# llliuqingyu/RSPL-SLAM

Measured on AMD Instinct MI355X. Metric: stereo frames/sec SuperPoint+SuperGlue+localBA @752x480 (all-keyframe: 2xSP, 2xSG, 1 BA per frame), higher is better.
Workload: dtype fp16 MFMA with fp32 accumulation for SuperPoint/SuperGlue (the reference's TensorRT kFP16 engines), fp32 Sinkhorn/decode, fp64 BA

## Files before the change

### include/rspl.h

```cpp
#ifndef RSPL_H_
#define RSPL_H_

#include <stddef.h>
#include <stdint.h>

#ifdef __cplusplus
extern "C" {
#endif

#define RSPL_OK 0
#define RSPL_E_ARG (-1)
#define RSPL_E_WEIGHTS (-2)
#define RSPL_E_DEVICE (-3)
#define RSPL_E_CAPACITY (-4)
#define RSPL_E_SOLVER (-5)

#define RSPL_FEATURE_ROWS 259

enum { RSPL_PREC_FP32 = 0, RSPL_PREC_FP16 = 1, RSPL_PREC_FP16X3 = 2 };

const char* rspl_last_error(void);
const char* rspl_version(void);
#define RSPL_ABI_VERSION 2
int rspl_abi_version(void);
// ... 163 lines not shown
  double th_mono_point, th_stereo_point, th_mono_line, th_stereo_line;
  int iterations_first;
  int iterations_second;
} rspl_ba_problem;

typedef struct {
  double* pose_q;
  double* pose_p;
  double* points;
  double* lines;
  uint8_t* mono_inlier;
  uint8_t* stereo_inlier;
  uint8_t* mono_line_inlier;
  uint8_t* stereo_line_inlier;
  double chi2_first;
  double chi2_second;
  int iterations_done_first;
  int iterations_done_second;
} rspl_ba_result;

typedef struct {
  int max_poses;
  int max_points;
  int max_lines;
  int max_edges;
  int device;
} rspl_ba_config;

typedef struct rspl_ba rspl_ba;

int rspl_ba_create(const rspl_ba_config* cfg, rspl_ba** out);
int rspl_ba_local(rspl_ba* ba, const rspl_ba_problem* problem, rspl_ba_result* result);
void rspl_ba_destroy(rspl_ba* ba);
int rspl_ba_submit(rspl_ba* ba, const rspl_ba_problem* problem, rspl_ba_result* result);
int rspl_ba_join(rspl_ba* ba, long long* calls, long long* iterations, double* ms);
int rspl_ba_use_reserved_cus(rspl_ba* ba, int reserve_cus);
int rspl_ba_kernel_timing(rspl_ba* ba, int every);
int rspl_ba_kernel_times(rspl_ba* ba, double* ms, long long* launches);
int rspl_ba_set_line_jacobian(rspl_ba* ba, int analytic);
#define RSPL_BA_TRACE_W 12
int rspl_ba_trace(rspl_ba* ba, double* out, int cap, int* n);
int rspl_ba_debug_stage(const rspl_ba_problem* problem, int par_edges, int rank, int nranks, int* n_local,
                        int* lm_off, int8_t* etype, int* epose, int* elm, int* ecam, int* gmap, int* lpose,
                        double* eobs);
typedef struct {
  int32_t nchk, lmchunk, dsub, lmsub;
  int32_t chunks, grid, ue_bpr;
  int64_t slots;
} rspl_ba_chunk_plan;
int rspl_ba_debug_chunk_plan(int n_landmarks, int n_poses, int max_landmarks, int max_poses,
                             rspl_ba_chunk_plan* out);
int rspl_ba_debug_chunk_geometry(int n_landmarks, int n_poses, int max_landmarks, int max_poses, int32_t* chunks,
                                 int32_t* order);

typedef int (*rspl_allreduce_fn)(void* ctx, double* d_buf, size_t count, void* stream);
int rspl_ba_set_shard(rspl_ba* ba, int rank, int nranks, rspl_allreduce_fn allreduce, void* ctx);

#define RSPL_COMM_ID_BYTES 128
typedef struct rspl_comm rspl_comm;
int rspl_comm_unique_id(uint8_t* id );
int rspl_comm_create(const uint8_t* id, int rank, int nranks, int device, rspl_comm** out);
int rspl_comm_allreduce_sum(void* comm, double* d_buf, size_t count, void* stream);
void rspl_comm_destroy(rspl_comm* comm);
int rspl_ba_set_comm(rspl_ba* ba, rspl_comm* comm);

typedef struct rspl_group rspl_group;
int rspl_group_create(int nranks, rspl_group** out);
void rspl_group_destroy(rspl_group* group);
int rspl_ba_set_group(rspl_ba* ba, rspl_group* group, int rank);

typedef struct {
  int n_cameras;
  const double* cameras;
  double pose_q[4];
  double pose_p[3];
  int n_points;
  const double* points;
  int n_mono;
  const int32_t* mono_point;
  const int32_t* mono_camera;
  const double* mono_obs;
  const uint8_t* mono_inlier_in;
  int n_stereo;
  const int32_t* stereo_point;
  const int32_t* stereo_camera;
  const double* stereo_obs;
  const uint8_t* stereo_inlier_in;
  double th_mono_point, th_stereo_point;
} rspl_frame_problem;

typedef struct {
  double pose_q[4];
  double pose_p[3];
  uint8_t* mono_inlier;
  uint8_t* stereo_inlier;
  int n_inliers;
  int rounds;
  int iterations[4];
  double chi2[4];
} rspl_frame_result;

typedef struct {
  int max_batch;
  int max_edges;
  int max_points;
  int device;
// ... 480 lines not shown
```

### rspl-slam_amd/api.py

```python
from __future__ import annotations

import ctypes as C
from dataclasses import dataclass, field
from typing import List, Optional, Tuple

import numpy as np

from . import capi


@dataclass
class SuperPointConfig:
    max_keypoints: int = 400
    keypoint_threshold: float = 0.004
    remove_borders: int = 4
    weights: str = ""
    max_height: int = 480
    max_width: int = 752
    max_batch: int = 2
    precision: int = capi.RSPL_PREC_FP32
    device: int = 0


class SuperPoint:
# ... 252 lines not shown

class LocalBA:

    def __init__(self, max_poses=32, max_points=20000, max_lines=2000, max_edges=200000, device=0):
        self._lib = capi.load()
        self._h = C.c_void_p()
        cfg = capi.BaConfig(max_poses, max_points, max_lines, max_edges, device)
        capi.check(self._lib.rspl_ba_create(C.byref(cfg), C.byref(self._h)), "rspl_ba_create")

    def run(self, problem, out=None):
        from .ba_types import DenseResult
        res = out if out is not None and out.fits(problem) else DenseResult.alloc(problem)
        P, R = problem.to_ctypes(), res.to_ctypes()
        capi.check(self._lib.rspl_ba_local(self._h, C.byref(P), C.byref(R)), "rspl_ba_local")
        res.read_back(R)
        return res

    def submit(self, problem, out=None):
        from .ba_types import DenseResult
        res = out if out is not None and out.fits(problem) else DenseResult.alloc(problem)
        P, R = problem.to_ctypes(), res.to_ctypes()
        inflight = self.__dict__.setdefault("_inflight", [])
        inflight.append((problem, res, P, R))
        capi.check(self._lib.rspl_ba_submit(self._h, C.byref(P), C.byref(R)), "rspl_ba_submit")
        return res

    def join(self):
        n, it, ms = C.c_longlong(), C.c_longlong(), C.c_double()
        rc = self._lib.rspl_ba_join(self._h, C.byref(n), C.byref(it), C.byref(ms))
        inflight, self._inflight = self.__dict__.get("_inflight", []), []
        for _, res, _, R in inflight:
            res.read_back(R)
        capi.check(rc, "rspl_ba_join")
        return n.value, it.value, ms.value

    def kernel_timing(self, every: int):
        capi.check(self._lib.rspl_ba_kernel_timing(self._h, every), "rspl_ba_kernel_timing")

    def kernel_times(self):
        ms, n = (C.c_double * 2)(), (C.c_longlong * 2)()
        capi.check(self._lib.rspl_ba_kernel_times(self._h, ms, n), "rspl_ba_kernel_times")
        return {"chunks+solve": (ms[0], n[0]), "update": (ms[1], n[1])}

    def set_line_jacobian(self, analytic: bool):
        capi.check(self._lib.rspl_ba_set_line_jacobian(self._h, 1 if analytic else 0), "rspl_ba_set_line_jacobian")

    def trace(self, cap=4096):
        if not hasattr(self._lib, "rspl_ba_trace"):
            return []
        buf, n = (C.c_double * (cap * capi.BA_TRACE_W))(), C.c_int()
        capi.check(self._lib.rspl_ba_trace(self._h, buf, cap, C.byref(n)), "rspl_ba_trace")
        a = np.frombuffer(buf, np.float64, n.value * capi.BA_TRACE_W).reshape(n.value, capi.BA_TRACE_W)
        return [dict(zip(capi.BA_TRACE_FIELDS, map(float, row))) for row in a]

    def use_reserved_cus(self, reserve_cus: int):
        capi.check(self._lib.rspl_ba_use_reserved_cus(self._h, reserve_cus), "rspl_ba_use_reserved_cus")

    def set_group(self, group: "ShardGroup", rank: int):
        capi.check(self._lib.rspl_ba_set_group(self._h, group.handle, rank), "rspl_ba_set_group")
        self._shard = group

    def set_shard(self, rank: int, nranks: int, host_allreduce):
        lib = self._lib
        AR = C.CFUNCTYPE(C.c_int, C.c_void_p, C.c_void_p, C.c_size_t, C.c_void_p)

        def cb(ctx, d_buf, count, stream):
            try:
                h = np.empty(count, np.float64)
                if lib.rspl_memcpy_d2h(h.ctypes.data, d_buf, count * 8, stream):
                    return -1
                host_allreduce(h)
                return 1 if lib.rspl_memcpy_h2d(d_buf, h.ctypes.data, count * 8, stream) else 0
            except Exception:
                return -1
        self._ar_cb = AR(cb)
        capi.check(lib.rspl_ba_set_shard(self._h, rank, nranks, self._ar_cb, None), "rspl_ba_set_shard")

    def set_comm(self, comm: "Comm"):
        capi.check(self._lib.rspl_ba_set_comm(self._h, comm.handle), "rspl_ba_set_comm")
        self._shard = comm

    def __del__(self):
        if getattr(self, "_h", None) and self._h.value:
            self._lib.rspl_ba_destroy(self._h)
            self._h = C.c_void_p()


class ShardGroup:

    def __init__(self, nranks: int):
        self._lib = capi.load()
        self.handle = C.c_void_p()
        self.nranks = nranks
        capi.check(self._lib.rspl_group_create(nranks, C.byref(self.handle)), "rspl_group_create")

    def __del__(self):
        if getattr(self, "handle", None) and self.handle.value:
            self._lib.rspl_group_destroy(self.handle)
            self.handle = C.c_void_p()


COMM_ID_BYTES = 128


def comm_unique_id() -> bytes:
    buf = (C.c_uint8 * COMM_ID_BYTES)()
# ... 579 lines not shown
```

### rspl-slam_amd/capi.py

```python
from __future__ import annotations

import ctypes as C
import os
import pathlib

PKG = pathlib.Path(__file__).resolve().parent
LIB_PATH = PKG / os.environ.get("RSPL_LIB", "librspl.so")

RSPL_OK = 0
RSPL_ABI_VERSION = 2
RSPL_PREC_FP32 = 0
RSPL_PREC_FP16 = 1
RSPL_PREC_FP16X3 = 2

BA_TRACE_W = 12
BA_TRACE_FIELDS = ("submit", "stage0", "stage1", "run0", "upload", "opt1", "opt2", "end", "slot", "grew", "iters",
                   "sync")

EXPORTS = [
    "rspl_last_error", "rspl_version", "rspl_abi_version",
    "rspl_device_count", "rspl_set_device", "rspl_malloc", "rspl_free", "rspl_memcpy_h2d", "rspl_memcpy_d2h",
    "rspl_memset", "rspl_memcpy_d2d", "rspl_stream_create", "rspl_stream_create_priority", "rspl_stream_create_reserving", "rspl_stream_destroy", "rspl_stream_synchronize",
    "rspl_device_synchronize", "rspl_event_create", "rspl_event_record", "rspl_stream_wait_event",
    "rspl_event_destroy", "rspl_timer_create", "rspl_timer_record", "rspl_timer_elapsed_ms",
    "rspl_timer_destroy",
    "rspl_sp_create", "rspl_sp_infer", "rspl_sp_infer_device", "rspl_sp_debug_maps", "rspl_sp_debug_nms", "rspl_sp_debug_layer",
    "rspl_sp_profile",
    "rspl_sp_stage_times", "rspl_sp_destroy",
    "rspl_sg_create", "rspl_sg_infer", "rspl_sg_infer_device", "rspl_sg_infer_device2", "rspl_sg_debug_scores", "rspl_sg_profile",
    "rspl_sg_status", "rspl_sg_debug_inject", "rspl_sg_debug_sinkhorn", "rspl_sg_debug_decode", "rspl_sg_debug_layers",
    "rspl_sg_debug_sinkhorn_plan",
    "rspl_sg_stage_times", "rspl_sg_destroy",
    "rspl_pm_match",
    "rspl_ba_create", "rspl_ba_local", "rspl_ba_submit", "rspl_ba_join", "rspl_ba_destroy", "rspl_ba_use_reserved_cus", "rspl_ba_kernel_timing",
    "rspl_ba_kernel_times", "rspl_ba_trace", "rspl_ba_set_line_jacobian", "rspl_ba_debug_stage",
    "rspl_ba_debug_chunk_plan", "rspl_ba_debug_chunk_geometry",
    "rspl_frame_create", "rspl_frame_optimize", "rspl_frame_destroy",
    "rspl_ba_set_shard", "rspl_comm_unique_id", "rspl_comm_create", "rspl_comm_allreduce_sum", "rspl_comm_destroy",
    "rspl_ba_set_comm", "rspl_group_create", "rspl_group_destroy", "rspl_ba_set_group",
    "rspl_pnp_create", "rspl_pnp_solve", "rspl_pnp_destroy", "rspl_pnp_debug_hypotheses",
    "rspl_line_extract", "rspl_lines_create", "rspl_lines_destroy", "rspl_lines_assign", "rspl_lines_match",
    "rspl_lines_stereo", "rspl_lines_stereo_device", "rspl_lines_status", "rspl_lines_detect",
    "rspl_lines_debug_canny",
    "rspl_lines_detect_device", "rspl_lines_detect_status", "rspl_lines_extract_async_device",
    "rspl_lines_debug_hysteresis", "rspl_lines_debug_chains", "rspl_lines_debug_fld_host",
    "rspl_lines_debug_fld_stats", "rspl_lines_debug_fld_profile", "rspl_lines_debug_fld_stage_ms",
    "rspl_track_create", "rspl_track_destroy", "rspl_track_set_keyframe", "rspl_track_enqueue", "rspl_track_fetch",
    "rspl_track_debug_stage", "rspl_track_keyframe_table",
    "rspl_track_enable_lines", "rspl_track_set_keyframe_lines", "rspl_track_enqueue_ext", "rspl_track_fetch_ext",
    "rspl_track_debug_lines", "rspl_track_frame_lines",
    "rspl_kf_create", "rspl_kf_destroy", "rspl_kf_enqueue", "rspl_kf_fetch", "rspl_kf_triangulate",
    "rspl_map_insert_keyframe", "rspl_map_get_mapline_observers",
    "rspl_rect_build_maps", "rspl_rect_debug_fixed", "rspl_rect_debug_sizeof", "rspl_rect_debug_copy", "rspl_rect_create", "rspl_rect_destroy",
    "rspl_rect_get_maps", "rspl_rect_set_maps", "rspl_rect_enqueue_device", "rspl_rect_pair",
    "rspl_rcf_debug_sizeof", "rspl_rcf_create", "rspl_rcf_destroy", "rspl_rcf_infer", "rspl_rcf_infer_device",
    "rspl_rcf_debug_logits", "rspl_rcf_debug_tile_rows", "rspl_rcf_profile", "rspl_rcf_stage_times",
    "rspl_fm_create", "rspl_fm_destroy", "rspl_fm_solve", "rspl_fm_enqueue", "rspl_fm_fetch",
    "rspl_fm_debug_subsets", "rspl_fm_debug_seven_point", "rspl_fm_debug_hypotheses",
]


class SpConfig(C.Structure):
    _fields_ = [("max_keypoints", C.c_int), ("keypoint_threshold", C.c_double), ("remove_borders", C.c_int),
                ("max_height", C.c_int), ("max_width", C.c_int), ("max_batch", C.c_int),
                ("precision", C.c_int), ("device", C.c_int)]


class SgConfig(C.Structure):
    _fields_ = [("image_width", C.c_int), ("image_height", C.c_int), ("max_keypoints", C.c_int),
                ("max_batch", C.c_int), ("sinkhorn_iterations", C.c_int), ("precision", C.c_int),
                ("device", C.c_int)]


class SgSinkhornPlan(C.Structure):
    _fields_ = [("kind", C.c_int32), ("groups", C.c_int32), ("rows_per_wave", C.c_int32), ("reserved", C.c_int32),
                ("ug_granules", C.c_uint64), ("vg_granules", C.c_uint64)]


class BaChunkPlan(C.Structure):
    _fields_ = [("nchk", C.c_int32), ("lmchunk", C.c_int32), ("dsub", C.c_int32), ("lmsub", C.c_int32),
                ("chunks", C.c_int32), ("grid", C.c_int32), ("ue_bpr", C.c_int32), ("slots", C.c_int64)]


class DMatch(C.Structure):
    _fields_ = [("query_idx", C.c_int32), ("train_idx", C.c_int32), ("distance", C.c_float)]


class BaConfig(C.Structure):
    _fields_ = [("max_poses", C.c_int), ("max_points", C.c_int), ("max_lines", C.c_int),
# ... 161 lines not shown
    lib.rspl_malloc.argtypes = [C.POINTER(vp), C.c_size_t]
    lib.rspl_free.argtypes = [vp]
    lib.rspl_memcpy_h2d.argtypes = [vp, vp, C.c_size_t, vp]
    lib.rspl_memcpy_d2h.argtypes = [vp, vp, C.c_size_t, vp]
    lib.rspl_memset.argtypes = [vp, ip, C.c_size_t, vp]
    lib.rspl_memcpy_d2d.argtypes = [vp, vp, C.c_size_t, vp]
    lib.rspl_sp_profile.argtypes = [vp, ip]
    lib.rspl_sp_stage_times.argtypes = [vp, C.POINTER(C.c_float), C.POINTER(ip)]
    lib.rspl_stream_create.argtypes = [C.POINTER(vp)]
    lib.rspl_stream_create_priority.argtypes = [C.POINTER(vp), ip]
    lib.rspl_stream_create_reserving.argtypes = [C.POINTER(vp), ip]
    lib.rspl_stream_destroy.argtypes = [vp]
    lib.rspl_stream_synchronize.argtypes = [vp]
    lib.rspl_event_create.argtypes = [C.POINTER(vp)]
    lib.rspl_event_record.argtypes = [vp, vp]
    lib.rspl_stream_wait_event.argtypes = [vp, vp]
    lib.rspl_event_destroy.argtypes = [vp]
    lib.rspl_timer_create.argtypes = [C.POINTER(vp)]
    lib.rspl_timer_record.argtypes = [vp, ip, vp]
    lib.rspl_timer_elapsed_ms.argtypes = [vp, C.POINTER(C.c_float)]
    lib.rspl_timer_destroy.argtypes = [vp]
    lib.rspl_timer_destroy.restype = None
    if hasattr(lib, "rspl_sg_create"):
        lib.rspl_sg_create.argtypes = [C.POINTER(SgConfig), C.c_char_p, C.POINTER(vp)]
        lib.rspl_sg_infer.argtypes = [vp, vp, ip, vp, ip, vp, vp, vp, vp]
        lib.rspl_sg_infer_device.argtypes = [vp, ip, vp, vp, vp, vp, ip, ip, vp, vp, vp, vp, vp]
        lib.rspl_sg_infer_device2.argtypes = [vp, ip, vp, vp, vp, vp, ip, ip, vp, vp, vp, vp, vp, vp]
        lib.rspl_sg_debug_scores.argtypes = [vp, ip, vp]
        lib.rspl_sg_status.argtypes = [vp, C.POINTER(C.c_uint32)]
        lib.rspl_sg_debug_inject.argtypes = [vp, ip, C.c_uint]
        lib.rspl_sg_debug_sinkhorn.argtypes = [vp, vp, ip, ip, C.c_float, ip, vp]
        lib.rspl_sg_debug_decode.argtypes = [vp, vp, ip, ip, vp, vp, vp, vp]
        lib.rspl_sg_debug_layers.argtypes = [vp, ip, vp, vp, vp, ip, ip, vp]
        lib.rspl_sg_debug_sinkhorn_plan.argtypes = [ip, ip, ip, C.POINTER(SgSinkhornPlan)]
        lib.rspl_sg_profile.argtypes = [vp, ip]
        lib.rspl_sg_stage_times.argtypes = [vp, C.POINTER(C.c_float), C.POINTER(ip)]
        lib.rspl_sg_destroy.argtypes = [vp]
        lib.rspl_sg_destroy.restype = None
        lib.rspl_pm_match.argtypes = [vp, vp, ip, vp, ip, C.POINTER(DMatch), ip, C.POINTER(ip), ip]
    if hasattr(lib, "rspl_ba_create"):
        lib.rspl_ba_create.argtypes = [C.POINTER(BaConfig), C.POINTER(vp)]
        lib.rspl_ba_local.argtypes = [vp, vp, vp]
        lib.rspl_ba_submit.argtypes = [vp, vp, vp]
        lib.rspl_ba_join.argtypes = [vp, vp, vp, vp]
        lib.rspl_ba_use_reserved_cus.argtypes = [vp, ip]
        lib.rspl_ba_kernel_timing.argtypes = [vp, ip]
        lib.rspl_ba_kernel_times.argtypes = [vp, C.POINTER(C.c_double), C.POINTER(C.c_longlong)]
        lib.rspl_ba_destroy.argtypes = [vp]
        lib.rspl_ba_destroy.restype = None
        lib.rspl_ba_debug_stage.argtypes = [vp, ip, ip, ip] + [vp] * 9
    if hasattr(lib, "rspl_ba_debug_chunk_plan"):
        lib.rspl_ba_debug_chunk_plan.argtypes = [ip, ip, ip, ip, C.POINTER(BaChunkPlan)]
        lib.rspl_ba_debug_chunk_geometry.argtypes = [ip, ip, ip, ip, vp, vp]
    if hasattr(lib, "rspl_ba_trace"):
        lib.rspl_ba_trace.argtypes = [vp, C.POINTER(C.c_double), ip, C.POINTER(ip)]
        lib.rspl_ba_set_line_jacobian.argtypes = [vp, ip]
    if hasattr(lib, "rspl_ba_set_shard"):
        lib.rspl_ba_set_shard.argtypes = [vp, ip, ip, vp, vp]
        lib.rspl_comm_unique_id.argtypes = [vp]
        lib.rspl_comm_create.argtypes = [vp, ip, ip, ip, C.POINTER(vp)]
        lib.rspl_comm_allreduce_sum.argtypes = [vp, vp, C.c_size_t, vp]
        lib.rspl_comm_destroy.argtypes = [vp]
        lib.rspl_comm_destroy.restype = None
        lib.rspl_ba_set_comm.argtypes = [vp, vp]
        lib.rspl_group_create.argtypes = [ip, C.POINTER(vp)]
        lib.rspl_group_destroy.argtypes = [vp]
        lib.rspl_group_destroy.restype = None
        lib.rspl_ba_set_group.argtypes = [vp, vp, ip]
    if hasattr(lib, "rspl_pnp_create"):
        lib.rspl_pnp_create.argtypes = [C.POINTER(PnpConfig), C.POINTER(vp)]
        lib.rspl_pnp_solve.argtypes = [vp, vp, ip, vp]
        lib.rspl_pnp_destroy.argtypes = [vp]
        lib.rspl_pnp_destroy.restype = None
        lib.rspl_pnp_debug_hypotheses.argtypes = [vp, C.c_int, C.c_int, vp, vp]
    if hasattr(lib, "rspl_fm_create"):
        lib.rspl_fm_create.argtypes = [C.POINTER(FmConfig), C.POINTER(vp)]
        lib.rspl_fm_destroy.argtypes = [vp]
        lib.rspl_fm_destroy.restype = None
        lib.rspl_fm_solve.argtypes = [vp, vp, ip, vp]
        lib.rspl_fm_enqueue.argtypes = [vp, ip, vp, vp]
        lib.rspl_fm_fetch.argtypes = [vp, vp]
        lib.rspl_fm_debug_subsets.argtypes = [ip, ip, vp, vp, vp, C.POINTER(C.c_int)]
        lib.rspl_fm_debug_seven_point.argtypes = [vp, vp, vp, C.POINTER(C.c_int)]
        lib.rspl_fm_debug_hypotheses.argtypes = [vp, ip, ip, vp, vp, vp]
    if hasattr(lib, "rspl_frame_create"):
        lib.rspl_frame_create.argtypes = [C.POINTER(FrameConfig), C.POINTER(vp)]
        lib.rspl_frame_optimize.argtypes = [vp, vp, ip, vp]
        lib.rspl_frame_destroy.argtypes = [vp]
        lib.rspl_frame_destroy.restype = None
    if hasattr(lib, "rspl_track_create"):
        lib.rspl_track_create.argtypes = [C.POINTER(TrackConfig), C.POINTER(vp)]
        lib.rspl_track_destroy.argtypes = [vp]
        lib.rspl_track_destroy.restype = None
        lib.rspl_track_set_keyframe.argtypes = [vp, ip, ip, vp, vp, vp, vp]
        lib.rspl_track_enqueue.argtypes = [vp, ip, vp, vp]
        lib.rspl_track_fetch.argtypes = [vp, vp]
        lib.rspl_track_debug_stage.argtypes = [vp, ip, C.POINTER(TrackDebug)]
    if hasattr(lib, "rspl_track_enable_lines"):
        lib.rspl_track_enable_lines.argtypes = [vp, C.POINTER(TrackLinesConfig)]
        lib.rspl_track_set_keyframe_lines.argtypes = [vp, ip, ip, vp, vp, vp, vp, vp, vp]
        lib.rspl_track_enqueue_ext.argtypes = [vp, ip, vp, vp, vp]
        lib.rspl_track_fetch_ext.argtypes = [vp, vp, vp]
        lib.rspl_track_debug_lines.argtypes = [vp, ip, C.POINTER(TrackDebugLines)]
        lib.rspl_track_frame_lines.argtypes = [vp, ip, C.POINTER(vp), C.POINTER(vp)]
    if hasattr(lib, "rspl_kf_create"):
        lib.rspl_track_keyframe_table.argtypes = [vp, ip, ip, C.POINTER(vp), C.POINTER(vp), C.POINTER(vp)]
# ... 165 lines not shown
```

### rspl-slam_amd/csrc/ba.cpp

```cpp
#include <immintrin.h>

#include <algorithm>
#include <chrono>
#include <cmath>
#include <cstdlib>
#include <cstring>
#include <limits>
#include <numeric>
#include <string>
#include <type_traits>
#include <memory>
#include <vector>
#include <condition_variable>
#include <deque>
#include <mutex>
#include <thread>

#include "ba_kernels.hpp"
#include "common.hpp"
#include "ba_stage.hpp"
#include "se3_host.hpp"

using namespace rspl;

// ... 27 lines not shown
  int *pp_cnt, *pp_off;
  size_t chunk_slots = 0;
  int4* pp_buf = nullptr;
  size_t pp_cap = 0;
  char* cbuf[2] = {nullptr, nullptr};
  char* stage[2] = {nullptr, nullptr};
  char* stage_dev[2] = {nullptr, nullptr};
  size_t stage_cap[2] = {0, 0};
  ba::Mail* mail = nullptr;
  ba::Mail* mail_dev = nullptr;
  unsigned long long seq = 0;
  ba::Stager stg;
  int rank = 0, nranks = 1;
  rspl_allreduce_fn allreduce = nullptr;
  void* ar_ctx = nullptr;
  double* red = nullptr;
  ba::LmCtrl* lmctl = nullptr;
  double* lm_trace = nullptr;
  double* gbuf = nullptr;
  size_t gcap = 0;
  double* pdg = nullptr;
  size_t pdg_cap = 0;
  int ktime_every = 0;
  unsigned long long ncalls = 0;
  bool ktime_on = false;
  std::vector<hipEvent_t> kev;
  std::vector<int> kev_eval;
  int kev_used = 0;
  double kt_ms[2] = {0, 0};
  long long kt_n[2] = {0, 0};
  struct Job {
    const rspl_ba_problem* pr;
    rspl_ba_result* res;
    std::shared_ptr<ba::StagedCall> sc;
    int state;
  };
  std::thread worker;
  std::thread stager;
  bool slot_busy[2] = {false, false};
  std::mutex qmu;
  std::condition_variable qcv;
  std::deque<Job> jobs;
  bool busy = false, quit = false;
  bool tracking_call = false;
  int q_err = 0;
  std::string q_msg;
  long long q_done = 0, q_iters = 0;
  double q_ms = 0.0;
  static constexpr int kTraceCap = 4096;
  std::vector<double> trace;
  long long trace_n = 0;
  unsigned grew = 0;
  int line_jac = 0;
};

namespace {

constexpr int kMaxCams = 16;
constexpr int kMaxRanks = 64;
constexpr int kParEdges = 8192;
constexpr int kChunkWaves = 1024;
constexpr int kEventTrials = 64;
int allreduce(rspl_ba* b, double* d, size_t n) {
  const int rc = b->allreduce(b->ar_ctx, d, n, b->stream);
  if (rc) {
    set_error("BA shard all-reduce failed (rank %d of %d, %zu doubles, rc %d)", b->rank, b->nranks, n, rc);
    return RSPL_E_DEVICE;
  }
  return RSPL_OK;
}


struct CallLayout {
  size_t cams, T, X, L, obs, type, pose, lm, cam, gmap, lm_pose, pidx, lm_off, lm_act, pairs, ltab, level, flags, out,
      bytes;
  CallLayout() = default;
  CallLayout(int ncam, int np, int nq, int nl, int E, size_t nobs) {
    const size_t nL = (size_t)nq + nl;
    size_t so = 0;
    auto place = [&](size_t n) {
      const size_t o = so;
      so = al256(so + n);
      return o;
    };
    cams = place(sizeof(double) * 5 * ncam); T = place(sizeof(double) * 8 * np); X = place(sizeof(double) * 3 * nq);
    L = place(sizeof(double) * 6 * nl); obs = place(sizeof(double) * nobs); type = place(E);
    pose = place(4 * (size_t)E); lm = place(4 * (size_t)E); cam = place(4 * (size_t)E); gmap = place(4 * (size_t)E);
    lm_pose = place(4 * (size_t)E);
    pidx = place(4 * (size_t)np); lm_off = place(4 * (nL + 1)); lm_act = place(nL);
    pairs = place(8 * (size_t)np * (np + 1) / 2);
    const size_t line_edges = nobs >= 4 * (size_t)E ? (nobs - 4 * (size_t)E) / 4 : 0;
    ltab = place(16 * ((size_t)nl + line_edges / ba::kLineBlk + 2));
    level = place(E); flags = place(4 * sizeof(int)); out = place(8 * sizeof(double));
    bytes = so;
  }
};

struct DownLayout {
  size_t inl, T, X, L, bytes;
  DownLayout() = default;
  DownLayout(int np, int nq, int nl, int E) {
    inl = 0; T = al256(E); X = T + al256(sizeof(double) * 8 * np); L = X + al256(sizeof(double) * 3 * nq);
    bytes = L + al256(sizeof(double) * 6 * nl);
  }
};

struct HostMarks {
  static bool on() {
    static const bool t = getenv("RSPL_BA_TIMING") != nullptr;
    return t;
  }
  std::chrono::steady_clock::time_point t[16];
  const char* name[16];
  int n = 0;
  void mark(const char* s) {
    if (on() && n < 16) {
      name[n] = s;
      t[n++] = std::chrono::steady_clock::now();
    }
  }
  void print(const char* label) const {
    if (!on()) return;
    fprintf(stderr, "%s", label);
    for (int i = 1; i < n; i++)
      fprintf(stderr, " %s %.1f", name[i], std::chrono::duration<double, std::micro>(t[i] - t[i - 1]).count());
    fprintf(stderr, "\n");
  }
};

double mono_s() {
  timespec ts;
  clock_gettime(CLOCK_MONOTONIC, &ts);
  return (double)ts.tv_sec + 1e-9 * (double)ts.tv_nsec;
}

}

struct rspl::ba::StagedCall {
  int slot = 0;
  int rc = RSPL_OK;
  std::string msg;
  int E = 0, Ep = 0, K = 0, n_lblk = 0;
  size_t pair_bound = 0;
  CallLayout cl;
  DownLayout dl;
  HostMarks tm;
  double tr[RSPL_BA_TRACE_W] = {};
  bool uploaded = false;
};

namespace {

template <typename F>
void carve(F& ar, rspl_ba* b) {
  const size_t E = b->maxE, NL = b->maxL, K = b->maxK, nq = b->cfg.max_points, nl = b->cfg.max_lines;
  auto take = [&](auto*& p, size_t n) {
    using Tp = std::remove_pointer_t<std::remove_reference_t<decltype(p)>>;
    if constexpr (std::is_same_v<F, Arena>) p = ar.template take<Tp>(n ? n : 1);
    else ar.template take<Tp>(n ? n : 1);
  };
  take(b->Tb, K * 8); take(b->Xb, nq * 3); take(b->Lb, nl * 6);
  take(b->err, E * 4);
  for (LinBank& k : b->bank) {
    take(k.Hpp, E * 21); take(k.bp, E * 6); take(k.Hll, E * 16); take(k.bl, E * 4); take(k.Hpl, E * 24);
  }
  take(b->bank[1].lm_Hll, NL * 16); take(b->bank[1].lm_bl, NL * 4);
  take(b->lm_act2, NL);
  take(b->bank[0].lm_Hll, NL * 16); take(b->bank[0].lm_bl, NL * 4); take(b->bp, K * 6);
  const size_t nblk = std::max(E / 256, NL * 8 / 256) + 2;
  take(b->S, 36 * K * K); take(b->x, 6 * K); take(b->partial, nblk + NL + E / ba::kLineBlk + 1032);
  take(b->partial2, std::max(std::max((size_t)b->maxV / 256, nblk) + 1026, K * (E / 256 + 1) * 6));
  take(b->lm_ctr, nl);
  const size_t npairs = K * (K + 1) / 2, slots = ba::chunk_slots_for((int)NL, (int)K);
  take(b->chunk, slots * 48); take(b->pairfin, npairs * 48 + 8); take(b->pair_ctr, npairs + 1);
  take(b->red, 6 * K + kMaxRanks + 8);
  take(b->lmctl, 2);
  take(b->pp_cnt, slots); take(b->pp_off, slots + 1);
  b->chunk_slots = slots;
}

int ensure_stage(rspl_ba* b, int slot, size_t bytes, bool* grew = nullptr) {
  if (bytes <= b->stage_cap[slot]) return RSPL_OK;
  const size_t cap = std::max(bytes, b->stage_cap[slot] * 2);
  char *nh = nullptr, *nd = nullptr;
  RSPL_HIP(hipHostMalloc((void**)&nh, cap, hipHostMallocMapped | hipHostMallocCoherent));
  if (hipHostGetDevicePointer((void**)&nd, nh, 0) != hipSuccess) {
    (void)hipHostFree(nh);
    set_error("BA staging slot: no device mapping");
    return RSPL_E_DEVICE;
  }
  if (b->stage[slot]) (void)hipHostFree(b->stage[slot]);
  b->stage[slot] = nh;
  b->stage_dev[slot] = nd;
  b->stage_cap[slot] = cap;
  if (grew) *grew = true;
  return RSPL_OK;
// ... 34 lines not shown
    volatile const double* mv = b->mail->v;
    for (int k = 0; k < 4; k++) v[k] = mv[k];
  }
  return RSPL_OK;
}

template <typename T>
int grow_device(rspl_ba* b, T*& buf, size_t& cap, size_t need, size_t min_cap, unsigned grew_bit) {
  if (need <= cap) return RSPL_OK;
  RSPL_HIP(hipStreamSynchronize(b->stream));
  if (buf) (void)hipFree(buf);
  buf = nullptr;
  cap = 0;
  const size_t n = std::max(need, min_cap);
  RSPL_HIP(hipMalloc((void**)&buf, sizeof(T) * n));
  cap = n;
  b->grew |= grew_bit;
  return RSPL_OK;
}

using se3h::Se3h;

void report_prof(rspl_ba* b) {
  std::vector<unsigned long long> h(ba::kProfLen);
  if (hipStreamSynchronize(b->stream) != hipSuccess ||
      hipMemcpy(h.data(), b->prof, sizeof(unsigned long long) * h.size(), hipMemcpyDeviceToHost) != hipSuccess)
    return;
  auto us = [](unsigned long long a, unsigned long long c) { return c && a ? ((double)c - (double)a) / 100.0 : -1.0; };
  auto first = [&](int off, int b0, int b1) {
    unsigned long long t = ~0ull;
    for (int i = b0; i < std::min(b1, 4096); i++)
      if (h[off + 4 * i]) t = std::min(t, h[off + 4 * i]);
    return t;
  };
  auto last = [&](int off, int b0, int b1, int slot) {
    unsigned long long t = 0;
    for (int i = b0; i < std::min(b1, 4096); i++) t = std::max(t, h[off + 4 * i + slot]);
    return t;
  };
  const int npc = b->prof_nb[0], nue = b->prof_nb[1], nbu = b->prof_nb[2];
  const unsigned long long p0 = first(ba::kProfPc, 0, npc), u0 = first(ba::kProfUe, 0, nue);
  fprintf(stderr,
          "ba_prof us: pcstarts %.1f pcloop %.1f pcticket %.1f pcend %.1f gap %.1f asm %.1f factor %.1f back %.1f"
          " poses %.1f gap %.1f uestarts %.1f loaded %.1f grpdone %.1f groupsend %.1f lineswait %.1f linescomp %.1f"
          " linesend %.1f sApanel %.1f sAtrail %.1f sBpanel %.1f sBtrail %.1f\n",
          us(p0, last(ba::kProfPc, 0, npc, 0)), us(p0, last(ba::kProfPc, 0, npc, 1)),
          us(p0, last(ba::kProfPc, 0, npc, 2)), us(p0, last(ba::kProfPc, 0, npc, 3)),
          us(last(ba::kProfPc, 0, npc, 3), h[0]), us(h[0], h[1]), us(h[1], h[2]), us(h[2], h[3]), us(h[3], h[4]),
          us(h[4], u0), us(u0, last(ba::kProfUe, 0, nue, 0)), us(u0, last(ba::kProfUe, 0, nbu, 1)),
          us(u0, last(ba::kProfUe, 0, nbu, 2)), us(u0, last(ba::kProfUe, 0, nbu, 3)),
          us(u0, last(ba::kProfUe, nbu, nue, 1)), us(u0, last(ba::kProfUe, nbu, nue, 2)),
          us(u0, last(ba::kProfUe, nbu, nue, 3)), us(h[1], h[5]), us(h[5], h[6]), us(h[6], h[7]), us(h[7], h[8]));
  fprintf(stderr,
          "ba_prof setup us: landmarks %.1f +pdiag %.1f lines %.1f +pdiag %.1f pairs %.1f | blocks done %.1f scan %.1f "
          "pose diagonals + control %.1f\n",
          us(h[9], h[ba::kProfX]), us(h[9], h[ba::kProfX + 1]), us(h[9], h[ba::kProfX + 2]),
          us(h[9], h[ba::kProfX + 3]), us(h[9], h[ba::kProfX + 4]), us(h[9], h[10]),
          us(h[10], h[11]), us(h[11], h[12]));
  {
    const int nchk = b->prof_nb[3], K = b->prof_nb[4];
    std::vector<double> dg, od;
    for (int c = 0; c < std::min(npc, 4096) && nchk > 0; c++) {
      const unsigned long long t0 = h[ba::kProfPc + 4 * c], t1 = h[ba::kProfPc + 4 * c + 1];
      if (!t0 || !t1) continue;
      int pr = ba::chunk_geo(b->prof_A, c).pr, a = 0, base = 0;
      while (pr >= base + (K - a)) base += K - a++;
      ((pr - base == 0) ? dg : od).push_back(((double)t1 - (double)t0) / 100.0);
    }
    auto q = [](std::vector<double>& v, double f) {
      if (v.empty()) return -1.0;
      std::sort(v.begin(), v.end());
      return v[std::min(v.size() - 1, (size_t)(f * v.size()))];
    };
    fprintf(stderr, "ba_chunks us: diag50 %.1f diag90 %.1f diagmax %.1f off50 %.1f off90 %.1f offmax %.1f "
            "ndiag %zu noff %zu\n", q(dg, 0.5), q(dg, 0.9), q(dg, 1.0), q(od, 0.5), q(od, 0.9), q(od, 1.0),
            dg.size(), od.size());
  }
  {
    std::vector<double> w, c, e, tot;
    for (int i = nbu; i < std::min(nue, 4096); i++) {
      const unsigned long long* r = &h[ba::kProfUe + 4 * i];
      if (!r[0] || !r[1] || !r[2] || !r[3]) continue;
      w.push_back((r[1] - (double)r[0]) / 100.0);
      c.push_back((r[2] - (double)r[1]) / 100.0);
      e.push_back((r[3] - (double)r[2]) / 100.0);
      tot.push_back((r[3] - (double)u0) / 100.0);
    }
    auto q = [](std::vector<double> v, double f) {
      if (v.empty()) return -1.0;
      std::sort(v.begin(), v.end());
      return v[std::min(v.size() - 1, (size_t)(f * v.size()))];
    };
    fprintf(stderr, "ba_lines us (p50/p90/max): operands %.1f/%.1f/%.1f evals %.1f/%.1f/%.1f tail %.1f/%.1f/%.1f "
            "end %.1f/%.1f/%.1f n %zu\n", q(w, .5), q(w, .9), q(w, 1), q(c, .5), q(c, .9), q(c, 1), q(e, .5), q(e, .9),
            q(e, 1), q(tot, .5), q(tot, .9), q(tot, 1), w.size());
  }
  b->prof_nb[0] = 0;
  (void)hipMemset(b->prof, 0, sizeof(unsigned long long) * ba::kProfLen);
}

void view_bank(const LinBank& k, ba::Lin& L, ba::Sys& S) {
  L.Hpp = k.Hpp; L.bp = k.bp; L.Hll = k.Hll; L.bl = k.bl; L.Hpl = k.Hpl;
  S.Hll = k.lm_Hll; S.bl = k.lm_bl;
}
void bank_views(const rspl_ba* b, ba::Lin& Lr, ba::Sys& S, ba::Lin& Ls, ba::Sys& Ss) {
  view_bank(b->bank[0], Lr, S);
  Ls = Lr;
  Ss = S;
  view_bank(b->bank[1], Ls, Ss);
}

void accept_swap(rspl_ba* b, ba::Problem& P, ba::Lin& Lr, ba::Sys& S, bool lin) {
  std::swap(P.T, P.Tn);
  std::swap(P.X, P.Xn);
  std::swap(P.L, P.Ln);
  if (!lin) return;
  std::swap(b->bank[0], b->bank[1]);
  view_bank(b->bank[0], Lr, S);
}

void arm_prof(rspl_ba* b, const ba::Active& A, ba::Sys& S) {
  if (!b->prof || b->prof_nb[0]) return;
  S.prof = b->prof;
  b->prof_A = A;
  b->prof_nb[0] = ba::chunk_count(A);
  b->prof_nb[1] = ba::update_errors_blocks(A) + A.n_lblk;
  b->prof_nb[2] = ba::update_errors_blocks(A);
  b->prof_nb[3] = A.nchk;
  b->prof_nb[4] = A.K;
}

struct SpecSetup {
  ba::Active A2{};
  uint8_t* level = nullptr;
  int iters2 = 0;
  bool queued = false;
  bool extra = false;
  bool topped_up = false;
};

struct SpecFinish {
  bool on = false;
  ba::Lin L{};
  int E = 0;
  const int* gmap = nullptr;
  uint8_t* inl = nullptr;
  double *Th = nullptr, *Xh = nullptr, *Lh = nullptr;
  unsigned long long q = 0;
};

void preupload_next(rspl_ba* b);

struct DevLmArgs {
  uint8_t* cls_level = nullptr;
  bool build_pp = false;
  SpecFinish* fin = nullptr;
  SpecSetup* nxt = nullptr;
  bool setup_done = false;
};

int optimize_dev(rspl_ba* b, ba::Problem& P, ba::Lin& Lr, ba::Sys& S, const ba::Active& A, int iters,
                 double* chi2_out, int* done_out, const DevLmArgs& d) {
  hipStream_t st = b->stream;
  uint8_t* const cls_level = d.cls_level;
  SpecFinish* const fin = d.fin;
  SpecSetup* const nxt = d.nxt;
  S.lm = b->lmctl;
  S.lm_slot = 0;
  static const bool trace = getenv("RSPL_BA_LMTRACE") != nullptr;
  if (trace && !b->lm_trace) {
    RSPL_HIP(hipMalloc((void**)&b->lm_trace, sizeof(double) * 8 * 64));
    RSPL_HIP(hipMemset(b->lm_trace, 0, sizeof(double) * 8 * 64));
  }
  S.lm_trace = trace ? b->lm_trace + (iters == 10 ? 0 : 8 * 32) : nullptr;
  if (d.setup_done) {
  } else {
    int rg;
    if ((rg = grow_device(b, b->pdg, b->pdg_cap, (size_t)ba::setup_pdg_len(A), (size_t)1 << 14, 4u))) return rg;
    ba::Sys Su = S;
    Su.prof = b->prof && !b->prof_nb[0] && !cls_level ? b->prof : nullptr;
    RSPL_HIP(ba::setup_dev(P, Lr, A, Su, cls_level, cls_level ? const_cast<uint8_t*>(A.lm_act) : nullptr, iters,
                           d.build_pp ? b->pp_cnt : nullptr, b->pp_off, b->pp_buf, b->pdg, st));
  }
  unsigned long long q = b->seq;
  const unsigned long long q_first = b->seq + 1;
  ba::Lin Ls;
  ba::Sys Ss;
  bank_views(b, Lr, S, Ls, Ss);
  int queued = 0;
  const int kev0 = b->kev_used;
  auto enqueue = [&](int n) -> int {
    for (int k = 0; k < n; k++, queued++) {
      q = ++b->seq;
      ba::Spec sp{Ls, Ss};
      if (queued == 3) arm_prof(b, A, S);
      S.lm_slot = queued & 1;
      S.lm_post = k == n - 1;
      hipEvent_t* ev = nullptr;
      if (b->ktime_on) {
        if ((size_t)3 * (b->kev_used + 1) > b->kev.size()) {
          for (int i = 0; i < 3; i++) {
            hipEvent_t e;
            RSPL_HIP(hipEventCreate(&e));
            b->kev.push_back(e);
          }
          b->grew |= 8;
        }
        ev = &b->kev[3 * (size_t)b->kev_used++];
      }
      const hipError_t e = ba::trial_dev(P, Lr, A, S, q, st, sp, ev);
      S.prof = nullptr;
      if (e != hipSuccess) {
        set_error("BA trial launch failed: %s", hipGetErrorString(e));
        return RSPL_E_DEVICE;
      }
    }
    return RSPL_OK;
  };
  int rc;
  unsigned long long q_last = 0;
  auto enqueue_batch = [&](int n) -> int {
    int r;
    if ((r = enqueue(n))) return r;
    q_last = b->seq;
    if (fin) {
      ba::Sys Sf = S;
      Sf.lm = b->lmctl;
      Sf.lm_slot = queued & 1;
      Sf.prof = nullptr;
      fin->q = ++b->seq;
      fin->on = true;
      RSPL_HIP(ba::finish(P, fin->L, fin->E, fin->gmap, fin->inl, fin->Th, fin->Xh, fin->Lh, Sf, fin->q, st));
    }
    return RSPL_OK;
  };
  if ((rc = enqueue_batch(iters))) return rc;
  if (fin) preupload_next(b);
  auto queue_spec_setup = [&]() -> int {
    if (!nxt || (size_t)ba::setup_pdg_len(nxt->A2) > b->pdg_cap) return RSPL_OK;
    ba::Sys S2 = S;
    S2.lm = b->lmctl;
    S2.lm_slot = 0;
    S2.prof = nullptr;
    S2.lm_trace = nullptr;
    RSPL_HIP(ba::setup_dev(P, Lr, nxt->A2, S2, nxt->level, const_cast<uint8_t*>(nxt->A2.lm_act), nxt->iters2,
                           nullptr, b->pp_off, b->pp_buf, b->pdg, st, queued & 1, &Ls, &Ss));
    nxt->queued = true;
    nxt->extra = false;
    return RSPL_OK;
  };
  if ((rc = queue_spec_setup())) return rc;
  double v[4];
  for (;;) {
    if ((rc = spin_mail(b, "the LM trials", [&] {
          const unsigned long long s1 = __atomic_load_n(&b->mail->seq, __ATOMIC_ACQUIRE);
          if (s1 >= q_first && s1 <= q_last) {
            volatile const double* mv = b->mail->v;
            for (int k = 0; k < 4; k++) v[k] = mv[k];
            __atomic_thread_fence(__ATOMIC_ACQUIRE);
            return __atomic_load_n(&b->mail->vseq, __ATOMIC_ACQUIRE) == s1 && (s1 == q_last || v[3] != 0.0);
          }
          if (fin && s1 == fin->q) {
            volatile const double* mv = b->mail->v;
            for (int k = 0; k < 4; k++) v[k] = mv[k];
            __atomic_thread_fence(__ATOMIC_ACQUIRE);
            const unsigned long long vs = __atomic_load_n(&b->mail->vseq, __ATOMIC_ACQUIRE);
            return vs >= q_first && vs <= q_last && v[3] != 0.0;
          }
          return false;
        })))
      return rc;
    if (v[3] != 0.0) {
      if (b->ktime_on) {
        unsigned long long s1 = __atomic_load_n(&b->mail->seq, __ATOMIC_ACQUIRE);
        for (unsigned long long t = q_first; t <= s1 && t <= q_last; t++) b->kev_eval.push_back(kev0 + (int)(t - q_first));
      }
      break;
    }
    if (nxt) nxt->extra = nxt->topped_up = true;
    if ((rc = enqueue_batch(std::max(1, iters - (int)v[1])))) return rc;
    if ((rc = queue_spec_setup())) return rc;
  }
  S.lm = nullptr;
  if (v[2] != 0.0) accept_swap(b, P, Lr, S, true);
  *chi2_out = v[0];
  *done_out = (int)v[1];
  return RSPL_OK;
}

bool dev_lm(const rspl_ba* b, const ba::Active& A, int iters) {
  return b->allreduce == nullptr && iters > 0 && ba::fast_path(A.K);
}

int optimize_host(rspl_ba* b, ba::Problem& P, ba::Lin& Lr, ba::Sys& S, const ba::Active& A, int iters,
                  double* chi2_out, int* done_out) {
  hipStream_t st = b->stream;
  double v[4];
  int rc;
  const bool sh = b->allreduce != nullptr;
// ... 54 lines not shown
      const double scale = ok ? v[1] + 1e-3 : 1.0;
      rho /= scale;
      if (rho > 0 && std::isfinite(tempChi) && ok) {
        double alpha = 1. - std::pow(2 * rho - 1, 3);
        alpha = std::min(alpha, 2. / 3.);
        lambda *= std::max(1. / 3., alpha);
        ni = 2;
        currentChi = tempChi;
        accept_swap(b, P, Lr, S, it + 1 < iters);
      } else {
        lambda *= ni;
        ni *= 2;
        if (!std::isfinite(lambda)) break;
      }
      qmax++;
    } while (rho < 0 && qmax < 10);
    done++;
    if (qmax == 10 || rho == 0 || !std::isfinite(lambda)) break;
  }
  *chi2_out = currentChi;
  *done_out = done;
  return RSPL_OK;
}

int optimize(rspl_ba* b, ba::Problem& P, ba::Lin& Lr, ba::Sys& S, const ba::Active& A, int iters,
             double* chi2_out, int* done_out, const DevLmArgs& d = {}) {
  return dev_lm(b, A, iters) ? optimize_dev(b, P, Lr, S, A, iters, chi2_out, done_out, d)
                             : optimize_host(b, P, Lr, S, A, iters, chi2_out, done_out);
}

}

extern "C" int rspl_ba_create(const rspl_ba_config* cfg, rspl_ba** out) {
  RSPL_CHECK_ARG(cfg && out, "rspl_ba_create: NULL argument");
  RSPL_CHECK_ARG(cfg->max_poses > 0 && cfg->max_poses <= 64 && cfg->max_points >= 0 && cfg->max_lines >= 0 &&
                     cfg->max_edges >= 0,
                 "capacities: 1 <= max_poses <= 64, others >= 0");
  *out = nullptr;
  RSPL_HIP(hipSetDevice(cfg->device));
  auto* b = new rspl_ba();
  b->cfg = *cfg;
  b->maxE = 4 * cfg->max_edges;
  b->maxL = cfg->max_points + cfg->max_lines;
  b->maxK = cfg->max_poses;
  b->maxV = cfg->max_poses + cfg->max_points + cfg->max_lines;
  Sizer sz;
  carve(sz, b);
  int rc = b->arena.reserve(sz.used);
  if (rc) { delete b; return rc; }
  carve(b->arena, b);
  int prio_lo = 0, prio_hi = 0;
  (void)hipDeviceGetStreamPriorityRange(&prio_lo, &prio_hi);
  {
    const size_t cbytes = CallLayout(kMaxCams, b->maxK, cfg->max_points, cfg->max_lines, b->maxE, 8 * (size_t)b->maxE).bytes;
    const char* what = nullptr;
    hipError_t e = hipSuccess;
    auto step = [&](hipError_t r, const char* w) {
      if (e == hipSuccess && r != hipSuccess) {
        e = r;
        what = w;
      }
    };
    step(hipStreamCreateWithPriority(&b->stream, hipStreamNonBlocking, prio_hi), "hipStreamCreateWithPriority");
    if (e == hipSuccess)
      step(hipHostMalloc((void**)&b->mail, sizeof(ba::Mail), hipHostMallocMapped | hipHostMallocCoherent), "hipHostMalloc(mailbox)");
    if (e == hipSuccess) step(hipHostGetDevicePointer((void**)&b->mail_dev, b->mail, 0), "hipHostGetDevicePointer(mailbox)");
    for (int i = 0; i < 2 && e == hipSuccess; i++) step(hipMalloc((void**)&b->cbuf[i], cbytes), "hipMalloc(call buffer)");
    if (e == hipSuccess) step(hipMemset(b->lm_ctr, 0, sizeof(unsigned) * std::max(b->cfg.max_lines, 1)), "hipMemset(lm_ctr)");
    if (e == hipSuccess)
      step(hipMemset(b->pair_ctr, 0, sizeof(unsigned) * (b->maxK * (b->maxK + 1) / 2 + 1)), "hipMemset(pair_ctr)");
    if (e != hipSuccess) {
      set_error("BA stream / mailbox allocation failed: %s: %s (call buffer %zu bytes, arena %zu bytes)", what,
                hipGetErrorString(e), cbytes, b->arena.size);
      rspl_ba_destroy(b);
      return RSPL_E_DEVICE;
    }
  }
  memset(b->mail, 0, sizeof(ba::Mail));
  {
    const size_t sb = std::max(CallLayout(kMaxCams, b->maxK, cfg->max_points, cfg->max_lines, b->maxE,
                                          8 * (size_t)b->maxE).bytes,
                               DownLayout(b->maxK, cfg->max_points, cfg->max_lines, b->maxE).bytes);
    ba::Active Amax{};
    Amax.nL = b->maxL;
    Amax.K = b->maxK;
    Amax.n_lblk = cfg->max_lines + b->maxE / ba::kLineBlk + 2;
    const size_t pdg = (size_t)ba::setup_pdg_len(Amax);
    const size_t pp = std::max<size_t>((size_t)1 << 16, 8 * (size_t)b->maxE);
    if (ensure_stage(b, 0, sb) || ensure_stage(b, 1, sb) ||
        hipMalloc((void**)&b->pdg, sizeof(double) * pdg) != hipSuccess ||
        hipMalloc((void**)&b->pp_buf, sizeof(int4) * pp) != hipSuccess) {
      set_error("BA staging / scratch allocation failed");
      rspl_ba_destroy(b);
      return RSPL_E_DEVICE;
    }
    b->pdg_cap = pdg;
    b->pp_cap = pp;
  }
  b->trace.assign((size_t)rspl_ba::kTraceCap * RSPL_BA_TRACE_W, 0.0);
  if (getenv("RSPL_BA_PROF") &&
      (hipMalloc((void**)&b->prof, sizeof(unsigned long long) * ba::kProfLen) != hipSuccess ||
       hipMemset(b->prof, 0, sizeof(unsigned long long) * ba::kProfLen) != hipSuccess)) {
    set_error("BA trace allocation failed");
    rspl_ba_destroy(b);
    return RSPL_E_DEVICE;
  }
  *out = b;
  return RSPL_OK;
}

extern "C" int rspl_ba_use_reserved_cus(rspl_ba* b, int reserve_cus) {
  RSPL_CHECK_ARG(b, "rspl_ba_use_reserved_cus: NULL handle");
  hipStream_t ns = nullptr;
  if (reserve_cus > 0) {
    std::vector<uint32_t> mask;
    int rc = cu_mask(reserve_cus, true, mask);
    if (rc) return rc;
    RSPL_HIP(hipExtStreamCreateWithCUMask(&ns, (uint32_t)mask.size(), mask.data()));
  } else {
    int lo = 0, hi = 0;
    RSPL_HIP(hipDeviceGetStreamPriorityRange(&lo, &hi));
    RSPL_HIP(hipStreamCreateWithPriority(&ns, hipStreamNonBlocking, hi));
  }
  RSPL_HIP(hipStreamSynchronize(b->stream));
  RSPL_HIP(hipStreamDestroy(b->stream));
  b->stream = ns;
  return RSPL_OK;
}

namespace {
bool queue_active(rspl_ba* b);
}

extern "C" int rspl_ba_set_shard(rspl_ba* b, int rank, int nranks, rspl_allreduce_fn fn, void* ctx) {
  RSPL_CHECK_ARG(b, "rspl_ba_set_shard: NULL handle");
  RSPL_CHECK_ARG(!queue_active(b), "rspl_ba_set_shard: calls are queued on the tracking thread (rspl_ba_join first)");
  RSPL_CHECK_ARG(nranks >= 1 && nranks <= kMaxRanks && rank >= 0 && rank < nranks, "rank %d of %d (1..%d ranks)", rank,
                 nranks, kMaxRanks);
  RSPL_CHECK_ARG(nranks == 1 || fn, "an all-reduce function is required for nranks > 1");
  b->rank = rank;
  b->nranks = nranks;
  b->allreduce = fn;
  b->ar_ctx = ctx;
  return RSPL_OK;
}

extern "C" void rspl_ba_destroy(rspl_ba* b) {
  if (!b) return;
  if (b->worker.joinable()) {
    {
      std::lock_guard<std::mutex> lk(b->qmu);
      b->quit = true;
    }
    b->qcv.notify_all();
    b->worker.join();
    b->stager.join();
  }
  for (hipEvent_t e : b->kev) (void)hipEventDestroy(e);
  if (b->stream) (void)hipStreamSynchronize(b->stream);
  if (b->gbuf) (void)hipFree(b->gbuf);
  if (b->pdg) (void)hipFree(b->pdg);
  b->arena.release();
  for (char* cb : b->cbuf)
    if (cb) (void)hipFree(cb);
  if (b->pp_buf) (void)hipFree(b->pp_buf);
  if (b->prof) (void)hipFree(b->prof);
  for (char* sg : b->stage)
    if (sg) (void)hipHostFree(sg);
  if (b->mail) (void)hipHostFree(b->mail);
  if (b->stream) (void)hipStreamDestroy(b->stream);
  delete b;
}

namespace {
int ba_local_impl(rspl_ba* b, const rspl_ba_problem* pr, rspl_ba_result* res);
int stage_call(rspl_ba* b, int slot, const rspl_ba_problem* pr, rspl_ba_result* res, ba::StagedCall& c);
int run_call(rspl_ba* b, const ba::StagedCall& c, const rspl_ba_problem* pr, rspl_ba_result* res, double* tr);
void push_trace(rspl_ba* b, const double* tr);

bool queue_active(rspl_ba* b) {
  std::lock_guard<std::mutex> lk(b->qmu);
  return !b->jobs.empty() || b->busy;
}

void begin_call(rspl_ba* b) {
  b->ktime_on = b->ktime_every > 0 && b->ncalls++ % (unsigned long long)b->ktime_every == 0;
  b->kev_used = 0;
  b->kev_eval.clear();
}

int end_call(rspl_ba* b, int rc) {
  if (rc != RSPL_E_DEVICE) return rc;
  const std::string msg = rspl_last_error();
  if (hipStreamSynchronize(b->stream) != hipSuccess ||
      hipMemset(b->lm_ctr, 0, sizeof(unsigned) * std::max(b->cfg.max_lines, 1)) != hipSuccess ||
      hipMemset(b->pair_ctr, 0, sizeof(unsigned) * (b->maxK * (b->maxK + 1) / 2 + 1)) != hipSuccess) {
    set_error("%s; the BA stream could not be drained: recreate the handle", msg.c_str());
    return rc;
  }
  set_error("%s", msg.c_str());
  return rc;
}
}

extern "C" int rspl_ba_kernel_timing(rspl_ba* b, int every) {
  RSPL_CHECK_ARG(b && every >= 0, "rspl_ba_kernel_timing: NULL handle or every < 0");
  RSPL_CHECK_ARG(!queue_active(b), "rspl_ba_kernel_timing: calls are queued on the tracking thread (rspl_ba_join first)");
  for (size_t n = b->kev.size(); every > 0 && n < 3 * (size_t)kEventTrials; n++) {
    hipEvent_t e;
    RSPL_HIP(hipEventCreate(&e));
    b->kev.push_back(e);
  }
  b->ktime_every = every;
  b->ncalls = 0;
  return RSPL_OK;
}

extern "C" int rspl_ba_set_line_jacobian(rspl_ba* b, int analytic) {
  RSPL_CHECK_ARG(b && (analytic == 0 || analytic == 1), "rspl_ba_set_line_jacobian: NULL handle or mode not 0 / 1");
  RSPL_CHECK_ARG(!queue_active(b), "rspl_ba_set_line_jacobian: calls are queued on the tracking thread (rspl_ba_join first)");
  b->line_jac = analytic;
  return RSPL_OK;
}

extern "C" int rspl_ba_trace(rspl_ba* b, double* out, int cap, int* n) {
  RSPL_CHECK_ARG(b && n && cap >= 0 && (out || cap == 0), "rspl_ba_trace: NULL argument or cap < 0");
  std::lock_guard<std::mutex> lk(b->qmu);
  const long long have = std::min<long long>(b->trace_n, rspl_ba::kTraceCap);
  const long long first = b->trace_n - have;
  const int m = (int)std::min<long long>(have, cap);
  for (int i = 0; i < m; i++) {
    const size_t r = (size_t)((first + i) % rspl_ba::kTraceCap);
    std::copy(b->trace.begin() + r * RSPL_BA_TRACE_W, b->trace.begin() + (r + 1) * RSPL_BA_TRACE_W,
              out + (size_t)i * RSPL_BA_TRACE_W);
  }
  *n = m;
  b->trace_n = 0;
  return RSPL_OK;
}

extern "C" int rspl_ba_kernel_times(rspl_ba* b, double* ms, long long* launches) {
  RSPL_CHECK_ARG(b && ms && launches, "rspl_ba_kernel_times: NULL argument");
  for (int i = 0; i < 2; i++) {
    ms[i] = b->kt_ms[i];
    launches[i] = b->kt_n[i];
    b->kt_ms[i] = 0;
    b->kt_n[i] = 0;
  }
  return RSPL_OK;
}

extern "C" int rspl_ba_local(rspl_ba* b, const rspl_ba_problem* pr, rspl_ba_result* res) {
  if (!b) return ba_local_impl(b, pr, res);
  RSPL_CHECK_ARG(!queue_active(b), "rspl_ba_local: calls are queued on the tracking thread (rspl_ba_join first)");
  begin_call(b);
  return end_call(b, ba_local_impl(b, pr, res));
}

namespace {
constexpr size_t kTrackingBuffer = 2;

void staging_loop(rspl_ba* b) {
  (void)hipSetDevice(b->cfg.device);
  std::unique_lock<std::mutex> lk(b->qmu);
  for (;;) {
    rspl_ba::Job* j = nullptr;
    int slot = -1;
    b->qcv.wait(lk, [&] {
      j = nullptr;
      for (rspl_ba::Job& q : b->jobs)
        if (q.state == 0) {
          j = &q;
          break;
        }
      slot = !b->slot_busy[0] ? 0 : !b->slot_busy[1] ? 1 : -1;
      return (j && slot >= 0) || (b->quit && !j);
    });
    if (!j) return;
    j->state = 1;
    b->slot_busy[slot] = true;
    const std::shared_ptr<ba::StagedCall> sc = j->sc;
    const rspl_ba_problem* pr = j->pr;
    rspl_ba_result* res = j->res;
    lk.unlock();
    sc->slot = slot;
    sc->tr[1] = mono_s();
    sc->rc = stage_call(b, slot, pr, res, *sc);
    sc->tr[2] = mono_s();
    sc->tr[8] = slot;
    if (sc->rc) sc->msg = rspl_last_error();
    lk.lock();
    j->state = 2;
    b->qcv.notify_all();
  }
}

void tracking_loop(rspl_ba* b) {
  (void)hipSetDevice(b->cfg.device);
  std::unique_lock<std::mutex> lk(b->qmu);
  for (;;) {
    b->qcv.wait(lk, [&] { return (!b->jobs.empty() && b->jobs.front().state == 2) || (b->quit && b->jobs.empty()); });
    if (b->jobs.empty()) return;
    const rspl_ba::Job j = b->jobs.front();
    b->jobs.pop_front();
    b->busy = true;
    lk.unlock();
    b->qcv.notify_all();
    const auto t0 = std::chrono::steady_clock::now();
    j.sc->tr[3] = mono_s();
    int rc;
    if (j.sc->rc) {
      set_error("%s", j.sc->msg.c_str());
      rc = j.sc->rc;
    } else {
      begin_call(b);
      b->tracking_call = true;
      rc = end_call(b, run_call(b, *j.sc, j.pr, j.res, j.sc->tr));
      b->tracking_call = false;
    }
    const double ms = std::chrono::duration<double, std::milli>(std::chrono::steady_clock::now() - t0).count();
    const std::string msg = rc ? std::string(rspl_last_error()) : std::string();
    lk.lock();
    b->slot_busy[j.sc->slot] = false;
    b->busy = false;
    b->q_done++;
    b->q_ms += ms;
    if (!rc) push_trace(b, j.sc->tr);
    if (!rc) b->q_iters += j.res->iterations_done_first + j.res->iterations_done_second;
    if (rc && !b->q_err) {
      b->q_err = rc;
      b->q_msg = msg;
    }
    b->qcv.notify_all();
  }
}
}

extern "C" int rspl_ba_submit(rspl_ba* b, const rspl_ba_problem* pr, rspl_ba_result* res) {
  RSPL_CHECK_ARG(b && pr && res, "rspl_ba_submit: NULL argument");
  std::unique_lock<std::mutex> lk(b->qmu);
// ... 70 lines not shown
}

extern "C" int rspl_ba_debug_chunk_geometry(int n_landmarks, int n_poses, int max_landmarks, int max_poses,
                                            int32_t* chunks, int32_t* order) {
  RSPL_CHECK_ARG(chunks && order, "rspl_ba_debug_chunk_geometry: NULL argument");
  rspl_ba_chunk_plan pl;
  if (const int rc = rspl_ba_debug_chunk_plan(n_landmarks, n_poses, max_landmarks, max_poses, &pl)) return rc;
  ba::Active A{};
  A.nchk = pl.nchk; A.lmchunk = pl.lmchunk; A.dsub = pl.dsub; A.lmsub = pl.lmsub;
  A.K = n_poses;
  A.npairs = n_poses * (n_poses + 1) / 2;
  A.nL = n_landmarks;
  for (int c = 0; c < pl.chunks; c++) {
    const ba::ChunkGeo q = ba::chunk_geo(A, c);
    const int32_t row[6] = {q.pr, q.g0, q.g1, q.c0, q.c1, q.gend};
    std::copy(row, row + 6, chunks + 6 * c);
  }
  for (int vb = 0; vb < pl.grid; vb++) {
    int c = -1;
    ba::ChunkGeo q;
    order[vb] = -1;
    if (!ba::chunk_at(A, vb, c, q)) continue;
    const ba::ChunkGeo r = ba::chunk_geo(A, c);
    const bool same = q.pr == r.pr && q.lb == r.lb && q.g0 == r.g0 && q.g1 == r.g1 && q.gend == r.gend &&
                      q.c0 == r.c0 && q.c1 == r.c1;
    order[vb] = same ? c : -2;
  }
  return RSPL_OK;
}

extern "C" int rspl_ba_debug_stage(const rspl_ba_problem* pr, int par_edges, int rank, int nranks, int* n_local,
                                   int* lm_off, int8_t* etype, int* epose, int* elm, int* ecam, int* gmap,
                                   int* lpose, double* eobs) {
  RSPL_CHECK_ARG(pr && n_local && lm_off && etype && epose && elm && ecam && gmap && lpose && eobs,
                 "rspl_ba_debug_stage: NULL argument");
  RSPL_CHECK_ARG(pr->n_poses >= 0 && pr->n_points >= 0 && pr->n_lines >= 0 && pr->n_mono >= 0 &&
                     pr->n_stereo >= 0 && pr->n_mono_line >= 0 && pr->n_stereo_line >= 0 &&
                     (pr->n_poses == 0 || pr->pose_fixed) && pr->n_cameras >= 1,
                 "rspl_ba_debug_stage: bad problem sizes");
  RSPL_CHECK_ARG(nranks >= 1 && rank >= 0 && rank < nranks, "rspl_ba_debug_stage: bad rank");
  ba::Stager stg;
  int rc;
  if ((rc = stg.count(pr, nranks > 1, rank, nranks, par_edges))) return rc;
  std::vector<int> pidx(pr->n_poses);
  int K = 0;
  for (int p = 0; p < pr->n_poses; p++) pidx[p] = (stg.pose_has_edge[p] && !pr->pose_fixed[p]) ? K++ : -1;
  ba::Stager::Out so{lm_off, etype, epose, elm, ecam, gmap, lpose, eobs, pidx.data()};
  stg.place(pr, so);
  n_local[0] = stg.E;
  n_local[1] = stg.Ep;
  return RSPL_OK;
}

namespace {
int stage_call(rspl_ba* b, int slot, const rspl_ba_problem* pr, rspl_ba_result* res, ba::StagedCall& c) {
  RSPL_CHECK_ARG(b && pr && res, "rspl_ba_local: NULL argument");
  const int np = pr->n_poses, nq = pr->n_points, nl = pr->n_lines;
  const int ne[4] = {pr->n_mono, pr->n_stereo, pr->n_mono_line, pr->n_stereo_line};
  RSPL_CHECK_ARG(np >= 0 && np <= b->cfg.max_poses && nq >= 0 && nq <= b->cfg.max_points && nl >= 0 &&
                     nl <= b->cfg.max_lines,
                 "problem exceeds the handle's vertex capacity");
  for (int t = 0; t < 4; t++) RSPL_CHECK_ARG(ne[t] >= 0 && ne[t] <= b->cfg.max_edges, "edge capacity exceeded");
  RSPL_CHECK_ARG(pr->n_cameras >= 1 && pr->n_cameras <= kMaxCams && pr->cameras, "1..16 cameras required");
  RSPL_CHECK_ARG(res->pose_q && res->pose_p && (res->points || !nq) && (res->lines || !nl), "NULL result arrays");
  RSPL_CHECK_ARG(np == 0 || pr->pose_fixed, "NULL pose_fixed");
  const int Eg = ne[0] + ne[1] + ne[2] + ne[3], nL = nq + nl;
  const bool sh = b->allreduce != nullptr;
  HostMarks tm;
  tm.mark("start");
  int rc;
  if ((rc = b->stg.count(pr, sh, b->rank, b->nranks, kParEdges))) return rc;
  const int E = b->stg.E, Ep = b->stg.Ep, n_line_local = E - Ep;
  tm.mark("count");
  const CallLayout cl(pr->n_cameras, np, nq, nl, E, 4 * (size_t)Ep + 8 * (size_t)(E - Ep));
  const DownLayout dl(np, nq, nl, Eg);
  bool grew = false;
  if ((rc = ensure_stage(b, slot, std::max(cl.bytes, dl.bytes), &grew))) return rc;
  if (grew) c.tr[9] = (double)((unsigned)c.tr[9] | 1u);
  char* sg = b->stage[slot];
  double* T = reinterpret_cast<double*>(sg + cl.T);
  for (int p = 0; p < np; p++) {
    Se3h Twc;
    Twc.q[0] = pr->pose_q[4 * p + 3];
    Twc.q[1] = pr->pose_q[4 * p + 0];
    Twc.q[2] = pr->pose_q[4 * p + 1];
    Twc.q[3] = pr->pose_q[4 * p + 2];
    for (int k = 0; k < 3; k++) Twc.t[k] = pr->pose_p[3 * p + k];
    normalize(Twc);
    const Se3h Tcw = inverse(Twc);
    for (int k = 0; k < 4; k++) T[8 * p + k] = Tcw.q[k];
    for (int k = 0; k < 3; k++) T[8 * p + 4 + k] = Tcw.t[k];
    T[8 * p + 7] = 0;
  }
  int* pidx = reinterpret_cast<int*>(sg + cl.pidx);
  int K = 0;
  for (int p = 0; p < np; p++) pidx[p] = (b->stg.pose_has_edge[p] && !pr->pose_fixed[p]) ? K++ : -1;
  int* lm_off = reinterpret_cast<int*>(sg + cl.lm_off);
  tm.mark("vertices");
  {
    ba::Stager::Out so;
    so.lm_off = lm_off;
    so.etype = reinterpret_cast<int8_t*>(sg + cl.type);
    so.epose = reinterpret_cast<int*>(sg + cl.pose);
    so.elm = reinterpret_cast<int*>(sg + cl.lm);
    so.ecam = reinterpret_cast<int*>(sg + cl.cam);
    so.gmap = reinterpret_cast<int*>(sg + cl.gmap);
    so.lpose = reinterpret_cast<int*>(sg + cl.lm_pose);
    so.eobs = reinterpret_cast<double*>(sg + cl.obs);
    so.pidx = pidx;
    b->stg.place(pr, so);
  }
  tm.mark("scatter");
  uint8_t* lm_act = reinterpret_cast<uint8_t*>(sg + cl.lm_act);
  size_t pair_bound = 0;
  for (int g = 0; g < nL; g++) {
    const size_t k = lm_off[g + 1] - lm_off[g];
    pair_bound += k * k;
    lm_act[g] = k > 0;
  }
  int4* ltab = reinterpret_cast<int4*>(sg + cl.ltab);
  int n_lblk = 0;
  {
    constexpr int kB = ba::kLineBlk;
    int p0 = 0, cnt = 0, gb = -1, ge = 0;
    auto flush = [&]() {
      if (gb >= 0 && cnt > 0) ltab[n_lblk++] = make_int4(p0, cnt, gb, ge);
      gb = -1;
      cnt = 0;
    };
    for (int g = nq; g < nL; g++) {
      const int k = lm_off[g + 1] - lm_off[g];
      if (k > kB) {
        flush();
        for (int o = 0; o < k; o += kB) ltab[n_lblk++] = make_int4(lm_off[g] + o, std::min(kB, k - o) | (1 << 8), g, g + 1);
        continue;
      }
      if (gb >= 0 && (cnt + k > kB || g - gb >= kB)) flush();
      if (gb < 0) {
        p0 = lm_off[g];
        gb = g;
      }
      cnt += k;
      ge = g + 1;
    }
    flush();
  }
  int* pairs = reinterpret_cast<int*>(sg + cl.pairs);
  for (int a = 0, q = 0; a < K; a++)
    for (int c = a; c < K; c++, q++) {
      pairs[2 * q] = a;
      pairs[2 * q + 1] = c;
    }
  tm.mark("tables");
  memcpy(sg + cl.cams, pr->cameras, sizeof(double) * 5 * pr->n_cameras);
  if (nq) memcpy(sg + cl.X, pr->points, sizeof(double) * 3 * nq);
  if (nl) memcpy(sg + cl.L, pr->lines, sizeof(double) * 6 * nl);
  memset(sg + cl.level, 0, cl.bytes - cl.level);
  c.slot = slot;
  c.E = E;
  c.Ep = Ep;
  c.K = K;
  c.n_lblk = n_lblk;
  c.pair_bound = pair_bound;
  c.cl = cl;
  c.dl = dl;
  c.tm = tm;
  return RSPL_OK;
}

void preupload_next(rspl_ba* b) {
  if (!b->tracking_call) return;
  std::shared_ptr<ba::StagedCall> nx;
  {
    std::lock_guard<std::mutex> lk(b->qmu);
    if (!b->jobs.empty() && b->jobs.front().state == 2 && b->jobs.front().sc->rc == RSPL_OK) nx = b->jobs.front().sc;
  }
  if (!nx || nx->uploaded) return;
  if (upload_mapped(b->cbuf[nx->slot], b->stage_dev[nx->slot], nx->cl.bytes, b->stream) == hipSuccess)
    nx->uploaded = true;
}

int run_call(rspl_ba* b, const ba::StagedCall& c, const rspl_ba_problem* pr, rspl_ba_result* res, double* tr) {
  const int np = pr->n_poses, nq = pr->n_points, nl = pr->n_lines;
  const int ne[4] = {pr->n_mono, pr->n_stereo, pr->n_mono_line, pr->n_stereo_line};
  hipStream_t st = b->stream;
  const int Eg = ne[0] + ne[1] + ne[2] + ne[3], nL = nq + nl;
  const bool sh = b->allreduce != nullptr;
  const int E = c.E, Ep = c.Ep, n_line_local = E - Ep, K = c.K, n_lblk = c.n_lblk;
  const size_t pair_bound = c.pair_bound;
  const CallLayout& cl = c.cl;
  const DownLayout& dl = c.dl;
  char* sg = b->stage[c.slot];
  HostMarks tm = c.tm;
  int rc;
  tm.mark("run");
  b->grew = 0;
  if ((rc = grow_device(b, b->pp_buf, b->pp_cap, pair_bound, (size_t)1 << 16, 2u))) return rc;
  char* cb = b->cbuf[c.slot];
  if (!c.uploaded)
    RSPL_HIP(upload_mapped(cb, b->stage_dev[c.slot], cl.bytes, st));
  tm.mark("upload");
  tr[4] = mono_s();
  uint8_t* level = reinterpret_cast<uint8_t*>(cb + cl.level);
  ba::Problem P{};
  P.cams = reinterpret_cast<double*>(cb + cl.cams);
  P.T = reinterpret_cast<double*>(cb + cl.T);
// ... 2 lines not shown
  P.np = np; P.nq = nq; P.nl = nl; P.ncam = pr->n_cameras;
  P.Tn = b->Tb; P.Xn = b->Xb; P.Ln = b->Lb;
  P.etype = reinterpret_cast<const int8_t*>(cb + cl.type);
  P.epose = reinterpret_cast<const int*>(cb + cl.pose);
  P.elm = reinterpret_cast<const int*>(cb + cl.lm);
  P.ecam = reinterpret_cast<const int*>(cb + cl.cam);
  P.eobs = reinterpret_cast<const double*>(cb + cl.obs);
  P.Ep = Ep;
  const double th[4] = {pr->th_mono_point, pr->th_stereo_point, pr->th_mono_line, pr->th_stereo_line};
  for (int t = 0; t < 4; t++) {
    P.th[t] = th[t];
    P.delta[t] = (double)(float)std::sqrt(th[t]);
  }
  P.line_jac = b->line_jac;
  ba::Lin Lr{};
  Lr.err = b->err;
  ba::Sys S{};
  view_bank(b->bank[0], Lr, S);
  S.bp = b->bp; S.S = b->S; S.x = b->x; S.partial = b->partial;
  S.partial2 = b->partial2;
  S.out = reinterpret_cast<double*>(cb + cl.out);
  S.fail = reinterpret_cast<int*>(cb + cl.flags);
  S.counter = reinterpret_cast<unsigned*>(cb + cl.flags + sizeof(int));
  S.lm_ctr = b->lm_ctr;
  S.mail = b->mail_dev;
  S.chunk = b->chunk;
  S.pairfin = b->pairfin;
  S.pair_ctr = b->pair_ctr;
  S.solve_ctr = b->pair_ctr + b->maxK * (b->maxK + 1) / 2;
  S.shard_out = sh ? b->red + 6 * K + b->nranks : nullptr;
  S.pose_scale = !sh || b->rank == 0;
  ba::Active A{};
  A.Ea = E;
  A.pidx = reinterpret_cast<const int*>(cb + cl.pidx);
  A.lm_off = reinterpret_cast<const int*>(cb + cl.lm_off);
  A.lm_pose = reinterpret_cast<const int*>(cb + cl.lm_pose);
  A.lm_act = reinterpret_cast<const uint8_t*>(cb + cl.lm_act);
  A.pairs = reinterpret_cast<const int*>(cb + cl.pairs);
  A.npairs = K * (K + 1) / 2;
  {
    const ba::ChunkPlan cp = ba::chunk_plan(nL, K, b->chunk_slots);
    A.nchk = cp.nchk;
    A.lmchunk = cp.lmchunk;
    A.dsub = cp.dsub;
    A.lmsub = cp.lmsub;
    ba::set_update_geometry(A);
  }
  A.n_line_edges = n_line_local;
  A.ltab = reinterpret_cast<const int4*>(cb + cl.ltab);
  A.n_lblk = n_lblk;
  A.K = K;
  A.nL = nL;
  A.robust = 1;
  A.pp_off = b->pp_off;
  A.pp = b->pp_buf;
  const bool pp_fused = dev_lm(b, A, pr->iterations_first);
  if (!pp_fused) RSPL_HIP(ba::build_pairs(A, b->pp_cnt, b->pp_off, b->pp_buf, st));
  tm.mark("pairs");
  SpecSetup nxt;
  nxt.A2 = A;
  nxt.A2.robust = 0;
  nxt.A2.elevel = level;
  nxt.A2.lm_act = b->lm_act2;
  nxt.level = level;
  nxt.iters2 = pr->iterations_second;
  const bool spec_setup = pp_fused && !sh && !b->ktime_on && dev_lm(b, nxt.A2, pr->iterations_second);
  DevLmArgs d1;
  d1.build_pp = pp_fused;
  d1.nxt = spec_setup ? &nxt : nullptr;
  if ((rc = optimize(b, P, Lr, S, A, pr->iterations_first, &res->chi2_first, &res->iterations_done_first, d1)))
    return rc;
  tm.mark("opt1");
  tr[5] = mono_s();
  uint8_t* inl_h = reinterpret_cast<uint8_t*>(b->stage_dev[c.slot] + dl.inl);
  double* T_h = reinterpret_cast<double*>(b->stage_dev[c.slot] + dl.T);
  double* X_h = reinterpret_cast<double*>(b->stage_dev[c.slot] + dl.X);
  double* L_h = reinterpret_cast<double*>(b->stage_dev[c.slot] + dl.L);
  SpecFinish fin;
  {
    A.robust = 0;
    A.elevel = level;
    A.lm_act = b->lm_act2;
    const bool fused = dev_lm(b, A, pr->iterations_second);
    if (!fused) {
      RSPL_HIP(ba::classify(P, Lr, E, level, nullptr, 0, st));
      RSPL_HIP(ba::landmark_active(A, level, b->lm_act2, st));
    }
    const bool spec_fin = fused && !sh && !b->ktime_on;
    if (spec_fin) {
      fin.L = Lr;
      fin.E = E;
      fin.gmap = reinterpret_cast<const int*>(cb + cl.gmap);
      fin.inl = inl_h;
      fin.Th = T_h;
      fin.Xh = X_h;
      fin.Lh = L_h;
    }
    DevLmArgs d2;
    d2.cls_level = fused ? level : nullptr;
    d2.fin = spec_fin ? &fin : nullptr;
    d2.setup_done = nxt.queued && !nxt.extra;
    if ((rc = optimize(b, P, Lr, S, A, pr->iterations_second, &res->chi2_second, &res->iterations_done_second, d2)))
      return rc;
    tm.mark("opt2");
    tr[6] = mono_s();
    tr[9] = (double)((unsigned)tr[9] | (nxt.queued && !nxt.extra ? 16u : 0u) | (nxt.topped_up ? 32u : 0u));
  }
  const unsigned long long q = fin.on ? fin.q : ++b->seq;
  if (fin.on) {
  } else if (sh) {
    const size_t glen = 3 * (size_t)nq + 6 * (size_t)nl + Eg;
    if ((rc = grow_device(b, b->gbuf, b->gcap, glen, (size_t)1024, 0u))) return rc;
    RSPL_HIP(hipMemsetAsync(b->gbuf, 0, sizeof(double) * glen, st));
    RSPL_HIP(ba::shard_gather(P, Lr, E, reinterpret_cast<const int*>(cb + cl.gmap), b->rank, b->nranks, b->gbuf, st));
    if (glen && (rc = allreduce(b, b->gbuf, glen))) return rc;
    RSPL_HIP(ba::shard_finish(P, Eg, b->gbuf, inl_h, T_h, X_h, L_h, S, q, st));
  } else {
    RSPL_HIP(ba::finish(P, Lr, E, reinterpret_cast<const int*>(cb + cl.gmap), inl_h, T_h, X_h, L_h, S, q, st));
  }
  if ((rc = wait_mail(b, q, nullptr))) return rc;
  if (b->ktime_on) {
    for (int i : b->kev_eval) {
      float a = 0.f, c = 0.f;
      if (hipEventElapsedTime(&a, b->kev[3 * (size_t)i], b->kev[3 * (size_t)i + 1]) == hipSuccess &&
          hipEventElapsedTime(&c, b->kev[3 * (size_t)i + 1], b->kev[3 * (size_t)i + 2]) == hipSuccess) {
        b->kt_ms[0] += a;
        b->kt_ms[1] += c;
        b->kt_n[0]++;
        b->kt_n[1]++;
      }
    }
  }
  if (b->prof && b->prof_nb[0]) report_prof(b);
  tr[9] = (double)((unsigned)tr[9] | b->grew);
  if (b->lm_trace) {
    std::vector<double> h(8 * 64);
    if (hipMemcpy(h.data(), b->lm_trace, sizeof(double) * h.size(), hipMemcpyDeviceToHost) == hipSuccess)
      for (int k = 0; k < 64; k++)
        if (h[8 * k] != 0.0)
          fprintf(stderr, "lmtrace phase %d trial %d chi2 %.17g scale %.6g fail %g lambda %.6g chi0 %.17g cur %g it %g q %g\n",
                  k / 32, k % 32, h[8 * k], h[8 * k + 1], h[8 * k + 2], h[8 * k + 3], h[8 * k + 4], h[8 * k + 5],
                  h[8 * k + 6], h[8 * k + 7]);
    (void)hipMemset(b->lm_trace, 0, sizeof(double) * h.size());
  }
  if (nq) memcpy(res->points, b->stage[c.slot] + dl.X, sizeof(double) * 3 * nq);
  if (nl) memcpy(res->lines, b->stage[c.slot] + dl.L, sizeof(double) * 6 * nl);
  const double* Tout = reinterpret_cast<const double*>(b->stage[c.slot] + dl.T);
  uint8_t* outs[4] = {res->mono_inlier, res->stereo_inlier, res->mono_line_inlier, res->stereo_line_inlier};
  int e = 0;
  for (int t = 0; t < 4; t++) {
    if (outs[t]) memcpy(outs[t], b->stage[c.slot] + dl.inl + e, ne[t]);
    e += ne[t];
  }
  for (int p = 0; p < np; p++) {
    Se3h Tcw;
    for (int k = 0; k < 4; k++) Tcw.q[k] = Tout[8 * p + k];
    for (int k = 0; k < 3; k++) Tcw.t[k] = Tout[8 * p + 4 + k];
    const Se3h Twc = inverse(Tcw);
    res->pose_q[4 * p + 0] = Twc.q[1];
    res->pose_q[4 * p + 1] = Twc.q[2];
    res->pose_q[4 * p + 2] = Twc.q[3];
    res->pose_q[4 * p + 3] = Twc.q[0];
    for (int k = 0; k < 3; k++) res->pose_p[3 * p + k] = Twc.t[k];
  }
  tm.mark("final");
  tm.print("rspl_ba_local us:");
  tr[7] = mono_s();
  tr[10] = res->iterations_done_first + res->iterations_done_second;
  return RSPL_OK;
}

int ba_local_impl(rspl_ba* b, const rspl_ba_problem* pr, rspl_ba_result* res) {
  RSPL_CHECK_ARG(b && pr && res, "rspl_ba_local: NULL argument");
  ba::StagedCall c;
  c.tr[0] = c.tr[1] = mono_s();
  c.tr[11] = 1;
  int rc = stage_call(b, 0, pr, res, c);
  c.tr[2] = c.tr[3] = mono_s();
  if (!rc) rc = run_call(b, c, pr, res, c.tr);
  if (!rc) {
    std::lock_guard<std::mutex> lk(b->qmu);
    push_trace(b, c.tr);
  }
  return rc;
}

void push_trace(rspl_ba* b, const double* tr) {
  if (b->trace.empty()) return;
  const size_t i = (size_t)(b->trace_n++ % rspl_ba::kTraceCap);
  std::copy(tr, tr + RSPL_BA_TRACE_W, b->trace.begin() + i * RSPL_BA_TRACE_W);
}
}
```

### rspl-slam_amd/csrc/ba_first.hip

```cpp
#include <hip/hip_runtime.h>

#include <algorithm>
#include <cstdint>

#include "ba_kernels.hpp"
#include "ba_linearize.hpp"

namespace rspl {
namespace ba {

__global__ __launch_bounds__(256) void post_kernel(Sys S, int K, int npd, unsigned long long seq) {
  __shared__ double part[4][64];
  if (npd > 0) {
    const int lane = threadIdx.x & 63, pt = threadIdx.x >> 6, nq6 = 6 * K;
    double mx = 0;
    for (int q0 = 0; q0 < nq6; q0 += 64) {
      const int q = q0 + lane;
      double sacc = 0;
      if (q < nq6) {
        const int pa = q / 6, i = q - 6 * pa;
        const double* src = S.partial2 + (size_t)pa * npd * 6 + i;
        for (int b = pt; b < npd; b += 4) sacc += src[(size_t)b * 6];
      }
      part[pt][lane] = sacc;
// ... 105 lines not shown
    __syncthreads();
  }
}

constexpr int kPdCap = 512;
__device__ __forceinline__ void pose_diag_lds(const Active& A, const double (*pd)[6], const int* pa, int n, double* dst,
                                              int nb, int b) {
  __shared__ double ws[4][64];
  const int lane = threadIdx.x & 63, wv = threadIdx.x >> 6;
  const int l0 = (n * wv) / 4, l1 = (n * (wv + 1)) / 4, nq = 6 * A.K;
  for (int q0 = 0; q0 < nq; q0 += 64) {
    const int q = q0 + lane, j = q / 6, i = q - 6 * j;
    double sm = 0;
    if (q < nq)
      for (int l = l0; l < l1; l += 8) {
        int pv[8];
        double dv[8];
#pragma unroll
        for (int u = 0; u < 8; u++) {
          const bool ok = l + u < l1;
          pv[u] = ok ? pa[l + u] : -1;
          dv[u] = ok ? pd[l + u][i] : 0.0;
        }
#pragma unroll
        for (int u = 0; u < 8; u++) sm += pv[u] == j ? dv[u] : 0.0;
      }
    ws[wv][lane] = sm;
    __syncthreads();
    if (wv == 0 && q < nq)
      __hip_atomic_store(dst + ((size_t)j * nb + b) * 6 + i, ((ws[0][lane] + ws[1][lane]) + ws[2][lane]) + ws[3][lane],
                         __ATOMIC_RELAXED, __HIP_MEMORY_SCOPE_AGENT);
    __syncthreads();
  }
}

template <bool FILL>
__device__ __forceinline__ void pair_scan(const Active& A, int c, int* pp_cnt, const int* pp_off, int4* pp) {
  const int lane = threadIdx.x & 63;
  int pr, g0, g1, nr;
  if (A.dsub <= 1) {
    pr = c / A.nchk;
    g0 = (c - pr * A.nchk) * A.lmchunk;
    g1 = A.nL;
    nr = A.lmchunk / 64;
  } else {
    const ChunkGeo cg = chunk_geo(A, c);
    pr = cg.pr;
    g0 = cg.g0;
    g1 = cg.g1;
    nr = (cg.g1 - cg.g0 + 63) / 64;
  }
  const int pa = A.pairs[2 * pr], pb = A.pairs[2 * pr + 1];
  int base = FILL ? pp_off[c] : 0;
  for (int r0 = 0; r0 < nr; r0 += 4) {
    int k0[4], k1[4], pz[4][8];
#pragma unroll
    for (int u = 0; u < 4; u++) {
      const int g = g0 + 64 * (r0 + u) + lane;
      const bool in = r0 + u < nr && g < g1;
      const int o0 = in ? A.lm_off[g] : 0, o1 = in ? A.lm_off[g + 1] : 0;
      const bool act = in && A.lm_act[g];
      k0[u] = act ? o0 : 0;
      k1[u] = act ? o1 : 0;
    }
#pragma unroll
    for (int u = 0; u < 4; u++)
#pragma unroll
      for (int v = 0; v < 8; v++) pz[u][v] = k1[u] > k0[u] ? A.lm_pose[min(k0[u] + v, k1[u] - 1)] : -1;
#pragma unroll
    for (int u = 0; u < 4; u++) {
      if (r0 + u >= nr) break;
      const int g = g0 + 64 * (r0 + u) + lane;
      const int e0 = k0[u], e1 = k1[u];
      int cnt = 0;
      unsigned ma1 = 0, mb1 = 0;
      if (e1 - e0 <= 8) {
        unsigned ma = 0, mb = 0;
#pragma unroll
        for (int v = 0; v < 8; v++) {
          ma |= (e0 + v < e1 && pz[u][v] == pa) ? 1u << v : 0u;
          mb |= (e0 + v < e1 && pz[u][v] == pb) ? 1u << v : 0u;
        }
        cnt = ma ? __popc(ma) * __popc(mb) : 0;
        ma1 = ma;
        mb1 = mb;
      } else {
        for (int ib = e0; ib < e1; ib += 8) {
          unsigned ma = 0;
          for (int v = 0; v < 8 && ib + v < e1; v++) ma |= A.lm_pose[ib + v] == pa ? 1u << v : 0u;
          if (!ma) continue;
          for (int jb = e0; jb < e1; jb += 8) {
            unsigned mb = 0;
            for (int v = 0; v < 8 && jb + v < e1; v++) mb |= A.lm_pose[jb + v] == pb ? 1u << v : 0u;
            cnt += __popc(ma) * __popc(mb);
          }
        }
      }
      int pre = cnt;
#pragma unroll
      for (int o = 1; o < 64; o <<= 1) {
        const int t = __shfl_up(pre, o);
        if (lane >= o) pre += t;
      }
      const int total = __shfl(pre, 63);
      if (FILL && cnt && e1 - e0 <= 8) {
        int q = base + pre - cnt;
        for (unsigned ma = ma1; ma; ma &= ma - 1) {
          const int ea = (e0 + __ffs(ma) - 1);
          for (unsigned mb = mb1; mb; mb &= mb - 1) pp[q++] = make_int4(ea, (e0 + __ffs(mb) - 1), g, 0);
        }
      } else if (FILL && cnt) {
        int q = base + pre - cnt;
        for (int ib = e0; ib < e1; ib++) {
          if (A.lm_pose[ib] != pa) continue;
          for (int jb = e0; jb < e1; jb++) {
            if (A.lm_pose[jb] != pb) continue;
            pp[q] = make_int4(ib, jb, g, 0);
            q++;
          }
        }
      }
      base += total;
    }
  }
  if (!FILL && lane == 0) __hip_atomic_store(pp_cnt + c, base, __ATOMIC_RELAXED, __HIP_MEMORY_SCOPE_AGENT);
}

__global__ __launch_bounds__(64) void pair_count_kernel(Active A, int* pp_cnt) {
  pair_scan<false>(A, blockIdx.x, pp_cnt, nullptr, nullptr);
}
__global__ __launch_bounds__(64) void pair_fill_kernel(Active A, const int* pp_off, int4* pp) {
  pair_scan<true>(A, blockIdx.x, nullptr, pp_off, pp);
}
__global__ __launch_bounds__(1024) void pair_offsets_kernel(const int* cnt, int* off, int n) {
  __shared__ int part[1024];
  const int tid = threadIdx.x;
  const int per = (n + 1023) / 1024, b0 = min(tid * per, n), b1 = min(b0 + per, n);
  int s = 0;
  for (int i = b0; i < b1; i++) s += cnt[i];
  part[tid] = s;
  __syncthreads();
  for (int o = 1; o < 1024; o <<= 1) {
    const int t = tid >= o ? part[tid - o] : 0;
    __syncthreads();
    part[tid] += t;
    __syncthreads();
  }
  int run = part[tid] - s;
  for (int i = b0; i < b1; i++) {
    off[i] = run;
    run += cnt[i];
  }
  if (tid == 1023) off[n] = part[1023];
}

__device__ __forceinline__ double setup_landmark(const Problem& P, const Lin& L, const Active& A, const Sys& S, int t,
                                                 uint8_t* level, uint8_t* lm_act2, double (*pd)[6] = nullptr,
                                                 int* pa = nullptr, int pe0 = 0) {
  const int g = t / kGroup, j = t % kGroup;
  const bool in = g < A.nL, point = g < P.nq;
  double hl[9] = {0, 0, 0, 0, 0, 0, 0, 0, 0}, bv[3] = {0, 0, 0}, chi = 0;
  int live = 0;
  if (in) {
    const int k1 = A.lm_off[g + 1];
    const double* Xg = P.X + 3 * g;
    for (int k = A.lm_off[g] + j; k < k1; k += kGroup) {
      bool lev = false;
      if (level && edge_outlier(P, L, k)) {
        lev = true;
        level[k] = 1;
// ... 4 lines not shown
      if (pd) pa[k - pe0] = pose_opt ? A.lm_pose[k] : -1;
      if (lev) {
        if (pose_opt) zero_pose_records<true>(L, k);
        if (pd)
#pragma unroll
          for (int i = 0; i < 6; i++) pd[k - pe0][i] = 0.0;
        continue;
      }
      const int te = P.etype[k];
      const SE3 T = load_T(P.T + 8 * P.epose[k]);
      const double* cm = P.cams + 5 * P.ecam[k];
      double er[4];
      const double chi2 = point_error(te, cm, obs_of(P, k, te), T, Xg, er);
#pragma unroll
      for (int q = 0; q < 4; q++) L.err[4 * k + q] = er[q];
      double cst = chi2;
      if (A.robust) {
        double r1;
        huber(chi2, pick4(P.delta, te), cst, r1);
      }
      chi += cst;
      double dg6[6] = {0, 0, 0, 0, 0, 0};
      point_edge_core<true>(P, L, A, k, te, pose_opt, T, cm, Xg, er, hl, bv, dg6);
      if (pd)
#pragma unroll
        for (int i = 0; i < 6; i++) pd[k - pe0][i] = dg6[i];
    }
  }
#pragma unroll
  for (int o = 1; o < kGroup; o <<= 1) live |= __shfl_xor(live, o);
  const bool act = level ? live != 0 : (in && A.lm_act[g] != 0);
  if (level && in && j == 0) lm_act2[g] = act ? 1 : 0;
  group_sum(hl);
  group_sum(bv);
  if (in && point && j == 0 && act) {
    double* H = S.Hll + 16 * g;
#pragma unroll
    for (int i = 0; i < 9; i++) H[i] = hl[i];
#pragma unroll
    for (int i = 9; i < 16; i++) H[i] = 0.0;
#pragma unroll
    for (int i = 0; i < 3; i++) S.bl[4 * g + i] = bv[i];
    S.bl[4 * g + 3] = 0.0;
    atomic_max_pos(S.out + 2, fmax(fabs(hl[0]), fmax(fabs(hl[4]), fabs(hl[8]))));
  }
  return chi;
}

__device__ __forceinline__ void prof_max(const Sys& S, int slot) {
  if (S.prof) atomicMax(S.prof + slot, (unsigned long long)wall_clock64());
}

__global__ __launch_bounds__(256) void setup_kernel(Problem P, Lin L, Active A, Sys S, int nbq, int nb_lm,
                                                    uint8_t* level, uint8_t* lm_act2, int* pp_cnt, int* pp_off,
                                                    double* pdg, int lm_iters, int gate, Lin Ls, Sys Ss) {
  __shared__ double red[4];
  __shared__ double part[4][64];
  __shared__ int last;
  if (gate >= 0) {
    const LmCtrl* c = S.lm + gate;
    if (!c->stop) return;
    if (c->cur) {
      bank_state(P);
      bank_lin(L, Ls, S, Ss);
    }
  }
  const int b = blockIdx.x;
  if (b == 0 && threadIdx.x == 0) prof_stamp(S, 9);
  if (b >= nb_lm) {
    const int c = (b - nb_lm) * 4 + (threadIdx.x >> 6);
    if (c < chunk_count(A)) pair_scan<false>(A, c, pp_cnt, nullptr, nullptr);
    if (threadIdx.x == 0) prof_max(S, kProfX + 4);
  } else if (b >= nbq) {
    double c = 0.0;
    lin_lines<kLinSetup>(P, L, A, S, b - nbq, true, nullptr, nullptr, 0.0, false, nullptr, level != nullptr, &c, pdg,
                         nb_lm, b);
    if (threadIdx.x == 0) __hip_atomic_store(S.partial + b, c, __ATOMIC_RELAXED, __HIP_MEMORY_SCOPE_AGENT);
    if (threadIdx.x == 0) prof_max(S, kProfX + 2);
  } else {
    __shared__ double pd[kPdCap][6];
    __shared__ int pa[kPdCap];
    const int g0 = min(b * (256 / kGroup), P.nq), g1 = min(b * (256 / kGroup) + 256 / kGroup, P.nq);
    const int e0 = A.lm_off[g0], e1 = A.lm_off[g1];
    const bool staged = e1 - e0 <= kPdCap;
    double acc[1] = {setup_landmark(P, L, A, S, b * 256 + threadIdx.x, level, lm_act2, staged ? pd : nullptr, pa, e0)};
    block_reduce<1>(acc, red);
    if (threadIdx.x == 0) __hip_atomic_store(S.partial + b, red[0], __ATOMIC_RELAXED, __HIP_MEMORY_SCOPE_AGENT);
    if (threadIdx.x == 0) prof_max(S, kProfX + 0);
    if (staged) {
      pose_diag_lds(A, pd, pa, e1 - e0, pdg, nb_lm, b);
    } else {
      asm volatile("s_waitcnt vmcnt(0)" ::: "memory");
      __syncthreads();
      pose_diag_range(P, L, A, pdg, nb_lm, b, e0, e1);
    }
    if (threadIdx.x == 0) prof_max(S, kProfX + 1);
  }
  asm volatile("s_waitcnt vmcnt(0)" ::: "memory");
  __syncthreads();
  if (threadIdx.x == 0) last = ticket(S.counter) == gridDim.x - 1;
  __syncthreads();
  if (!last) return;
  if (threadIdx.x == 0) prof_stamp(S, 10);
  double cs[1] = {0.0};
  for (int k = threadIdx.x; k < nb_lm; k += 256) cs[0] += __hip_atomic_load(S.partial + k, __ATOMIC_RELAXED, __HIP_MEMORY_SCOPE_AGENT);
  block_reduce<1>(cs, red);
  const double chi2 = red[0];
  if (pp_cnt) {
    __shared__ int sc[256];
    const int tid = threadIdx.x, nc = chunk_count(A);
    const int per = (nc + 255) / 256, b0 = min(tid * per, nc), b1 = min(b0 + per, nc);
    int sm = 0;
    for (int i = b0; i < b1; i++) sm += __hip_atomic_load(pp_cnt + i, __ATOMIC_RELAXED, __HIP_MEMORY_SCOPE_AGENT);
    sc[tid] = sm;
    __syncthreads();
    for (int o = 1; o < 256; o <<= 1) {
      const int t = tid >= o ? sc[tid - o] : 0;
      __syncthreads();
      sc[tid] += t;
      __syncthreads();
    }
    int run = sc[tid] - sm;
    for (int i = b0; i < b1; i++) {
      pp_off[i] = run;
// ... 29 lines not shown
  if (pt != 0) return;
#pragma unroll
  for (int o = 32; o >= 1; o >>= 1) mx = fmax(mx, __shfl_xor(mx, o));
  if (lane != 0) return;
  __hip_atomic_store(S.counter, 0u, __ATOMIC_RELAXED, __HIP_MEMORY_SCOPE_AGENT);
  prof_stamp(S, 12);
  const double md = fmax(__hip_atomic_load(S.out + 2, __ATOMIC_RELAXED, __HIP_MEMORY_SCOPE_AGENT), mx);
  S.out[0] = chi2;
  S.out[2] = md;
  LmCtrl* ctl = S.lm;
  ctl->lambda = 1e-5 * md;
  ctl->ni = 2;
  ctl->chi = chi2;
  ctl->cur = 0;
  ctl->it = 0;
  ctl->qmax = 0;
  ctl->stop = 0;
  ctl->iters = lm_iters;
  ctl->trials = 0;
}

__global__ __launch_bounds__(256) void landmark_active_kernel(Active A, const uint8_t* level, uint8_t* lm_act) {
  const int g = blockIdx.x * blockDim.x + threadIdx.x;
  if (g >= A.nL) return;
  uint8_t on = 0;
  for (int k = A.lm_off[g]; k < A.lm_off[g + 1]; k++) on |= level[(k)] == 0;
  lm_act[g] = on;
}

__device__ __forceinline__ bool edge_inlier(const Problem& P, const Lin& L, int e) {
  double chi2;
  bool depth_ok;
  edge_status(P, L, e, chi2, depth_ok);
  return chi2 <= pick4(P.th, P.etype[e]) && depth_ok;
}
__device__ __forceinline__ void classify_edge(const Problem& P, const Lin& L, int e, uint8_t* level, uint8_t* inlier,
                                              int final_pass) {
  if (final_pass) {
    inlier[e] = edge_inlier(P, L, e) ? 1 : 0;
    return;
  }
  double chi2;
  bool depth_ok;
  edge_status(P, L, e, chi2, depth_ok);
  if (chi2 > pick4(P.th, P.etype[e]) || !depth_ok) level[e] = 1;
}

__global__ __launch_bounds__(256) void classify_kernel(Problem P, Lin L, int E, uint8_t* level, uint8_t* inlier,
                                                       int final_pass) {
  const int e = blockIdx.x * blockDim.x + threadIdx.x;
  if (e < E) classify_edge(P, L, e, level, inlier, final_pass);
}

__global__ __launch_bounds__(256) void finish_kernel(Problem P, Lin L, int E, const int* gmap, uint8_t* inl, double* Th,
                                                     double* Xh, double* Lh, Sys S, unsigned long long seq) {
  __shared__ int last;
  if (S.lm) {
    const LmCtrl* c = S.lm + S.lm_slot;
    if (!c->stop) return;
    if (c->cur) bank_state(P);
  }
  const int i = blockIdx.x * blockDim.x + threadIdx.x;
  if (i < E) inl[gmap[i]] = edge_inlier(P, L, i) ? 1 : 0;
  if (i < 8 * P.np) Th[i] = P.T[i];
  if (i < 3 * P.nq) Xh[i] = P.X[i];
  if (i < 6 * P.nl) Lh[i] = P.L[i];
  __threadfence_system();
  __syncthreads();
  if (threadIdx.x == 0) {
    const unsigned tk = __hip_atomic_fetch_add(S.counter, 1u, __ATOMIC_ACQ_REL, __HIP_MEMORY_SCOPE_AGENT);
    last = tk == gridDim.x - 1;
  }
  __syncthreads();
  if (!last || threadIdx.x != 0) return;
  __hip_atomic_store(S.counter, 0u, __ATOMIC_RELAXED, __HIP_MEMORY_SCOPE_AGENT);
  __hip_atomic_store(&S.mail->seq, seq, __ATOMIC_RELEASE, __HIP_MEMORY_SCOPE_SYSTEM);
}

__global__ __launch_bounds__(256) void shard_fold_kernel(Sys S, double* red, int K, int npd, int rank, int nranks) {
  const int n6 = 6 * K;
  for (int q = threadIdx.x; q < n6; q += 256) {
    double acc = 0;
    if (npd > 0) {
      const int pa = q / 6, i = q - 6 * pa;
      const double* src = S.partial2 + (size_t)pa * npd * 6 + i;
      for (int b = 0; b < npd; b++) acc += src[(size_t)b * 6];
    }
    red[q] = acc;
  }
  for (int r = threadIdx.x; r < nranks; r += 256) red[n6 + r] = r == rank ? S.out[2] : 0.0;
}

__global__ void shard_post_kernel(Sys S, const double* red, int n6, int nranks, int mode, int add_pose_scale,
                                  unsigned long long seq) {
  __shared__ double mxs[64];
  const double* so = red + n6 + nranks;
  double mx = 0;
  if (mode == 0) {
    for (int q = threadIdx.x; q < n6; q += 64) mx = fmax(mx, fabs(red[q]));
    for (int r = threadIdx.x; r < nranks; r += 64) mx = fmax(mx, red[n6 + r]);
  }
  mxs[threadIdx.x] = mx;
  __syncthreads();
  if (threadIdx.x != 0) return;
  for (int k = 1; k < 64; k++) mx = fmax(mx, mxs[k]);
  const double chi2 = so[0], scale = so[1] + (add_pose_scale ? S.out[4] : 0.0), f = so[2] != 0.0 ? 1.0 : 0.0;
  if (mode == 0) S.out[2] = mx;
  S.out[0] = chi2;
  S.out[1] = scale;
  S.out[3] = f;
  post_mail(S.mail, chi2, scale, mode == 0 ? mx : S.out[2], f, seq);
}

__global__ __launch_bounds__(256) void shard_gather_kernel(Problem P, Lin L, int E, const int* gmap, int rank,
                                                           int nranks, double* G) {
  const int i = blockIdx.x * blockDim.x + threadIdx.x;
  const int nq3 = 3 * P.nq, nl6 = 6 * P.nl;
  if (i < E) {
    G[nq3 + nl6 + gmap[i]] = edge_inlier(P, L, i) ? 1.0 : 0.0;
  }
  if (i < nq3 && (i / 3) % nranks == rank) G[i] = P.X[i];
  if (i < nl6 && (P.nq + i / 6) % nranks == rank) G[nq3 + i] = P.L[i];
}

__global__ __launch_bounds__(256) void shard_finish_kernel(Problem P, int E, const double* G, uint8_t* inl,
                                                           double* Th, double* Xh, double* Lh, Sys S,
                                                           unsigned long long seq) {
  __shared__ int last;
  const int i = blockIdx.x * blockDim.x + threadIdx.x;
  const int nq3 = 3 * P.nq, nl6 = 6 * P.nl;
  if (i < E) inl[i] = G[nq3 + nl6 + i] != 0.0;
  if (i < 8 * P.np) Th[i] = P.T[i];
  if (i < nq3) Xh[i] = G[i];
  if (i < nl6) Lh[i] = G[nq3 + i];
  __threadfence_system();
  __syncthreads();
  if (threadIdx.x == 0) {
    const unsigned tk = __hip_atomic_fetch_add(S.counter, 1u, __ATOMIC_ACQ_REL, __HIP_MEMORY_SCOPE_AGENT);
    last = tk == gridDim.x - 1;
  }
  __syncthreads();
  if (!last || threadIdx.x != 0) return;
  __hip_atomic_store(S.counter, 0u, __ATOMIC_RELAXED, __HIP_MEMORY_SCOPE_AGENT);
  __hip_atomic_store(&S.mail->seq, seq, __ATOMIC_RELEASE, __HIP_MEMORY_SCOPE_SYSTEM);
}

int shard_red_len(int K, int nranks) { return 6 * K + nranks + 3; }

hipError_t linearize(const Problem& P, const Lin& L, const Active& A, const Sys& S, bool with_maxdiag,
                     hipStream_t s) {
  const int nbq = (P.nq * kGroup + 255) / 256, nbl = A.n_lblk;
  if (nbq + nbl > 0)
    hipLaunchKernelGGL(linearize_kernel, dim3(nbq + nbl), dim3(256), 0, s, P, L, A, S, nbq, with_maxdiag ? 1 : 0);
  if (with_maxdiag && A.K > 0 && A.Ea > 0)
    hipLaunchKernelGGL(pose_diag_kernel, dim3((A.Ea + 255) / 256), dim3(256), 0, s, P, L, A, S);
  return hipGetLastError();
}

int setup_pdg_len(const Active& A) {
  const int nbq = A.nL > 0 ? (A.nL * kGroup + 255) / 256 : 0;
  return 6 * A.K * (nbq + A.n_lblk) + 6;
}

hipError_t setup_dev(const Problem& P, const Lin& L, const Active& A, Sys& S, uint8_t* level, uint8_t* lm_act2,
                     int lm_iters, int* pp_cnt, int* pp_off, int4* pp, double* pdg, hipStream_t s, int gate,
                     const Lin* Ls, const Sys* Ss) {
  if (gate >= 0 && (!Ls || !Ss || pp_cnt)) return hipErrorInvalidValue;
  if (!S.lm || lm_iters <= 0) return hipErrorInvalidValue;
  Active A0 = A;
  A0.elevel = nullptr;
  const int nc = chunk_count(A);
  if (nc == 0) pp_cnt = nullptr;
  const int nbq = A.nL > 0 ? (A.nL * kGroup + 255) / 256 : 0, nb = nbq + A.n_lblk;
  const int nbp = pp_cnt ? (nc + 3) / 4 : 0;
  hipLaunchKernelGGL(setup_kernel, dim3(std::max(nb + nbp, 1)), dim3(256), 0, s, P, L, A0, S, nbq, nb, level, lm_act2,
                     pp_cnt, pp_off, pdg, lm_iters, gate, Ls ? *Ls : L, Ss ? *Ss : S);
  if (pp_cnt) hipLaunchKernelGGL(pair_fill_kernel, dim3(nc), dim3(64), 0, s, A, pp_off, pp);
  return hipGetLastError();
}

hipError_t post(Sys& S, unsigned long long seq, hipStream_t s, const Active* A) {
  const int npd = (A && A->K > 0 && A->Ea > 0) ? (A->Ea + 255) / 256 : 0;
  hipLaunchKernelGGL(post_kernel, dim3(1), dim3(256), 0, s, S, A ? A->K : 0, npd, seq);
  return hipGetLastError();
}

hipError_t finish(const Problem& P, const Lin& L, int E, const int* gmap, uint8_t* inl, double* Th, double* Xh,
                  double* Lh, Sys& S, unsigned long long seq, hipStream_t s) {
  const int n = std::max(std::max(E, 8 * P.np), std::max(3 * P.nq, 6 * P.nl));
  hipLaunchKernelGGL(finish_kernel, dim3(std::max((n + 255) / 256, 1)), dim3(256), 0, s, P, L, E, gmap, inl, Th, Xh,
                     Lh, S, seq);
  return hipGetLastError();
}

hipError_t build_pairs(const Active& A, int* pp_cnt, int* pp_off, int4* pp, hipStream_t s) {
  const int nc = chunk_count(A);
  if (nc == 0) return hipSuccess;
  hipLaunchKernelGGL(pair_count_kernel, dim3(nc), dim3(64), 0, s, A, pp_cnt);
  hipLaunchKernelGGL(pair_offsets_kernel, dim3(1), dim3(1024), 0, s, pp_cnt, pp_off, nc);
  hipLaunchKernelGGL(pair_fill_kernel, dim3(nc), dim3(64), 0, s, A, pp_off, pp);
  return hipGetLastError();
}

hipError_t landmark_active(const Active& A, const uint8_t* level, uint8_t* lm_act, hipStream_t s) {
  if (A.nL > 0) hipLaunchKernelGGL(landmark_active_kernel, dim3((A.nL + 255) / 256), dim3(256), 0, s, A, level, lm_act);
  return hipGetLastError();
}

hipError_t classify(const Problem& P, const Lin& L, int E, uint8_t* level, uint8_t* inlier, int final_pass,
                    hipStream_t s) {
  if (E > 0) hipLaunchKernelGGL(classify_kernel, dim3((E + 255) / 256), dim3(256), 0, s, P, L, E, level, inlier,
                                final_pass);
  return hipGetLastError();
}

hipError_t shard_fold(const Active& A, Sys& S, double* red, int rank, int nranks, hipStream_t s) {
  const int npd = (A.K > 0 && A.Ea > 0) ? (A.Ea + 255) / 256 : 0;
  hipLaunchKernelGGL(shard_fold_kernel, dim3(1), dim3(256), 0, s, S, red, A.K, npd, rank, nranks);
  return hipGetLastError();
}

hipError_t shard_post(Sys& S, const double* red, int n6, int nranks, int mode, int add_pose_scale,
                      unsigned long long seq, hipStream_t s) {
  hipLaunchKernelGGL(shard_post_kernel, dim3(1), dim3(64), 0, s, S, red, n6, nranks, mode, add_pose_scale, seq);
  return hipGetLastError();
}

hipError_t shard_gather(const Problem& P, const Lin& L, int E, const int* gmap, int rank, int nranks, double* G,
                        hipStream_t s) {
  const int n = std::max(E, std::max(3 * P.nq, 6 * P.nl));
  if (n > 0)
    hipLaunchKernelGGL(shard_gather_kernel, dim3((n + 255) / 256), dim3(256), 0, s, P, L, E, gmap, rank, nranks, G);
  return hipGetLastError();
}

hipError_t shard_finish(const Problem& P, int E_global, const double* G, uint8_t* inl, double* Th, double* Xh,
                        double* Lh, Sys& S, unsigned long long seq, hipStream_t s) {
  const int n = std::max(std::max(E_global, 8 * P.np), std::max(3 * P.nq, 6 * P.nl));
  hipLaunchKernelGGL(shard_finish_kernel, dim3(std::max((n + 255) / 256, 1)), dim3(256), 0, s, P, E_global, G, inl,
                     Th, Xh, Lh, S, seq);
  return hipGetLastError();
}

// ... 3 lines not shown
```

### rspl-slam_amd/csrc/ba_kernels.hpp

```cpp
#pragma once
#include <hip/hip_runtime.h>

#include <cstdint>

namespace rspl {
namespace ba {

struct Problem {
  const double* cams;
  double* T;
  double* X;
  double* L;
  double* Tn;
  double* Xn;
  double* Ln;
  int np, nq, nl;
  int ncam;
  const int8_t* etype;
  const int* epose;
  const int* elm;
  const int* ecam;
  const double* eobs;
  int Ep;
  double delta[4];
// ... 108 lines not shown
struct Mail {
  double v[4];
  unsigned long long seq;
  unsigned long long vseq;
  unsigned long long pad[2];
};

struct LmCtrl {
  double lambda, ni, chi;
  int cur;
  int it;
  int qmax;
  int stop;
  int iters;
  int trials;
};

struct Sys {
  double* Hll;
  double* bl;
  double* bp;
  double* S;
  double* x;
  double* chunk;
  double* pairfin;
  unsigned* pair_ctr;
  unsigned* solve_ctr;
  double* partial;
  double* partial2;
  double* out;
  int* fail;
  unsigned* counter;
  unsigned* lm_ctr;
  Mail* mail;
  double* shard_out;
  int pose_scale;
  unsigned long long* prof;
  LmCtrl* lm;
  double* lm_trace;
  int lm_slot;
  int lm_post;
};
constexpr int kProfPc = 16, kProfUe = kProfPc + 4 * 4096, kProfX = kProfUe + 4 * 4096, kProfLen = kProfX + 8;

constexpr int kLmChunk = 256;
constexpr int kLineBlk = 8;

hipError_t compute_errors(const Problem& P, const Lin& L, const Active& A, Sys& S, unsigned long long seq,
                          hipStream_t s);
hipError_t linearize(const Problem& P, const Lin& L, const Active& A, const Sys& S, bool with_maxdiag,
                     hipStream_t s);
hipError_t post(Sys& S, unsigned long long seq, hipStream_t s, const Active* A = nullptr);
hipError_t setup_dev(const Problem& P, const Lin& L, const Active& A, Sys& S, uint8_t* level, uint8_t* lm_act2,
                     int lm_iters, int* pp_cnt, int* pp_off, int4* pp, double* pdg, hipStream_t s, int gate = -1,
                     const Lin* Ls = nullptr, const Sys* Ss = nullptr);
int setup_pdg_len(const Active& A);
struct Spec {
  Lin Ls;
  Sys Ss;
};
hipError_t trial_host_large(const Problem& P, const Lin& L, const Active& A, Sys& S, double lambda,
                            unsigned long long seq, hipStream_t s);
hipError_t trial_dev(const Problem& P, const Lin& L, const Active& A, Sys& S, unsigned long long seq, hipStream_t s,
                     const Spec& spec, hipEvent_t* ev = nullptr);
hipError_t build_pairs(const Active& A, int* pp_cnt, int* pp_off, int4* pp, hipStream_t s);
hipError_t landmark_active(const Active& A, const uint8_t* level, uint8_t* lm_act, hipStream_t s);
hipError_t classify(const Problem& P, const Lin& L, int E, uint8_t* level, uint8_t* inlier, int final_pass,
                    hipStream_t s);
hipError_t finish(const Problem& P, const Lin& L, int E, const int* gmap, uint8_t* inl, double* Th, double* Xh,
                  double* Lh, Sys& S, unsigned long long seq, hipStream_t s);
hipError_t trial_chunks(const Problem& P, const Lin& L, const Active& A, Sys& S, double lambda, hipStream_t s);
hipError_t trial_solve(const Problem& P, const Lin& L, const Active& A, Sys& S, double lambda, hipStream_t s);
hipError_t shard_fold(const Active& A, Sys& S, double* red, int rank, int nranks, hipStream_t s);
hipError_t shard_post(Sys& S, const double* red, int n6, int nranks, int mode, int add_pose_scale,
                      unsigned long long seq, hipStream_t s);
hipError_t shard_gather(const Problem& P, const Lin& L, int E, const int* gmap, int rank, int nranks, double* G,
                        hipStream_t s);
hipError_t shard_finish(const Problem& P, int E_global, const double* G, uint8_t* inl, double* Th, double* Xh,
                        double* Lh, Sys& S, unsigned long long seq, hipStream_t s);
int shard_red_len(int K, int nranks);
bool fast_path(int K);
bool wave_path(int K);
int update_blocks(const Problem& P);
int errors_blocks(int Ea);
int update_errors_blocks(const Active& A);
void set_update_geometry(Active& A);

}
}
```

### rspl-slam_amd/csrc/ba_stage.cpp

```cpp
#include "ba_stage.hpp"

#include <algorithm>

namespace rspl {
namespace ba {

namespace {

constexpr int kParWorkers = 3;

template <typename F>
void pool_run(HostPool* pool, F& f) {
  pool->run([](void* c, int q) { (*static_cast<F*>(c))(q); }, &f);
}

struct Edges {
  const int32_t* pose[4];
  const int32_t* lm[4];
  const int32_t* cam[4];
  const double* obs[4];
  int ne[4], base[5];
  explicit Edges(const rspl_ba_problem* pr) {
    const int32_t* p[4] = {pr->mono_pose, pr->stereo_pose, pr->mono_line_pose, pr->stereo_line_pose};
    const int32_t* l[4] = {pr->mono_point, pr->stereo_point, pr->mono_line_line, pr->stereo_line_line};
// ... 81 lines not shown
      rstart_[0] = 0;
      for (int q = 0; q < NP; q++) {
        int tot = 0;
        for (int c : pcnt_[q]) tot += c;
        rstart_[q + 1] = rstart_[q] + tot;
        for (int p = 0; p < np; p++) pact[p] |= ppact_[q][p];
      }
      E = Eg;
      Ep = ed.ne[0] + ed.ne[1];
      return RSPL_OK;
    }
    NP_ = 1;
  }
  lm_cnt_.assign(nL + 1, 0);
  int* cnt = lm_cnt_.data();
  for (int t = 0; t < 4; t++) {
    const int n = ed.ne[t], lmax = t < 2 ? nq : nl, loff = t < 2 ? 0 : nq;
    const int32_t *pt = ed.pose[t], *lt = ed.lm[t], *ct = ed.cam[t];
    bool bad = false;
    for (int i = 0; i < n; i++) {
      const unsigned p = (unsigned)pt[i], l = (unsigned)lt[i];
      bad |= (p >= (unsigned)np) | (l >= (unsigned)lmax);
    }
    if (ct)
      for (int i = 0; i < n; i++) bad |= (unsigned)ct[i] >= (unsigned)pr->n_cameras;
    if (bad)
      for (int i = 0; i < n; i++) {
        const int p = pt[i], l = lt[i], c = ct ? ct[i] : 0;
        RSPL_CHECK_ARG(p >= 0 && p < np && l >= 0 && l < lmax && c >= 0 && c < pr->n_cameras,
                       "edge %d of type %d references a missing vertex/camera", i, t);
      }
    for (int i = 0; i < n; i++) pact[pt[i]] = 1;
    if (!sharded) {
      for (int i = 0; i < n; i++) cnt[loff + lt[i] + 1]++;
      E += n;
      Ep += t < 2 ? n : 0;
    } else {
      for (int i = 0; i < n; i++)
        if ((loff + lt[i]) % nranks == rank) {
          cnt[loff + lt[i] + 1]++;
          E++;
          Ep += t < 2;
        }
    }
  }
  return RSPL_OK;
}

void Stager::place(const rspl_ba_problem* pr, const Out& o) {
  const Edges ed(pr);
  const int nq = pr->n_points, nL = nq + pr->n_lines;
  int* lm_off = o.lm_off;
  int* gmap = o.gmap;
  const int* pidx = o.pidx;
  const int Ep_ = Ep;
  double* lobs = o.eobs + 4 * (size_t)Ep_;
  auto gather = [&](int k0, int k1) {
    const int e1 = ed.base[1], e2 = ed.base[2], e3 = ed.base[3];
    static const double zero = 0.0;
    for (int k = k0; k < std::min(k1, Ep_); k++) {
      const int eg = gmap[k];
      const bool st = eg >= e1;
      const int i = st ? eg - e1 : eg;
      const int32_t* pt = st ? ed.pose[1] : ed.pose[0];
      const int32_t* ct = st ? ed.cam[1] : ed.cam[0];
      const int p = pt[i];
      o.etype[k] = (int8_t)st;
      o.epose[k] = p;
      o.elm[k] = (st ? ed.lm[1] : ed.lm[0])[i];
      o.ecam[k] = ct ? ct[i] : 0;
      o.lpose[k] = pidx[p];
      const double* ob = st ? ed.obs[1] + 3 * (size_t)i : ed.obs[0] + 2 * (size_t)i;
      double* ov = o.eobs + 4 * (size_t)k;
      ov[0] = ob[0];
      ov[1] = ob[1];
      ov[2] = *(st ? ob + 2 : &zero);
    }
    for (int k = std::max(k0, Ep_); k < k1; k++) {
      const int eg = gmap[k];
      const int t = eg >= e3 ? 3 : 2;
      const int i = eg - (t == 3 ? e3 : e2);
      const int p = ed.pose[t][i];
      o.etype[k] = (int8_t)t;
      o.epose[k] = p;
      o.elm[k] = nq + ed.lm[t][i];
      o.ecam[k] = ed.cam[t] ? ed.cam[t][i] : 0;
      o.lpose[k] = pidx[p];
      const int D = t == 3 ? 8 : 4;
      const double* ob = ed.obs[t] + (size_t)D * i;
      double* ov = lobs + 8 * (size_t)(k - Ep_);
      for (int q = 0; q < D; q++) ov[q] = ob[q];
    }
  };
  if (par_) {
    const int NP = NP_;
    auto place_range = [&](int q) {
      const int g0 = gcut_[q], g1 = gcut_[q + 1];
      int* c = pcnt_[q].data();
      int run = rstart_[q];
      for (int g = g0; g < g1; g++) {
        lm_off[g] = run;
        const int n = c[g - g0];
        c[g - g0] = run;
        run += n;
      }
      if (q == NP - 1) lm_off[nL] = run;
      for (int p = 0; p < NP; p++)
        for (const int2& e : bkt_[(size_t)p * NP + q]) gmap[c[e.y - g0]++] = e.x;
      gather(rstart_[q], rstart_[q + 1]);
    };
    pool_run(pool_.get(), place_range);
    return;
  }
  lm_off[0] = 0;
  for (int g = 0; g < nL; g++) lm_off[g + 1] = lm_off[g] + lm_cnt_[g + 1];
  int* fill = lm_cnt_.data();
  for (int g = 0; g < nL; g++) fill[g] = lm_off[g];
  for (int t = 0; t < 4; t++) {
    const int n = ed.ne[t], loff = t < 2 ? 0 : nq;
    const int32_t* lt = ed.lm[t];
    if (!sh_) {
      for (int i = 0; i < n; i++) gmap[fill[loff + lt[i]]++] = ed.base[t] + i;
    } else {
      for (int i = 0; i < n; i++)
        if ((loff + lt[i]) % nranks_ == rank_) gmap[fill[loff + lt[i]]++] = ed.base[t] + i;
    }
  }
  gather(0, E);
}

}
}
```

### rspl-slam_amd/csrc/ba_stage.hpp

```cpp
#pragma once

#include <memory>
#include <vector>

#include "common.hpp"
#include "host_pool.hpp"

namespace rspl {
namespace ba {

struct Stager {
  int count(const rspl_ba_problem* pr, bool sharded, int rank, int nranks, int par_edges);
  struct Out {
    int* lm_off;
    int8_t* etype;
    int* epose;
    int* elm;
    int* ecam;
    int* gmap;
    int* lpose;
    double* eobs;
    const int* pidx;
  };
  void place(const rspl_ba_problem* pr, const Out& o);

  int E = 0, Ep = 0;
  std::vector<uint8_t> pose_has_edge;

 private:
  bool sh_ = false, par_ = false;
  int rank_ = 0, nranks_ = 1, NP_ = 1;
  std::vector<int> lm_cnt_;
  std::unique_ptr<HostPool> pool_;
  std::vector<std::vector<int2>> bkt_;
  std::vector<std::vector<int>> pcnt_;
  std::vector<std::vector<uint8_t>> ppact_;
  std::vector<int> pcut_, gcut_, rstart_;
};

}
}
```

### rspl-slam_amd/csrc/common.hpp

```cpp
#pragma once

#include <hip/hip_runtime.h>

#include <cstdarg>
#include <cstdint>
#include <cstdio>
#include <string>
#include <vector>

#include "../../include/rspl.h"

namespace rspl {

void set_error(const char* fmt, ...);
int cu_mask(int reserve_cus, bool reserved_only, std::vector<uint32_t>& mask);

#define RSPL_HIP(expr)                                                                   \
  do {                                                                                   \
    hipError_t _e = (expr);                                                              \
    if (_e != hipSuccess) {                                                              \
      ::rspl::set_error("%s:%d %s: %s", __FILE__, __LINE__, #expr, hipGetErrorString(_e)); \
      return RSPL_E_DEVICE;                                                              \
    }                                                                                    \
  } while (0)
// ... 29 lines not shown
    return reinterpret_cast<T*>(base + off);
  }
  void release() {
    if (base) (void)hipFree(base);
    base = nullptr;
  }
};

struct PinnedArena {
  char *base = nullptr, *dev = nullptr;
  size_t size = 0, used = 0;
  int reserve(size_t bytes) {
    size = bytes;
    used = 0;
    if (hipHostMalloc((void**)&base, bytes, hipHostMallocMapped | hipHostMallocCoherent) != hipSuccess) {
      set_error("hipHostMalloc(%zu) failed", bytes);
      base = nullptr;
      return RSPL_E_DEVICE;
    }
    if (hipHostGetDevicePointer((void**)&dev, base, 0) != hipSuccess) {
      set_error("hipHostGetDevicePointer failed");
      release();
      return RSPL_E_DEVICE;
    }
    return RSPL_OK;
  }
  template <typename T, typename D>
  T* take(size_t count, D** dev_out) {
    size_t off = al256(used);
    used = off + count * sizeof(T);
    if (used > size) return nullptr;
    *dev_out = reinterpret_cast<T*>(dev + off);
    return reinterpret_cast<T*>(base + off);
  }
  void release() {
    if (base) (void)hipHostFree(base);
    base = dev = nullptr;
  }
};

struct Sizer {
  size_t used = 0;
  template <typename T>
  T* take(size_t count) {
    used = al256(used) + count * sizeof(T);
    return nullptr;
  }
  template <typename T, typename D>
  T* take(size_t count, D**) {
    return take<T>(count);
  }
};

struct StageTimer {
  static constexpr int kRing = 64, kMax = 8;
  int n = 0;
  bool enabled = false;
  hipEvent_t ev[kRing][kMax + 1] = {};
  bool pending[kRing] = {};
  int head = 0;
  double acc[kMax] = {};
  long calls = 0;
  int init(int nstages) {
    n = nstages;
    for (int r = 0; r < kRing; r++)
      for (int i = 0; i <= n; i++)
        if (hipEventCreate(&ev[r][i]) != hipSuccess) return RSPL_E_DEVICE;
    return RSPL_OK;
  }
  void destroy() {
    for (int r = 0; r < kRing; r++)
      for (int i = 0; i <= n; i++)
        if (ev[r][i]) (void)hipEventDestroy(ev[r][i]);
  }
  void mark(int i, hipStream_t s) {
    if (enabled) (void)hipEventRecord(ev[head][i], s);
  }
  hipEvent_t slot(int i) const { return enabled ? ev[head][i] : nullptr; }
  void harvest(int r) {
    if (!pending[r]) return;
    (void)hipEventSynchronize(ev[r][n]);
    for (int i = 0; i < n; i++) {
      float ms = 0.f;
      (void)hipEventElapsedTime(&ms, ev[r][i], ev[r][i + 1]);
      acc[i] += ms;
    }
    pending[r] = false;
    calls++;
  }
  void end_call() {
    if (!enabled) return;
    pending[head] = true;
    head = (head + 1) % kRing;
    harvest(head);
  }
  void reset(bool on) {
    for (int r = 0; r < kRing; r++) pending[r] = false;
    for (double& a : acc) a = 0;
    calls = 0;
    head = 0;
    enabled = on;
  }
  int query(float* ms, int* ncalls) {
    for (int k = 0; k < kRing; k++) harvest((head + k) % kRing);
    for (int i = 0; i < n; i++) ms[i] = (float)acc[i];
    if (ncalls) *ncalls = (int)calls;
    return RSPL_OK;
  }
};

struct Tensor {
  std::string name;
  std::vector<int64_t> dims;
  std::vector<float> data;
};
int load_blob(const char* path, std::vector<Tensor>& out);

hipError_t upload_mapped(void* dst, const void* src_mapped, size_t bytes, hipStream_t s);
const Tensor* find(const std::vector<Tensor>& ts, const std::string& name, int64_t numel);

}
```

### rspl-slam_amd/csrc/copy_kernels.hip

```cpp
#include <hip/hip_runtime.h>

#include <algorithm>
#include <cstdint>

#include "common.hpp"

namespace rspl {

__global__ __launch_bounds__(256) void upload_kernel(uint4* dst, const uint4* src, size_t n16, uint8_t* dtail,
                                                     const uint8_t* stail, int ntail) {
  const size_t t = (size_t)blockIdx.x * 256 + threadIdx.x;
  for (size_t i = t; i < n16; i += (size_t)gridDim.x * 256) dst[i] = src[i];
  if (t < (size_t)ntail) dtail[t] = stail[t];
}

hipError_t upload_mapped(void* dst, const void* src_mapped, size_t bytes, hipStream_t s) {
  const size_t n16 = bytes / 16;
  const int ntail = (int)(bytes - 16 * n16);
  if (!bytes) return hipSuccess;
  const unsigned blocks = (unsigned)std::max<size_t>(1, std::min<size_t>((n16 + 255) / 256, 1024));
  hipLaunchKernelGGL(upload_kernel, dim3(blocks), dim3(256), 0, s, static_cast<uint4*>(dst),
                     static_cast<const uint4*>(src_mapped), n16, static_cast<uint8_t*>(dst) + 16 * n16,
                     static_cast<const uint8_t*>(src_mapped) + 16 * n16, ntail);
  return hipGetLastError();
}

}
```

### rspl-slam_amd/csrc/lines.cpp

```cpp
#include <algorithm>
#include <chrono>
#include <condition_variable>
#include <mutex>
#include <string>
#include <thread>
#include <array>
#include <cmath>
#include <cstring>
#include <numeric>
#include <set>
#include <type_traits>
#include <unordered_map>
#include <vector>

#include "common.hpp"
#include "fld_kernels.hpp"
#include "line_kernels.hpp"

#pragma clang fp contract(off)

using namespace rspl;

namespace {

// ... 832 lines not shown
    h->a_img = image;
    h->a_H = H;
    h->a_W = W;
    h->a_stride = stride;
    h->a_cfg = *cfg;
    h->a_merge = do_merge;
    h->a_dev = false;
    h->job = true;
    h->done = false;
  }
  ensure_worker(h);
  h->cv.notify_all();
  return RSPL_OK;
}

extern "C" int rspl_lines_extract_wait(rspl_lines* h, double* lines, int capacity, int* n_out, double* job_us) {
  RSPL_CHECK_ARG(h && n_out && (capacity == 0 || lines) && capacity >= 0, "rspl_lines_extract_wait: bad argument");
  std::unique_lock<std::mutex> lk(h->mu);
  RSPL_CHECK_ARG(h->job, "rspl_lines_extract_wait: no job submitted");
  h->cv.wait(lk, [h] { return h->done; });
  h->job = false;
  *n_out = h->a_n;
  if (job_us) *job_us = h->a_us;
  if (h->a_rc != RSPL_OK) {
    set_error("%s", h->a_err.c_str());
    return h->a_rc;
  }
  if (h->a_n > capacity) {
    set_error("%d lines exceed capacity %d", h->a_n, capacity);
    return RSPL_E_CAPACITY;
  }
  if (h->a_n) memcpy(lines, h->a_lines.data(), sizeof(double) * 4 * h->a_n);
  return RSPL_OK;
}

extern "C" int rspl_lines_extract_wait_device(rspl_lines* h, double* d_lines, int capacity, int* n_out,
                                              double* job_us, void* stream) {
  RSPL_CHECK_ARG(h && n_out && (capacity == 0 || d_lines) && capacity >= 0,
                 "rspl_lines_extract_wait_device: bad argument");
  constexpr int S = rspl_lines::kPinSlots;
  if (h->pin_cap < capacity) {
    for (int k = 0; k < S; k++) {
      if (h->copy_pending[k]) RSPL_HIP(hipEventSynchronize(h->copy_ev[k]));
      h->copy_pending[k] = false;
      if (h->pin_lines[k]) (void)hipHostFree(h->pin_lines[k]);
      h->pin_lines[k] = nullptr;
    }
    h->pin_cap = 0;
    for (int k = 0; k < S; k++)
      RSPL_HIP(hipHostMalloc((void**)&h->pin_lines[k], sizeof(double) * 4 * capacity, hipHostMallocDefault));
    h->pin_cap = capacity;
  }
  const int k = h->pin_next;
  if (!h->copy_ev[k]) RSPL_HIP(hipEventCreateWithFlags(&h->copy_ev[k], hipEventDisableTiming));
  if (h->copy_pending[k]) {
    RSPL_HIP(hipEventSynchronize(h->copy_ev[k]));
    h->copy_pending[k] = false;
  }
  int rc = rspl_lines_extract_wait(h, h->pin_lines[k], capacity, n_out, job_us);
  if (rc != RSPL_OK) return rc;
  if (*n_out) {
    RSPL_HIP(hipMemcpyAsync(d_lines, h->pin_lines[k], sizeof(double) * 4 * *n_out, hipMemcpyHostToDevice,
                            (hipStream_t)stream));
    RSPL_HIP(hipEventRecord(h->copy_ev[k], (hipStream_t)stream));
    h->copy_pending[k] = true;
    h->pin_next = (k + 1) % S;
  }
  return RSPL_OK;
}

namespace {

int fld_check_cfg(const rspl_fld_config* cfg) {
  RSPL_CHECK_ARG(cfg, "NULL rspl_fld_config");
  RSPL_CHECK_ARG(cfg->canny_aperture_size == 3, "canny_aperture_size %d: only 3 (the configs' value)",
                 cfg->canny_aperture_size);
  RSPL_CHECK_ARG(cfg->length_threshold >= 1 && cfg->length_threshold < fld::kMaxEdge && cfg->distance_threshold >= 0,
                 "bad FLD thresholds");
  return RSPL_OK;
}

int fld_check_half(int hh, int hw) {
  RSPL_CHECK_ARG(hh >= 2 && hw >= 2 && hh < 65536 && hw < 65536, "half image %dx%d outside [2, 65535]", hw, hh);
  RSPL_CHECK_ARG(fld::mask_fits(hh, hw),
                 "half image %dx%d: its two bitmasks (rows * ceil(width / 32) * 8 = %lld bytes) exceed the %d-byte LDS "
                 "budget", hw, hh, (long long)hh * fld::words_per_row(hw) * 8, fld::kMaskLdsBytes);
  return RSPL_OK;
}

int fld_check_images(int batch, int H, int W, size_t stride, size_t pitch, const rspl_fld_config* cfg) {
  RSPL_CHECK_ARG(batch >= 1 && batch <= fld::kMaxBatch, "batch %d outside [1, %d]", batch, fld::kMaxBatch);
  RSPL_CHECK_ARG(H >= 4 && W >= 4 && H % 2 == 0 && W % 2 == 0, "image %dx%d: even sizes >= 4 required", W, H);
  RSPL_CHECK_ARG(stride >= (size_t)W && stride <= (size_t)INT32_MAX, "stride %zu below the width %d (or beyond int)",
                 stride, W);
  RSPL_CHECK_ARG(pitch >= stride * (size_t)(H - 1) + (size_t)W, "pitch %zu below one %dx%d image of stride %zu", pitch, W,
                 H, stride);
  if (int rc = fld_check_half(H / 2, W / 2)) return rc;
  return fld_check_cfg(cfg);
}

int fld_reserve(rspl_lines* h, size_t hp) {
  constexpr size_t B = fld::kMaxBatch, E = fld::kMaxEdge, S = fld::kMaxSeg;
  if (!h->fld_arena.base) {
    const size_t words = fld::kMaskLdsBytes / 8;
    const size_t bytes = B * (words * 4 + E * 4 * 5 + 4 + E * 12 + S * 8 + S * 16 + fld::kMetaInts * 4) +
                         rspl_lines::kDevSegCap * 16 + B * 4 + 16 * 256;
    if (int rc = h->fld_arena.reserve(bytes)) return rc;
    Arena& ar = h->fld_arena;
    fld::Args& a = h->fld;
    a.ebits = ar.take<uint32_t>(B * words);
    a.pix = ar.take<int>(B * E);
    a.lab = ar.take<int>(B * E);
    a.spix = ar.take<int>(B * E);
    a.cstart = ar.take<int>(B * (E + 1));
    a.pts = ar.take<uint32_t>(B * E);
    a.chains = ar.take<int>(B * E * 3);
    a.skey = ar.take<unsigned long long>(B * S);
    a.sseg = ar.take<float>(B * S * 4);
    a.meta = ar.take<int>(B * fld::kMetaInts);
    h->dev_seg = ar.take<float>((size_t)rspl_lines::kDevSegCap * 4);
    h->dev_cnt = ar.take<int32_t>(B);
    if (!h->dev_cnt) {
      h->fld_arena.release();
      set_error("detector scratch carving failed");
      return RSPL_E_DEVICE;
    }
    for (hipEvent_t& e : h->fld_ev) RSPL_HIP(hipEventCreate(&e));
  }
  if (hp > h->fld_hp) {
    if (h->fld_img) {
      RSPL_HIP(hipDeviceSynchronize());
      (void)hipFree(h->fld_img);
      h->fld_img = nullptr;
      h->fld_hp = 0;
    }
    RSPL_HIP(hipMalloc((void**)&h->fld_img, B * 2 * hp));
    h->fld_hp = hp;
  }
  return RSPL_OK;
}

void fld_shape(rspl_lines* h, int hh, int hw, const rspl_fld_config* cfg) {
  fld::Args& a = h->fld;
  a.hh = hh;
  a.hw = hw;
  a.half = h->fld_img;
  a.cls = h->fld_img + (size_t)fld::kMaxBatch * hh * hw;
  a.len_thr = cfg ? cfg->length_threshold : 1;
  a.dist_thr = cfg ? cfg->distance_threshold : 0.0;
  a.out = nullptr;
  a.capacity = 0;
  a.counts = h->dev_cnt;
}

int fld_clear_meta(rspl_lines* h, int B, hipStream_t st) {
  h->fld_batch = B;
  RSPL_HIP(hipMemsetAsync(h->fld.meta, 0, sizeof(int) * fld::kMetaInts * B, st));
  return RSPL_OK;
}

}

extern "C" int rspl_lines_detect_device(rspl_lines* h, const uint8_t* d_images, int batch, int H, int W, size_t stride,
                                        size_t pitch, const rspl_fld_config* cfg, float* d_segments, int capacity,
                                        int32_t* d_counts, void* stream) {
  if (int rc = fld_check_images(batch, H, W, stride, pitch, cfg)) return rc;
  RSPL_CHECK_ARG(capacity >= 0 && (capacity == 0 || d_segments), "capacity %d without a segment buffer", capacity);
  RSPL_CHECK_ARG(h && d_images && d_counts, "rspl_lines_detect_device: NULL argument");
  const int hh = H / 2, hw = W / 2;
  const size_t hp = (size_t)hh * hw;
  if (int rc = fld_reserve(h, hp)) return rc;
  hipStream_t st = stream ? (hipStream_t)stream : h->stream;
  fld_shape(h, hh, hw, cfg);
  fld::Args a = h->fld;
  a.out = d_segments;
  a.capacity = capacity;
  a.counts = d_counts;
  const bool prof = h->fld_profile;
  if (int rc = fld_clear_meta(h, batch, st)) return rc;
  if (prof) RSPL_HIP(hipEventRecord(h->fld_ev[0], st));
// ... 165 lines not shown
                              if (!fld::finish_segment(half, hh, hw, lt, x1, y1, x2, y2, o)) return;
                              if (n < capacity) memcpy(segments + 4 * (size_t)n, o, sizeof(o));
                              n++;
                            });
    }
  *n_out = n;
  if (n > capacity) {
    set_error("%d segments exceed capacity %d", n, capacity);
    return RSPL_E_CAPACITY;
  }
  return RSPL_OK;
}

namespace {

void extract_job_device(rspl_lines* h) {
  int rc = RSPL_OK;
  h->a_n = 0;
  if (hipEventSynchronize(h->dev_done) != hipSuccess) {
    set_error("rspl_lines_extract_async_device: the detector's stream failed");
    rc = RSPL_E_DEVICE;
  }
  const int32_t* pin = h->dev_pin;
  const int status = pin[fld::kStatus], n = pin[fld::kMetaInts];
  if (rc == RSPL_OK && (status || n > rspl_lines::kDevSegCap)) {
    set_error("device detector status %d, %d segments (1: more than %d edge pixels, 2: more than %d segments, 4: "
              "internal bound)", status, n, fld::kMaxEdge, rspl_lines::kDevSegCap);
    rc = RSPL_E_CAPACITY;
  }
  if (rc == RSPL_OK) {
    h->a_lines.resize((size_t)std::max(n, 1) * 4);
    rc = rspl_line_extract((const float*)(pin + fld::kMetaInts + 1), n, h->a_merge, h->a_lines.data(), std::max(n, 1),
                           &h->a_n);
  }
  h->a_rc = rc;
  h->a_err = rc == RSPL_OK ? std::string() : std::string(rspl_last_error());
  h->a_us = std::chrono::duration<double, std::micro>(std::chrono::steady_clock::now() - h->a_t0).count();
}

}

extern "C" int rspl_lines_extract_async_device(rspl_lines* h, const uint8_t* d_image, int H, int W, size_t stride,
                                               const rspl_fld_config* cfg, int do_merge, void* stream) {
  if (int rc = fld_check_images(1, H, W, stride, stride * (size_t)(H > 0 ? H : 0), cfg)) return rc;
  RSPL_CHECK_ARG(h && d_image, "rspl_lines_extract_async_device: NULL argument");
  {
    std::lock_guard<std::mutex> lk(h->mu);
    RSPL_CHECK_ARG(!h->job, "rspl_lines_extract_async_device: the previous job has not been waited for");
  }
  const auto t0 = std::chrono::steady_clock::now();
  constexpr size_t kPinBytes = sizeof(int32_t) * (fld::kMetaInts + 1) + sizeof(float) * 4 * rspl_lines::kDevSegCap;
  if (!h->dev_pin) {
    RSPL_HIP(hipHostMalloc((void**)&h->dev_pin, kPinBytes, hipHostMallocDefault));
    RSPL_HIP(hipEventCreateWithFlags(&h->dev_in, hipEventDisableTiming));
    RSPL_HIP(hipEventCreateWithFlags(&h->dev_done, hipEventDisableTiming));
  }
  if (int rc = fld_reserve(h, (size_t)(H / 2) * (W / 2))) return rc;
  RSPL_HIP(hipEventRecord(h->dev_in, (hipStream_t)stream));
  RSPL_HIP(hipStreamWaitEvent(h->stream, h->dev_in, 0));
  if (int rc = rspl_lines_detect_device(h, d_image, 1, H, W, stride, stride * (size_t)H, cfg, h->dev_seg,
                                        rspl_lines::kDevSegCap, h->dev_cnt, h->stream))
    return rc;
  RSPL_HIP(hipMemcpyAsync(h->dev_pin, h->fld.meta, sizeof(int32_t) * fld::kMetaInts, hipMemcpyDeviceToHost, h->stream));
  RSPL_HIP(hipMemcpyAsync(h->dev_pin + fld::kMetaInts, h->dev_cnt, sizeof(int32_t), hipMemcpyDeviceToHost, h->stream));
  RSPL_HIP(hipMemcpyAsync(h->dev_pin + fld::kMetaInts + 1, h->dev_seg, sizeof(float) * 4 * rspl_lines::kDevSegCap,
                          hipMemcpyDeviceToHost, h->stream));
  RSPL_HIP(hipEventRecord(h->dev_done, h->stream));
  {
    std::lock_guard<std::mutex> lk(h->mu);
    h->a_merge = do_merge;
    h->a_dev = true;
    h->a_t0 = t0;
    h->job = true;
    h->done = false;
  }
  ensure_worker(h);
  h->cv.notify_all();
  return RSPL_OK;
}
```

### rspl-slam_amd/csrc/runtime.cpp

```cpp
#include <vector>

#include "common.hpp"

using namespace rspl;

struct rspl_timer {
  hipEvent_t ev[2] = {nullptr, nullptr};
};

namespace rspl {
int cu_mask(int reserve_cus, bool reserved_only, std::vector<uint32_t>& mask) {
  int dev = 0, ncu = 0;
  RSPL_HIP(hipGetDevice(&dev));
  RSPL_HIP(hipDeviceGetAttribute(&ncu, hipDeviceAttributeMultiprocessorCount, dev));
  RSPL_CHECK_ARG(reserve_cus > 0 && reserve_cus < ncu, "cannot reserve %d of %d CUs", reserve_cus, ncu);
  mask.assign((ncu + 31) / 32, 0u);
  const int step = ncu / reserve_cus;
  int left = reserve_cus;
  for (int c = 0; c < ncu; c++) {
    const bool reserved = left > 0 && c % step == step - 1;
    if (reserved) left--;
    if (reserved == reserved_only) mask[c / 32] |= 1u << (c % 32);
  }
  return RSPL_OK;
}
}

extern "C" {

int rspl_device_count(int* count) {
  RSPL_CHECK_ARG(count, "NULL count");
  RSPL_HIP(hipGetDeviceCount(count));
  return RSPL_OK;
}
int rspl_set_device(int device) {
  RSPL_HIP(hipSetDevice(device));
  return RSPL_OK;
}
int rspl_malloc(void** ptr, size_t bytes) {
  RSPL_CHECK_ARG(ptr, "NULL ptr");
  RSPL_HIP(hipMalloc(ptr, bytes ? bytes : 1));
  return RSPL_OK;
}
int rspl_free(void* ptr) {
  RSPL_HIP(hipFree(ptr));
  return RSPL_OK;
}
int rspl_memcpy_h2d(void* dst, const void* src, size_t bytes, void* stream) {
  if (!bytes) return RSPL_OK;
  RSPL_HIP(hipMemcpyAsync(dst, src, bytes, hipMemcpyHostToDevice, (hipStream_t)stream));
  RSPL_HIP(hipStreamSynchronize((hipStream_t)stream));
  return RSPL_OK;
}
int rspl_memcpy_d2h(void* dst, const void* src, size_t bytes, void* stream) {
  if (!bytes) return RSPL_OK;
  RSPL_HIP(hipMemcpyAsync(dst, src, bytes, hipMemcpyDeviceToHost, (hipStream_t)stream));
  RSPL_HIP(hipStreamSynchronize((hipStream_t)stream));
  return RSPL_OK;
}
int rspl_memset(void* dst, int value, size_t bytes, void* stream) {
  RSPL_HIP(hipMemsetAsync(dst, value, bytes, (hipStream_t)stream));
  return RSPL_OK;
}
int rspl_memcpy_d2d(void* dst, const void* src, size_t bytes, void* stream) {
  if (!bytes) return RSPL_OK;
  RSPL_HIP(hipMemcpyAsync(dst, src, bytes, hipMemcpyDeviceToDevice, (hipStream_t)stream));
  return RSPL_OK;
}
int rspl_stream_create(void** stream) {
  RSPL_CHECK_ARG(stream, "NULL stream");
  RSPL_HIP(hipStreamCreateWithFlags((hipStream_t*)stream, hipStreamNonBlocking));
  return RSPL_OK;
}
int rspl_stream_create_priority(void** stream, int high) {
  RSPL_CHECK_ARG(stream, "NULL stream");
  int lo = 0, hi = 0;
  RSPL_HIP(hipDeviceGetStreamPriorityRange(&lo, &hi));
  RSPL_HIP(hipStreamCreateWithPriority((hipStream_t*)stream, hipStreamNonBlocking, high ? hi : lo));
  return RSPL_OK;
}

int rspl_stream_create_reserving(void** stream, int reserve_cus) {
  RSPL_CHECK_ARG(stream && reserve_cus >= 0, "rspl_stream_create_reserving: bad arguments");
  if (reserve_cus == 0) {
    RSPL_HIP(hipStreamCreateWithFlags((hipStream_t*)stream, hipStreamNonBlocking));
    return RSPL_OK;
  }
  std::vector<uint32_t> mask;
  int rc = rspl::cu_mask(reserve_cus, false, mask);
  if (rc) return rc;
  RSPL_HIP(hipExtStreamCreateWithCUMask((hipStream_t*)stream, (uint32_t)mask.size(), mask.data()));
  return RSPL_OK;
}
int rspl_stream_destroy(void* stream) {
  RSPL_HIP(hipStreamDestroy((hipStream_t)stream));
  return RSPL_OK;
}
int rspl_stream_synchronize(void* stream) {
  RSPL_HIP(hipStreamSynchronize((hipStream_t)stream));
  return RSPL_OK;
}
int rspl_event_create(void** event) {
  RSPL_CHECK_ARG(event, "NULL event");
  RSPL_HIP(hipEventCreateWithFlags((hipEvent_t*)event, hipEventDisableTiming));
  return RSPL_OK;
}
int rspl_event_record(void* event, void* stream) {
  RSPL_HIP(hipEventRecord((hipEvent_t)event, (hipStream_t)stream));
  return RSPL_OK;
}
int rspl_stream_wait_event(void* stream, void* event) {
  RSPL_HIP(hipStreamWaitEvent((hipStream_t)stream, (hipEvent_t)event, 0));
  return RSPL_OK;
}
int rspl_event_destroy(void* event) {
  RSPL_HIP(hipEventDestroy((hipEvent_t)event));
  return RSPL_OK;
}
int rspl_device_synchronize(void) {
  RSPL_HIP(hipDeviceSynchronize());
  return RSPL_OK;
}
int rspl_timer_create(rspl_timer** t) {
  RSPL_CHECK_ARG(t, "NULL timer");
  auto* x = new rspl_timer();
  if (hipEventCreate(&x->ev[0]) != hipSuccess || hipEventCreate(&x->ev[1]) != hipSuccess) {
    set_error("hipEventCreate failed");
    delete x;
    return RSPL_E_DEVICE;
  }
  *t = x;
  return RSPL_OK;
}
int rspl_timer_record(rspl_timer* t, int which, void* stream) {
  RSPL_CHECK_ARG(t && (which == 0 || which == 1), "bad timer / which");
  RSPL_HIP(hipEventRecord(t->ev[which], (hipStream_t)stream));
  return RSPL_OK;
}
int rspl_timer_elapsed_ms(rspl_timer* t, float* ms) {
  RSPL_CHECK_ARG(t && ms, "bad timer");
  RSPL_HIP(hipEventSynchronize(t->ev[1]));
  RSPL_HIP(hipEventElapsedTime(ms, t->ev[0], t->ev[1]));
  return RSPL_OK;
}
void rspl_timer_destroy(rspl_timer* t) {
  if (!t) return;
  for (auto& e : t->ev)
    if (e) (void)hipEventDestroy(e);
  delete t;
}

}
```

### rspl-slam_amd/csrc/sg.cpp

```cpp
#include <algorithm>
#include <cmath>
#include <cstdlib>
#include <cstring>
#include <string>
#include <vector>

#include "common.hpp"
#include "sg_kernels.hpp"

using namespace rspl;

namespace {
constexpr int kLayers = 18;
constexpr int kKencIn = 16;
const int kKencCh[6] = {3, 32, 64, 128, 256, 256};
}

struct rspl_sg {
  rspl_sg_config cfg{};
  hipStream_t stream = nullptr;
  Arena arena;
  int nmax = 0, B = 0, ld = 0;
  float* kw[5];
  float* kb[5];
// ... 258 lines not shown
  sk.nmax = s->nmax; sk.iters = iters;
  sk.sleep = 1;
  return sg::sinkhorn(sk, s->sink, B, st, t0, t1);
}

extern "C" int rspl_sg_create(const rspl_sg_config* cfg, const char* weights_path, rspl_sg** out) {
  RSPL_CHECK_ARG(cfg && out, "rspl_sg_create: NULL argument");
  RSPL_CHECK_ARG(cfg->max_keypoints > 0 && cfg->max_keypoints <= 4096, "max_keypoints must be in [1, 4096]");
  RSPL_CHECK_ARG(cfg->precision == RSPL_PREC_FP32 || cfg->precision == RSPL_PREC_FP16,
                 "precision must be RSPL_PREC_FP32 or RSPL_PREC_FP16");
  RSPL_CHECK_ARG(cfg->image_width > 0 && cfg->image_height > 0, "image size must be positive");
  RSPL_CHECK_ARG(cfg->sinkhorn_iterations < 4096, "sinkhorn_iterations must be < 4096");
  *out = nullptr;
  std::vector<Tensor> ts;
  int rc = load_blob(weights_path, ts);
  if (rc) return rc;
  RSPL_HIP(hipSetDevice(cfg->device));
  auto* s = new rspl_sg();
  s->cfg = *cfg;
  if (s->cfg.max_batch < 1) s->cfg.max_batch = 1;
  if (s->cfg.sinkhorn_iterations <= 0) s->cfg.sinkhorn_iterations = 100;
  s->B = s->cfg.max_batch;
  s->nmax = cfg->max_keypoints;
  s->ld = s->nmax + 1;
  s->ldv = (s->nmax + 31) / 32 * 32;
  {
    int ncu = 0;
    if (hipDeviceGetAttribute(&ncu, hipDeviceAttributeMultiprocessorCount, cfg->device) != hipSuccess || ncu < 1) {
      set_error("hipDeviceGetAttribute(MultiprocessorCount) failed");
      delete s;
      return RSPL_E_DEVICE;
    }
    if (int prc = plan_sinkhorn(s->nmax, s->B, ncu, &s->sink)) {
      delete s;
      return prc;
    }
  }
  Sizer sz;
  carve(sz, s);
  if ((rc = s->arena.reserve(sz.used))) { delete s; return rc; }
  carve(s->arena, s);
  if (hipMemset(s->ug, 0, sizeof(unsigned long long) * s->sink.ug_granules) != hipSuccess ||
      hipMemset(s->vg, 0, sizeof(unsigned long long) * s->sink.vg_granules) != hipSuccess ||
      hipMemset(s->Kf[0], 0, sizeof(_Float16) * s->B * 2 * 256 * s->ldv) != hipSuccess ||
      hipMemset(s->Kf[1], 0, sizeof(_Float16) * s->B * 2 * 256 * s->ldv) != hipSuccess ||
      hipMemset(s->Vf[0], 0, sizeof(_Float16) * s->B * 2 * 256 * s->ldv) != hipSuccess ||
      hipMemset(s->Vf[1], 0, sizeof(_Float16) * s->B * 2 * 256 * s->ldv) != hipSuccess) {
    set_error("sinkhorn exchange buffer init failed");
    rspl_sg_destroy(s);
    return RSPL_E_DEVICE;
  }
  const size_t nm = s->nmax;
  if (s->timer.init(RSPL_SG_STAGES) != RSPL_OK || hipStreamCreateWithFlags(&s->stream, hipStreamNonBlocking) != hipSuccess ||
      hipEventCreateWithFlags(&s->ev_ready, hipEventDisableTiming) != hipSuccess ||
      hipEventCreateWithFlags(&s->ev_sink[0], hipEventDisableTiming) != hipSuccess ||
      hipEventCreateWithFlags(&s->ev_sink[1], hipEventDisableTiming) != hipSuccess ||
      hipEventCreateWithFlags(&s->ev_done, hipEventDisableTiming) != hipSuccess ||
      hipHostMalloc(&s->h_f, sizeof(double) * nm * 259 * 2) != hipSuccess ||
      hipHostMalloc(&s->h_idx, sizeof(int32_t) * nm * 2 + 16) != hipSuccess ||
      hipHostMalloc(&s->h_ms, sizeof(double) * nm * 2) != hipSuccess ||
      hipHostMalloc(&s->err, sizeof(unsigned) * s->B, hipHostMallocMapped) != hipSuccess ||
      hipHostGetDevicePointer((void**)&s->d_err, s->err, 0) != hipSuccess) {
    set_error("stream / pinned allocation failed");
    rspl_sg_destroy(s);
    return RSPL_E_DEVICE;
  }
  memset(s->err, 0, sizeof(unsigned) * s->B);
  if ((rc = upload_weights(s, ts))) { rspl_sg_destroy(s); return rc; }
  {
    bool okh = true;
    for (int i = 0; i < 5; i++)
      okh &= sg::to_half_t(s->kw[i], i == 0 ? kKencIn : kKencCh[i], kKencCh[i + 1], s->hkw[i], s->stream) == hipSuccess;
    for (int l = 0; l < kLayers; l++) {
      okh &= sg::to_half_t(s->wqkv + (size_t)l * 256 * 768, 256, 768, s->hwqkv + (size_t)l * 256 * 768, s->stream) ==
             hipSuccess;
      okh &= sg::to_half_t(s->w1m + (size_t)l * 512 * 512, 512, 512, s->hw1 + (size_t)l * 512 * 512, s->stream) ==
             hipSuccess;
      okh &= sg::to_half_t(s->w2 + (size_t)l * 512 * 256, 512, 256, s->hw2 + (size_t)l * 512 * 256, s->stream) ==
             hipSuccess;
      okh &= sg::to_frag(s->hwqkv + (size_t)l * 256 * 768, 768, 256, s->fwqkv + (size_t)l * 256 * 768, s->stream) ==
             hipSuccess;
      okh &= sg::to_frag(s->hw1 + (size_t)l * 512 * 512, 512, 512, s->fw1 + (size_t)l * 512 * 512, s->stream) ==
             hipSuccess;
      okh &= sg::to_frag(s->hw2 + (size_t)l * 512 * 256, 256, 512, s->fw2 + (size_t)l * 512 * 256, s->stream) ==
             hipSuccess;
    }
    okh &= sg::to_half_t(s->wf, 256, 256, s->hwf, s->stream) == hipSuccess;
    okh &= hipStreamSynchronize(s->stream) == hipSuccess;
    if (!okh) {
      set_error("fp16 weight conversion failed");
      rspl_sg_destroy(s);
      return RSPL_E_DEVICE;
    }
  }
  *out = s;
  return RSPL_OK;
}

extern "C" void rspl_sg_destroy(rspl_sg* s) {
  if (!s) return;
  rspl_fm_destroy(s->fm);

  if (s->stream) (void)hipStreamSynchronize(s->stream);
  s->arena.release();
  s->timer.destroy();
  if (s->h_f) (void)hipHostFree(s->h_f);
  if (s->h_idx) (void)hipHostFree(s->h_idx);
  if (s->h_ms) (void)hipHostFree(s->h_ms);
  if (s->err) (void)hipHostFree(s->err);
  if (s->ev_ready) (void)hipEventDestroy(s->ev_ready);
// ... 361 lines not shown
```

Before: 1031.

## Precompute BA pair offsets on host, add inverse edge map, relax event fences

Several unrelated changes land together. BA pair-list offsets are now computed on the host during staging, and an inverse edge map (ginv) is uploaded so the device pair build and the finish scatter need fewer passes. Events get release-to-device or no-system-fence flags to cut synchronisation cost, and local device-to-device memcpy is routed through a custom vectorised copy kernel. Debug entry points for pairs and final state are also added. The trade-off is extra host staging work and possible ordering risk from the relaxed event fences.

```diff
diff --git a/include/rspl.h b/include/rspl.h
--- a/include/rspl.h
+++ b/include/rspl.h
@@ -239,6 +239,11 @@
                              rspl_ba_chunk_plan* out);
 int rspl_ba_debug_chunk_geometry(int n_landmarks, int n_poses, int max_landmarks, int max_poses, int32_t* chunks,
                                  int32_t* order);
+int rspl_ba_debug_pair_offsets(const rspl_ba_problem* problem, int max_landmarks, int max_poses, int32_t* pp_off,
+                               int cap, int* n_chunks);
+int rspl_ba_debug_pairs(rspl_ba* ba, int rebuild, int32_t* pp_off, int cap_off, int32_t* pp, long long cap_pairs,
+                        int* n_chunks, long long* n_pairs, int* fused);
+int rspl_ba_debug_final(rspl_ba* ba, uint8_t* inlier, double* T_dev, double* T_out, double* X, double* L);
 
 typedef int (*rspl_allreduce_fn)(void* ctx, double* d_buf, size_t count, void* stream);
 int rspl_ba_set_shard(rspl_ba* ba, int rank, int nranks, rspl_allreduce_fn allreduce, void* ctx);
diff --git a/rspl-slam_amd/api.py b/rspl-slam_amd/api.py
--- a/rspl-slam_amd/api.py
+++ b/rspl-slam_amd/api.py
@@ -328,6 +328,29 @@
         capi.check(self._lib.rspl_ba_trace(self._h, buf, cap, C.byref(n)), "rspl_ba_trace")
         a = np.frombuffer(buf, np.float64, n.value * capi.BA_TRACE_W).reshape(n.value, capi.BA_TRACE_W)
         return [dict(zip(capi.BA_TRACE_FIELDS, map(float, row))) for row in a]
+
+    def debug_pairs(self, rebuild=False):
+        cap_off, cap = 1 << 16, 1 << 20
+        while True:
+            off, pp = np.zeros(cap_off, np.int32), np.zeros((cap, 4), np.int32)
+            nc, n, fused = C.c_int(), C.c_longlong(), C.c_int()
+            rc = self._lib.rspl_ba_debug_pairs(self._h, 1 if rebuild else 0, off.ctypes.data, cap_off, pp.ctypes.data,
+                                               cap, C.byref(nc), C.byref(n), C.byref(fused))
+            if rc and (nc.value + 1 > cap_off or n.value > cap) and cap < 1 << 26:
+                cap_off, cap = max(cap_off, nc.value + 1), max(cap, int(n.value))
+                continue
+            capi.check(rc, "rspl_ba_debug_pairs")
+            return off[:nc.value + 1].copy(), pp[:n.value].copy(), bool(fused.value)
+
+    def debug_final(self, problem):
+        E = sum(problem.n_edges(k) for k in ("mono", "stereo", "mono_line", "stereo_line"))
+        npo, nq, nl = problem.pose_q.shape[0], problem.points.shape[0], problem.lines.shape[0]
+        inl = np.full(max(E, 1), 255, np.uint8)
+        Td, To = np.zeros((max(npo, 1), 8)), np.zeros((max(npo, 1), 8))
+        X, L = np.zeros((max(nq, 1), 3)), np.zeros((max(nl, 1), 6))
+        capi.check(self._lib.rspl_ba_debug_final(self._h, inl.ctypes.data, Td.ctypes.data, To.ctypes.data, X.ctypes.data,
+                                                 L.ctypes.data), "rspl_ba_debug_final")
+        return {"inlier": inl[:E], "T_dev": Td[:npo], "T_out": To[:npo], "points": X[:nq], "lines": L[:nl]}
 
     def use_reserved_cus(self, reserve_cus: int):
         capi.check(self._lib.rspl_ba_use_reserved_cus(self._h, reserve_cus), "rspl_ba_use_reserved_cus")
diff --git a/rspl-slam_amd/capi.py b/rspl-slam_amd/capi.py
--- a/rspl-slam_amd/capi.py
+++ b/rspl-slam_amd/capi.py
@@ -35,6 +35,7 @@
     "rspl_ba_create", "rspl_ba_local", "rspl_ba_submit", "rspl_ba_join", "rspl_ba_destroy", "rspl_ba_use_reserved_cus", "rspl_ba_kernel_timing",
     "rspl_ba_kernel_times", "rspl_ba_trace", "rspl_ba_set_line_jacobian", "rspl_ba_debug_stage",
     "rspl_ba_debug_chunk_plan", "rspl_ba_debug_chunk_geometry",
+    "rspl_ba_debug_pair_offsets", "rspl_ba_debug_pairs", "rspl_ba_debug_final",
     "rspl_frame_create", "rspl_frame_optimize", "rspl_frame_destroy",
     "rspl_ba_set_shard", "rspl_comm_unique_id", "rspl_comm_create", "rspl_comm_allreduce_sum", "rspl_comm_destroy",
     "rspl_ba_set_comm", "rspl_group_create", "rspl_group_destroy", "rspl_ba_set_group",
@@ -302,6 +303,11 @@
     if hasattr(lib, "rspl_ba_debug_chunk_plan"):
         lib.rspl_ba_debug_chunk_plan.argtypes = [ip, ip, ip, ip, C.POINTER(BaChunkPlan)]
         lib.rspl_ba_debug_chunk_geometry.argtypes = [ip, ip, ip, ip, vp, vp]
+    if hasattr(lib, "rspl_ba_debug_pair_offsets"):
+        lib.rspl_ba_debug_pair_offsets.argtypes = [vp, ip, ip, vp, ip, C.POINTER(ip)]
+        lib.rspl_ba_debug_pairs.argtypes = [vp, ip, vp, ip, vp, C.c_longlong, C.POINTER(ip), C.POINTER(C.c_longlong),
+                                            C.POINTER(ip)]
+        lib.rspl_ba_debug_final.argtypes = [vp, vp, vp, vp, vp, vp]
     if hasattr(lib, "rspl_ba_trace"):
         lib.rspl_ba_trace.argtypes = [vp, C.POINTER(C.c_double), ip, C.POINTER(ip)]
         lib.rspl_ba_set_line_jacobian.argtypes = [vp, ip]
diff --git a/rspl-slam_amd/csrc/ba.cpp b/rspl-slam_amd/csrc/ba.cpp
--- a/rspl-slam_amd/csrc/ba.cpp
+++ b/rspl-slam_amd/csrc/ba.cpp
@@ -103,6 +103,15 @@
   long long trace_n = 0;
   unsigned grew = 0;
   int line_jac = 0;
+  struct Last {
+    bool valid = false, fused = false;
+    rspl::ba::Problem P{};
+    rspl::ba::Lin L{};
+    rspl::ba::Active A{};
+    int E = 0;
+    const int* gmap = nullptr;
+    const double* T_out = nullptr;
+  } last;
 };
 
 namespace {
@@ -123,10 +132,10 @@
 
 
 struct CallLayout {
-  size_t cams, T, X, L, obs, type, pose, lm, cam, gmap, lm_pose, pidx, lm_off, lm_act, pairs, ltab, level, flags, out,
-      bytes;
+  size_t cams, T, X, L, obs, type, pose, lm, cam, gmap, ginv, lm_pose, pidx, lm_off, lm_act, pairs, ltab, pp_off, level,
+      flags, out, bytes;
   CallLayout() = default;
-  CallLayout(int ncam, int np, int nq, int nl, int E, size_t nobs) {
+  CallLayout(int ncam, int np, int nq, int nl, int E, size_t nobs, size_t nchunks) {
     const size_t nL = (size_t)nq + nl;
     size_t so = 0;
     auto place = [&](size_t n) {
@@ -137,11 +146,13 @@
     cams = place(sizeof(double) * 5 * ncam); T = place(sizeof(double) * 8 * np); X = place(sizeof(double) * 3 * nq);
     L = place(sizeof(double) * 6 * nl); obs = place(sizeof(double) * nobs); type = place(E);
     pose = place(4 * (size_t)E); lm = place(4 * (size_t)E); cam = place(4 * (size_t)E); gmap = place(4 * (size_t)E);
+    ginv = place(4 * (size_t)E);
     lm_pose = place(4 * (size_t)E);
     pidx = place(4 * (size_t)np); lm_off = place(4 * (nL + 1)); lm_act = place(nL);
     pairs = place(8 * (size_t)np * (np + 1) / 2);
     const size_t line_edges = nobs >= 4 * (size_t)E ? (nobs - 4 * (size_t)E) / 4 : 0;
     ltab = place(16 * ((size_t)nl + line_edges / ba::kLineBlk + 2));
+    pp_off = place(4 * (nchunks + 1));
     level = place(E); flags = place(4 * sizeof(int)); out = place(8 * sizeof(double));
     bytes = so;
   }
@@ -193,6 +204,7 @@
   std::string msg;
   int E = 0, Ep = 0, K = 0, n_lblk = 0;
   size_t pair_bound = 0;
+  bool pp_staged = false;
   CallLayout cl;
   DownLayout dl;
   HostMarks tm;
@@ -333,7 +345,7 @@
           us(u0, last(ba::kProfUe, nbu, nue, 1)), us(u0, last(ba::kProfUe, nbu, nue, 2)),
           us(u0, last(ba::kProfUe, nbu, nue, 3)), us(h[1], h[5]), us(h[5], h[6]), us(h[6], h[7]), us(h[7], h[8]));
   fprintf(stderr,
-          "ba_prof setup us: landmarks %.1f +pdiag %.1f lines %.1f +pdiag %.1f pairs %.1f | blocks done %.1f scan %.1f "
+          "ba_prof setup us: landmarks %.1f +pdiag %.1f lines %.1f +pdiag %.1f pair fill %.1f | blocks done %.1f cost %.1f "
           "pose diagonals + control %.1f\n",
           us(h[9], h[ba::kProfX]), us(h[9], h[ba::kProfX + 1]), us(h[9], h[ba::kProfX + 2]),
           us(h[9], h[ba::kProfX + 3]), us(h[9], h[ba::kProfX + 4]), us(h[9], h[10]),
@@ -424,7 +436,7 @@
   bool on = false;
   ba::Lin L{};
   int E = 0;
-  const int* gmap = nullptr;
+  const int* ginv = nullptr;
   uint8_t* inl = nullptr;
   double *Th = nullptr, *Xh = nullptr, *Lh = nullptr;
   unsigned long long q = 0;
@@ -435,6 +447,7 @@
 struct DevLmArgs {
   uint8_t* cls_level = nullptr;
   bool build_pp = false;
+  bool pp_staged = false;
   SpecFinish* fin = nullptr;
   SpecSetup* nxt = nullptr;
   bool setup_done = false;
@@ -461,7 +474,8 @@
     ba::Sys Su = S;
     Su.prof = b->prof && !b->prof_nb[0] && !cls_level ? b->prof : nullptr;
     RSPL_HIP(ba::setup_dev(P, Lr, A, Su, cls_level, cls_level ? const_cast<uint8_t*>(A.lm_act) : nullptr, iters,
-                           d.build_pp ? b->pp_cnt : nullptr, b->pp_off, b->pp_buf, b->pdg, st));
+                           d.build_pp ? b->pp_buf : nullptr, d.build_pp && !d.pp_staged ? b->pp_cnt : nullptr,
+                           b->pp_off, b->pdg, st));
   }
   unsigned long long q = b->seq;
   const unsigned long long q_first = b->seq + 1;
@@ -482,7 +496,7 @@
         if ((size_t)3 * (b->kev_used + 1) > b->kev.size()) {
           for (int i = 0; i < 3; i++) {
             hipEvent_t e;
-            RSPL_HIP(hipEventCreate(&e));
+            RSPL_HIP(hipEventCreateWithFlags(&e, kTimingEventFlags));
             b->kev.push_back(e);
           }
           b->grew |= 8;
@@ -511,7 +525,7 @@
       Sf.prof = nullptr;
       fin->q = ++b->seq;
       fin->on = true;
-      RSPL_HIP(ba::finish(P, fin->L, fin->E, fin->gmap, fin->inl, fin->Th, fin->Xh, fin->Lh, Sf, fin->q, st));
+      RSPL_HIP(ba::finish(P, fin->L, fin->E, fin->ginv, fin->inl, fin->Th, fin->Xh, fin->Lh, Sf, fin->q, st));
     }
     return RSPL_OK;
   };
@@ -525,7 +539,7 @@
     S2.prof = nullptr;
     S2.lm_trace = nullptr;
     RSPL_HIP(ba::setup_dev(P, Lr, nxt->A2, S2, nxt->level, const_cast<uint8_t*>(nxt->A2.lm_act), nxt->iters2,
-                           nullptr, b->pp_off, b->pp_buf, b->pdg, st, queued & 1, &Ls, &Ss));
+                           nullptr, nullptr, nullptr, b->pdg, st, queued & 1, &Ls, &Ss));
     nxt->queued = true;
     nxt->extra = false;
     return RSPL_OK;
@@ -686,7 +700,8 @@
   int prio_lo = 0, prio_hi = 0;
   (void)hipDeviceGetStreamPriorityRange(&prio_lo, &prio_hi);
   {
-    const size_t cbytes = CallLayout(kMaxCams, b->maxK, cfg->max_points, cfg->max_lines, b->maxE, 8 * (size_t)b->maxE).bytes;
+    const size_t cbytes = CallLayout(kMaxCams, b->maxK, cfg->max_points, cfg->max_lines, b->maxE, 8 * (size_t)b->maxE,
+                                     b->chunk_slots).bytes;
     const char* what = nullptr;
     hipError_t e = hipSuccess;
     auto step = [&](hipError_t r, const char* w) {
@@ -713,7 +728,7 @@
   memset(b->mail, 0, sizeof(ba::Mail));
   {
     const size_t sb = std::max(CallLayout(kMaxCams, b->maxK, cfg->max_points, cfg->max_lines, b->maxE,
-                                          8 * (size_t)b->maxE).bytes,
+                                          8 * (size_t)b->maxE, b->chunk_slots).bytes,
                                DownLayout(b->maxK, cfg->max_points, cfg->max_lines, b->maxE).bytes);
     ba::Active Amax{};
     Amax.nL = b->maxL;
@@ -808,7 +823,8 @@
 
 namespace {
 int ba_local_impl(rspl_ba* b, const rspl_ba_problem* pr, rspl_ba_result* res);
-int stage_call(rspl_ba* b, int slot, const rspl_ba_problem* pr, rspl_ba_result* res, ba::StagedCall& c);
+int stage_call(rspl_ba* b, int slot, const rspl_ba_problem* pr, rspl_ba_result* res, ba::StagedCall& c,
+               bool off_chain);
 int run_call(rspl_ba* b, const ba::StagedCall& c, const rspl_ba_problem* pr, rspl_ba_result* res, double* tr);
 void push_trace(rspl_ba* b, const double* tr);
 
@@ -842,7 +858,7 @@
   RSPL_CHECK_ARG(!queue_active(b), "rspl_ba_kernel_timing: calls are queued on the tracking thread (rspl_ba_join first)");
   for (size_t n = b->kev.size(); every > 0 && n < 3 * (size_t)kEventTrials; n++) {
     hipEvent_t e;
-    RSPL_HIP(hipEventCreate(&e));
+    RSPL_HIP(hipEventCreateWithFlags(&e, kTimingEventFlags));
     b->kev.push_back(e);
   }
   b->ktime_every = every;
@@ -854,6 +870,60 @@
   RSPL_CHECK_ARG(b && (analytic == 0 || analytic == 1), "rspl_ba_set_line_jacobian: NULL handle or mode not 0 / 1");
   RSPL_CHECK_ARG(!queue_active(b), "rspl_ba_set_line_jacobian: calls are queued on the tracking thread (rspl_ba_join first)");
   b->line_jac = analytic;
+  return RSPL_OK;
+}
+
+extern "C" int rspl_ba_debug_pairs(rspl_ba* b, int rebuild, int32_t* pp_off, int cap_off, int32_t* pp, long long cap_pairs,
+                                   int* n_chunks, long long* n_pairs, int* fused) {
+  RSPL_CHECK_ARG(b && pp_off && pp && n_chunks && n_pairs, "rspl_ba_debug_pairs: NULL argument");
+  RSPL_CHECK_ARG(!queue_active(b), "rspl_ba_debug_pairs: calls are queued on the tracking thread (rspl_ba_join first)");
+  RSPL_CHECK_ARG(b->last.valid, "rspl_ba_debug_pairs: no completed unsharded call");
+  ba::Active A = b->last.A;
+  const int nc = ba::chunk_count(A);
+  *n_chunks = nc;
+  *n_pairs = 0;
+  if (fused) *fused = b->last.fused;
+  RSPL_CHECK_ARG(cap_off >= nc + 1, "rspl_ba_debug_pairs: %d offsets, room for %d", nc + 1, cap_off);
+  RSPL_HIP(hipStreamSynchronize(b->stream));
+  if (rebuild) {
+    A.pp_off = b->pp_off;
+    RSPL_HIP(ba::build_pairs(A, b->pp_cnt, b->pp_off, b->pp_buf, b->stream));
+    RSPL_HIP(hipStreamSynchronize(b->stream));
+  }
+  pp_off[0] = 0;
+  if (nc == 0) return RSPL_OK;
+  RSPL_HIP(hipMemcpy(pp_off, A.pp_off, sizeof(int) * (nc + 1), hipMemcpyDeviceToHost));
+  *n_pairs = pp_off[nc];
+  RSPL_CHECK_ARG(pp_off[nc] >= 0 && (size_t)pp_off[nc] <= b->pp_cap && *n_pairs <= cap_pairs,
+                 "rspl_ba_debug_pairs: %d pairs, list capacity %zu, room for %lld", pp_off[nc], b->pp_cap, cap_pairs);
+  if (*n_pairs) RSPL_HIP(hipMemcpy(pp, b->pp_buf, sizeof(int4) * (size_t)*n_pairs, hipMemcpyDeviceToHost));
+  return RSPL_OK;
+}
+
+extern "C" int rspl_ba_debug_final(rspl_ba* b, uint8_t* inlier, double* T_dev, double* T_out, double* X, double* L) {
+  RSPL_CHECK_ARG(b && inlier && T_dev && T_out && X && L, "rspl_ba_debug_final: NULL argument");
+  RSPL_CHECK_ARG(!queue_active(b), "rspl_ba_debug_final: calls are queued on the tracking thread (rspl_ba_join first)");
+  RSPL_CHECK_ARG(b->last.valid, "rspl_ba_debug_final: no completed unsharded call");
+  const ba::Problem& P = b->last.P;
+  const int E = b->last.E;
+  RSPL_HIP(hipStreamSynchronize(b->stream));
+  if (E) {
+    uint8_t* d = nullptr;
+    RSPL_HIP(hipMalloc((void**)&d, E));
+    std::vector<uint8_t> f(E);
+    std::vector<int> gmap(E);
+    hipError_t e = ba::classify(P, b->last.L, E, nullptr, d, 1, b->stream);
+    if (e == hipSuccess) e = hipStreamSynchronize(b->stream);
+    if (e == hipSuccess) e = hipMemcpy(f.data(), d, E, hipMemcpyDeviceToHost);
+    if (e == hipSuccess) e = hipMemcpy(gmap.data(), b->last.gmap, sizeof(int) * E, hipMemcpyDeviceToHost);
+    (void)hipFree(d);
+    RSPL_HIP(e);
+    for (int k = 0; k < E; k++) inlier[gmap[k]] = f[k];
+  }
+  if (P.np) RSPL_HIP(hipMemcpy(T_dev, P.T, sizeof(double) * 8 * P.np, hipMemcpyDeviceToHost));
+  if (P.nq) RSPL_HIP(hipMemcpy(X, P.X, sizeof(double) * 3 * P.nq, hipMemcpyDeviceToHost));
+  if (P.nl) RSPL_HIP(hipMemcpy(L, P.L, sizeof(double) * 6 * P.nl, hipMemcpyDeviceToHost));
+  std::copy(b->last.T_out, b->last.T_out + 8 * (size_t)P.np, T_out);
   return RSPL_OK;
 }
 
@@ -919,7 +989,7 @@
     lk.unlock();
     sc->slot = slot;
     sc->tr[1] = mono_s();
-    sc->rc = stage_call(b, slot, pr, res, *sc);
+    sc->rc = stage_call(b, slot, pr, res, *sc, true);
     sc->tr[2] = mono_s();
     sc->tr[8] = slot;
     if (sc->rc) sc->msg = rspl_last_error();
@@ -1096,8 +1166,43 @@
   return RSPL_OK;
 }
 
+extern "C" int rspl_ba_debug_pair_offsets(const rspl_ba_problem* pr, int max_landmarks, int max_poses, int32_t* pp_off,
+                                          int cap, int* n_chunks) {
+  RSPL_CHECK_ARG(pr && pp_off && n_chunks, "rspl_ba_debug_pair_offsets: NULL argument");
+  RSPL_CHECK_ARG(pr->n_poses >= 0 && pr->n_points >= 0 && pr->n_lines >= 0 && pr->n_mono >= 0 &&
+                     pr->n_stereo >= 0 && pr->n_mono_line >= 0 && pr->n_stereo_line >= 0 &&
+                     (pr->n_poses == 0 || pr->pose_fixed) && pr->n_cameras >= 1,
+                 "rspl_ba_debug_pair_offsets: bad problem sizes");
+  const int nL = pr->n_points + pr->n_lines;
+  RSPL_CHECK_ARG(max_landmarks >= nL && max_poses >= pr->n_poses, "rspl_ba_debug_pair_offsets: window beyond the handle");
+  ba::Stager stg;
+  int rc;
+  if ((rc = stg.count(pr, false, 0, 1, 0))) return rc;
+  const int E = stg.E;
+  std::vector<int> pidx(pr->n_poses);
+  ba::Active G{};
+  for (int p = 0; p < pr->n_poses; p++) pidx[p] = (stg.pose_has_edge[p] && !pr->pose_fixed[p]) ? G.K++ : -1;
+  std::vector<int> lm_off(nL + 1), epose(E + 1), elm(E + 1), ecam(E + 1), gmap(E + 1), lpose(E + 1);
+  std::vector<int8_t> etype(E + 1);
+  std::vector<double> eobs(8 * (size_t)E + 8);
+  std::vector<uint8_t> lm_act(nL + 1);
+  ba::Stager::Out so{lm_off.data(), etype.data(), epose.data(), elm.data(), ecam.data(),
+                     gmap.data(),   lpose.data(), eobs.data(),  pidx.data()};
+  stg.place(pr, so);
+  for (int g = 0; g < nL; g++) lm_act[g] = lm_off[g + 1] > lm_off[g];
+  G.npairs = G.K * (G.K + 1) / 2;
+  G.nL = nL;
+  const ba::ChunkPlan cp = ba::chunk_plan(nL, G.K, ba::chunk_slots_for(max_landmarks, max_poses));
+  G.nchk = cp.nchk; G.lmchunk = cp.lmchunk; G.dsub = cp.dsub; G.lmsub = cp.lmsub;
+  *n_chunks = ba::chunk_count(G);
+  RSPL_CHECK_ARG(cap >= *n_chunks + 1, "rspl_ba_debug_pair_offsets: %d offsets, room for %d", *n_chunks + 1, cap);
+  ba::pair_offsets(G, lm_off.data(), lpose.data(), lm_act.data(), pp_off);
+  return RSPL_OK;
+}
+
 namespace {
-int stage_call(rspl_ba* b, int slot, const rspl_ba_problem* pr, rspl_ba_result* res, ba::StagedCall& c) {
+int stage_call(rspl_ba* b, int slot, const rspl_ba_problem* pr, rspl_ba_result* res, ba::StagedCall& c,
+               bool off_chain) {
   RSPL_CHECK_ARG(b && pr && res, "rspl_ba_local: NULL argument");
   const int np = pr->n_poses, nq = pr->n_points, nl = pr->n_lines;
   const int ne[4] = {pr->n_mono, pr->n_stereo, pr->n_mono_line, pr->n_stereo_line};
@@ -1116,7 +1221,18 @@
   if ((rc = b->stg.count(pr, sh, b->rank, b->nranks, kParEdges))) return rc;
   const int E = b->stg.E, Ep = b->stg.Ep, n_line_local = E - Ep;
   tm.mark("count");
-  const CallLayout cl(pr->n_cameras, np, nq, nl, E, 4 * (size_t)Ep + 8 * (size_t)(E - Ep));
+  ba::Active G{};
+  for (int p = 0; p < np; p++) G.K += b->stg.pose_has_edge[p] && !pr->pose_fixed[p];
+  G.npairs = G.K * (G.K + 1) / 2;
+  G.nL = nL;
+  {
+    const ba::ChunkPlan cp = ba::chunk_plan(nL, G.K, b->chunk_slots);
+    G.nchk = cp.nchk;
+    G.lmchunk = cp.lmchunk;
+    G.dsub = cp.dsub;
+    G.lmsub = cp.lmsub;
+  }
+  const CallLayout cl(pr->n_cameras, np, nq, nl, E, 4 * (size_t)Ep + 8 * (size_t)(E - Ep), (size_t)ba::chunk_count(G));
   const DownLayout dl(np, nq, nl, Eg);
   bool grew = false;
   if ((rc = ensure_stage(b, slot, std::max(cl.bytes, dl.bytes), &grew))) return rc;
@@ -1152,6 +1268,7 @@
     so.lpose = reinterpret_cast<int*>(sg + cl.lm_pose);
     so.eobs = reinterpret_cast<double*>(sg + cl.obs);
     so.pidx = pidx;
+    so.ginv = sh ? nullptr : reinterpret_cast<int*>(sg + cl.ginv);
     b->stg.place(pr, so);
   }
   tm.mark("scatter");
@@ -1196,6 +1313,11 @@
       pairs[2 * q + 1] = c;
     }
   tm.mark("tables");
+  c.pp_staged = off_chain && !sh && pr->iterations_first > 0 && ba::fast_path(G.K);
+  if (c.pp_staged)
+    pair_bound = ba::pair_offsets(G, lm_off, reinterpret_cast<const int*>(sg + cl.lm_pose), lm_act,
+                                  reinterpret_cast<int*>(sg + cl.pp_off));
+  tm.mark("ppoff");
   memcpy(sg + cl.cams, pr->cameras, sizeof(double) * 5 * pr->n_cameras);
   if (nq) memcpy(sg + cl.X, pr->points, sizeof(double) * 3 * nq);
   if (nl) memcpy(sg + cl.L, pr->lines, sizeof(double) * 6 * nl);
@@ -1304,11 +1426,14 @@
   A.K = K;
   A.nL = nL;
   A.robust = 1;
-  A.pp_off = b->pp_off;
+  A.pp_off = c.pp_staged ? reinterpret_cast<const int*>(cb + cl.pp_off) : b->pp_off;
   A.pp = b->pp_buf;
   const bool pp_fused = dev_lm(b, A, pr->iterations_first);
   if (!pp_fused) RSPL_HIP(ba::build_pairs(A, b->pp_cnt, b->pp_off, b->pp_buf, st));
   tm.mark("pairs");
+  b->last.valid = false;
+  b->last.A = A;
+  b->last.fused = pp_fused && c.pp_staged;
   SpecSetup nxt;
   nxt.A2 = A;
   nxt.A2.robust = 0;
@@ -1319,6 +1444,7 @@
   const bool spec_setup = pp_fused && !sh && !b->ktime_on && dev_lm(b, nxt.A2, pr->iterations_second);
   DevLmArgs d1;
   d1.build_pp = pp_fused;
+  d1.pp_staged = c.pp_staged;
   d1.nxt = spec_setup ? &nxt : nullptr;
   if ((rc = optimize(b, P, Lr, S, A, pr->iterations_first, &res->chi2_first, &res->iterations_done_first, d1)))
     return rc;
@@ -1342,7 +1468,7 @@
     if (spec_fin) {
       fin.L = Lr;
       fin.E = E;
-      fin.gmap = reinterpret_cast<const int*>(cb + cl.gmap);
+      fin.ginv = reinterpret_cast<const int*>(cb + cl.ginv);
       fin.inl = inl_h;
       fin.Th = T_h;
       fin.Xh = X_h;
@@ -1368,7 +1494,7 @@
     if (glen && (rc = allreduce(b, b->gbuf, glen))) return rc;
     RSPL_HIP(ba::shard_finish(P, Eg, b->gbuf, inl_h, T_h, X_h, L_h, S, q, st));
   } else {
-    RSPL_HIP(ba::finish(P, Lr, E, reinterpret_cast<const int*>(cb + cl.gmap), inl_h, T_h, X_h, L_h, S, q, st));
+    RSPL_HIP(ba::finish(P, Lr, E, reinterpret_cast<const int*>(cb + cl.ginv), inl_h, T_h, X_h, L_h, S, q, st));
   }
   if ((rc = wait_mail(b, q, nullptr))) return rc;
   if (b->ktime_on) {
@@ -1415,6 +1541,12 @@
     res->pose_q[4 * p + 3] = Twc.q[0];
     for (int k = 0; k < 3; k++) res->pose_p[3 * p + k] = Twc.t[k];
   }
+  b->last.P = P;
+  b->last.L = Lr;
+  b->last.E = E;
+  b->last.gmap = reinterpret_cast<const int*>(cb + cl.gmap);
+  b->last.T_out = Tout;
+  b->last.valid = !sh;
   tm.mark("final");
   tm.print("rspl_ba_local us:");
   tr[7] = mono_s();
@@ -1427,7 +1559,7 @@
   ba::StagedCall c;
   c.tr[0] = c.tr[1] = mono_s();
   c.tr[11] = 1;
-  int rc = stage_call(b, 0, pr, res, c);
+  int rc = stage_call(b, 0, pr, res, c, false);
   c.tr[2] = c.tr[3] = mono_s();
   if (!rc) rc = run_call(b, c, pr, res, c.tr);
   if (!rc) {
diff --git a/rspl-slam_amd/csrc/ba_first.hip b/rspl-slam_amd/csrc/ba_first.hip
--- a/rspl-slam_amd/csrc/ba_first.hip
+++ b/rspl-slam_amd/csrc/ba_first.hip
@@ -181,6 +181,7 @@
   }
   const int pa = A.pairs[2 * pr], pb = A.pairs[2 * pr + 1];
   int base = FILL ? pp_off[c] : 0;
+  const int lim = FILL ? pp_off[c + 1] : 0;
   for (int r0 = 0; r0 < nr; r0 += 4) {
     int k0[4], k1[4], pz[4][8];
 #pragma unroll
@@ -236,7 +237,8 @@
         int q = base + pre - cnt;
         for (unsigned ma = ma1; ma; ma &= ma - 1) {
           const int ea = (e0 + __ffs(ma) - 1);
-          for (unsigned mb = mb1; mb; mb &= mb - 1) pp[q++] = make_int4(ea, (e0 + __ffs(mb) - 1), g, 0);
+          for (unsigned mb = mb1; mb; mb &= mb - 1, q++)
+            if (q < lim) pp[q] = make_int4(ea, (e0 + __ffs(mb) - 1), g, 0);
         }
       } else if (FILL && cnt) {
         int q = base + pre - cnt;
@@ -244,7 +246,7 @@
           if (A.lm_pose[ib] != pa) continue;
           for (int jb = e0; jb < e1; jb++) {
             if (A.lm_pose[jb] != pb) continue;
-            pp[q] = make_int4(ib, jb, g, 0);
+            if (q < lim) pp[q] = make_int4(ib, jb, g, 0);
             q++;
           }
         }
@@ -355,8 +357,9 @@
 }
 
 __global__ __launch_bounds__(256) void setup_kernel(Problem P, Lin L, Active A, Sys S, int nbq, int nb_lm,
-                                                    uint8_t* level, uint8_t* lm_act2, int* pp_cnt, int* pp_off,
-                                                    double* pdg, int lm_iters, int gate, Lin Ls, Sys Ss) {
+                                                    uint8_t* level, uint8_t* lm_act2, int4* pp_fill, int* pp_cnt,
+                                                    int* pp_off, double* pdg, int lm_iters, int gate, Lin Ls,
+                                                    Sys Ss) {
   __shared__ double red[4];
   __shared__ double part[4][64];
   __shared__ int last;
@@ -372,7 +375,10 @@
   if (b == 0 && threadIdx.x == 0) prof_stamp(S, 9);
   if (b >= nb_lm) {
     const int c = (b - nb_lm) * 4 + (threadIdx.x >> 6);
-    if (c < chunk_count(A)) pair_scan<false>(A, c, pp_cnt, nullptr, nullptr);
+    if (c < chunk_count(A)) {
+      if (pp_fill) pair_scan<true>(A, c, nullptr, A.pp_off, pp_fill);
+      else pair_scan<false>(A, c, pp_cnt, nullptr, nullptr);
+    }
     if (threadIdx.x == 0) prof_max(S, kProfX + 4);
   } else if (b >= nbq) {
     double c = 0.0;
@@ -508,19 +514,27 @@
   if (e < E) classify_edge(P, L, e, level, inlier, final_pass);
 }
 
-__global__ __launch_bounds__(256) void finish_kernel(Problem P, Lin L, int E, const int* gmap, uint8_t* inl, double* Th,
+__global__ __launch_bounds__(256) void finish_kernel(Problem P, Lin L, int E, const int* ginv, uint8_t* inl, double* Th,
                                                      double* Xh, double* Lh, Sys S, unsigned long long seq) {
   __shared__ int last;
+  __shared__ uint4 fl4[16];
   if (S.lm) {
     const LmCtrl* c = S.lm + S.lm_slot;
     if (!c->stop) return;
     if (c->cur) bank_state(P);
   }
   const int i = blockIdx.x * blockDim.x + threadIdx.x;
-  if (i < E) inl[gmap[i]] = edge_inlier(P, L, i) ? 1 : 0;
-  if (i < 8 * P.np) Th[i] = P.T[i];
-  if (i < 3 * P.nq) Xh[i] = P.X[i];
-  if (i < 6 * P.nl) Lh[i] = P.L[i];
+  reinterpret_cast<uint8_t*>(fl4)[threadIdx.x] = i < E && edge_inlier(P, L, ginv[i]) ? 1 : 0;
+  auto put2 = [i](double* dst, const double* src, int n) {
+    if (2 * i + 1 < n) *reinterpret_cast<double2*>(dst + 2 * i) = make_double2(src[2 * i], src[2 * i + 1]);
+    else if (2 * i < n) dst[2 * i] = src[2 * i];
+  };
+  put2(Th, P.T, 8 * P.np);
+  put2(Xh, P.X, 3 * P.nq);
+  put2(Lh, P.L, 6 * P.nl);
+  __syncthreads();
+  if (threadIdx.x < 16 && blockIdx.x * 256 + 16 * (int)threadIdx.x < E)
+    reinterpret_cast<uint4*>(inl)[blockIdx.x * 16 + threadIdx.x] = fl4[threadIdx.x];
   __threadfence_system();
   __syncthreads();
   if (threadIdx.x == 0) {
@@ -619,18 +633,21 @@
 }
 
 hipError_t setup_dev(const Problem& P, const Lin& L, const Active& A, Sys& S, uint8_t* level, uint8_t* lm_act2,
-                     int lm_iters, int* pp_cnt, int* pp_off, int4* pp, double* pdg, hipStream_t s, int gate,
+                     int lm_iters, int4* pp, int* pp_cnt, int* pp_off, double* pdg, hipStream_t s, int gate,
                      const Lin* Ls, const Sys* Ss) {
-  if (gate >= 0 && (!Ls || !Ss || pp_cnt)) return hipErrorInvalidValue;
+  if (gate >= 0 && (!Ls || !Ss || pp)) return hipErrorInvalidValue;
+  if (pp_cnt && !pp_off) return hipErrorInvalidValue;
   if (!S.lm || lm_iters <= 0) return hipErrorInvalidValue;
   Active A0 = A;
   A0.elevel = nullptr;
   const int nc = chunk_count(A);
-  if (nc == 0) pp_cnt = nullptr;
+  if (nc == 0) pp = nullptr;
+  if (!pp) pp_cnt = nullptr;
+  int4* const pp_fill = pp_cnt ? nullptr : pp;
   const int nbq = A.nL > 0 ? (A.nL * kGroup + 255) / 256 : 0, nb = nbq + A.n_lblk;
-  const int nbp = pp_cnt ? (nc + 3) / 4 : 0;
+  const int nbp = pp ? (nc + 3) / 4 : 0;
   hipLaunchKernelGGL(setup_kernel, dim3(std::max(nb + nbp, 1)), dim3(256), 0, s, P, L, A0, S, nbq, nb, level, lm_act2,
-                     pp_cnt, pp_off, pdg, lm_iters, gate, Ls ? *Ls : L, Ss ? *Ss : S);
+                     pp_fill, pp_cnt, pp_off, pdg, lm_iters, gate, Ls ? *Ls : L, Ss ? *Ss : S);
   if (pp_cnt) hipLaunchKernelGGL(pair_fill_kernel, dim3(nc), dim3(64), 0, s, A, pp_off, pp);
   return hipGetLastError();
 }
@@ -641,10 +658,10 @@
   return hipGetLastError();
 }
 
-hipError_t finish(const Problem& P, const Lin& L, int E, const int* gmap, uint8_t* inl, double* Th, double* Xh,
+hipError_t finish(const Problem& P, const Lin& L, int E, const int* ginv, uint8_t* inl, double* Th, double* Xh,
                   double* Lh, Sys& S, unsigned long long seq, hipStream_t s) {
-  const int n = std::max(std::max(E, 8 * P.np), std::max(3 * P.nq, 6 * P.nl));
-  hipLaunchKernelGGL(finish_kernel, dim3(std::max((n + 255) / 256, 1)), dim3(256), 0, s, P, L, E, gmap, inl, Th, Xh,
+  const int n = std::max(std::max(E, 4 * P.np), std::max((3 * P.nq + 1) / 2, 3 * P.nl));
+  hipLaunchKernelGGL(finish_kernel, dim3(std::max((n + 255) / 256, 1)), dim3(256), 0, s, P, L, E, ginv, inl, Th, Xh,
                      Lh, S, seq);
   return hipGetLastError();
 }
diff --git a/rspl-slam_amd/csrc/ba_kernels.hpp b/rspl-slam_amd/csrc/ba_kernels.hpp
--- a/rspl-slam_amd/csrc/ba_kernels.hpp
+++ b/rspl-slam_amd/csrc/ba_kernels.hpp
@@ -184,7 +184,7 @@
                      hipStream_t s);
 hipError_t post(Sys& S, unsigned long long seq, hipStream_t s, const Active* A = nullptr);
 hipError_t setup_dev(const Problem& P, const Lin& L, const Active& A, Sys& S, uint8_t* level, uint8_t* lm_act2,
-                     int lm_iters, int* pp_cnt, int* pp_off, int4* pp, double* pdg, hipStream_t s, int gate = -1,
+                     int lm_iters, int4* pp, int* pp_cnt, int* pp_off, double* pdg, hipStream_t s, int gate = -1,
                      const Lin* Ls = nullptr, const Sys* Ss = nullptr);
 int setup_pdg_len(const Active& A);
 struct Spec {
@@ -199,7 +199,7 @@
 hipError_t landmark_active(const Active& A, const uint8_t* level, uint8_t* lm_act, hipStream_t s);
 hipError_t classify(const Problem& P, const Lin& L, int E, uint8_t* level, uint8_t* inlier, int final_pass,
                     hipStream_t s);
-hipError_t finish(const Problem& P, const Lin& L, int E, const int* gmap, uint8_t* inl, double* Th, double* Xh,
+hipError_t finish(const Problem& P, const Lin& L, int E, const int* ginv, uint8_t* inl, double* Th, double* Xh,
                   double* Lh, Sys& S, unsigned long long seq, hipStream_t s);
 hipError_t trial_chunks(const Problem& P, const Lin& L, const Active& A, Sys& S, double lambda, hipStream_t s);
 hipError_t trial_solve(const Problem& P, const Lin& L, const Active& A, Sys& S, double lambda, hipStream_t s);
diff --git a/rspl-slam_amd/csrc/ba_stage.cpp b/rspl-slam_amd/csrc/ba_stage.cpp
--- a/rspl-slam_amd/csrc/ba_stage.cpp
+++ b/rspl-slam_amd/csrc/ba_stage.cpp
@@ -157,6 +157,7 @@
   const int nq = pr->n_points, nL = nq + pr->n_lines;
   int* lm_off = o.lm_off;
   int* gmap = o.gmap;
+  int* ginv = o.ginv;
   const int* pidx = o.pidx;
   const int Ep_ = Ep;
   double* lobs = o.eobs + 4 * (size_t)Ep_;
@@ -165,6 +166,7 @@
     static const double zero = 0.0;
     for (int k = k0; k < std::min(k1, Ep_); k++) {
       const int eg = gmap[k];
+      if (ginv) ginv[eg] = k;
       const bool st = eg >= e1;
       const int i = st ? eg - e1 : eg;
       const int32_t* pt = st ? ed.pose[1] : ed.pose[0];
@@ -183,6 +185,7 @@
     }
     for (int k = std::max(k0, Ep_); k < k1; k++) {
       const int eg = gmap[k];
+      if (ginv) ginv[eg] = k;
       const int t = eg >= e3 ? 3 : 2;
       const int i = eg - (t == 3 ? e3 : e2);
       const int p = ed.pose[t][i];
@@ -234,5 +237,40 @@
   gather(0, E);
 }
 
-}
-}
+size_t pair_offsets(const Active& G, const int* lm_off, const int* lm_pose, const uint8_t* lm_act, int* pp_off) {
+  const int nc = chunk_count(G), K = G.K;
+  static thread_local std::vector<int> n, first, cnt, seen;
+  n.assign((size_t)nc + 1, 0);
+  first.assign(std::max(G.npairs, 1), 0);
+  for (int c = 0; c < nc;) {
+    const ChunkGeo q = chunk_geo(G, c);
+    first[q.pr] = q.c0;
+    c = q.c1;
+  }
+  cnt.assign(std::max(K, 1), 0);
+  for (int g = 0; g < G.nL; g++) {
+    if (!lm_act[g]) continue;
+    seen.clear();
+    for (int k = lm_off[g]; k < lm_off[g + 1]; k++) {
+      const int p = lm_pose[k];
+      if (p >= 0 && cnt[p]++ == 0) seen.push_back(p);
+    }
+    const int lb = g / G.lmchunk;
+    const int sub = G.dsub > 1 ? lb * G.dsub + (g - lb * G.lmchunk) / G.lmsub : lb;
+    for (size_t i = 0; i < seen.size(); i++) {
+      const int a = seen[i];
+      n[first[a * K - a * (a - 1) / 2] + sub + 1] += cnt[a] * cnt[a];
+      for (size_t j = i + 1; j < seen.size(); j++) {
+        const int lo = std::min(a, seen[j]), hi = std::max(a, seen[j]);
+        n[first[lo * K - lo * (lo - 1) / 2 + hi - lo] + lb + 1] += cnt[lo] * cnt[hi];
+      }
+    }
+    for (const int p : seen) cnt[p] = 0;
+  }
+  for (int c = 0; c < nc; c++) n[c + 1] += n[c];
+  std::copy(n.begin(), n.end(), pp_off);
+  return (size_t)n[nc];
+}
+
+}
+}
diff --git a/rspl-slam_amd/csrc/ba_stage.hpp b/rspl-slam_amd/csrc/ba_stage.hpp
--- a/rspl-slam_amd/csrc/ba_stage.hpp
+++ b/rspl-slam_amd/csrc/ba_stage.hpp
@@ -3,6 +3,7 @@
 #include <memory>
 #include <vector>
 
+#include "ba_kernels.hpp"
 #include "common.hpp"
 #include "host_pool.hpp"
 
@@ -21,6 +22,7 @@
     int* lpose;
     double* eobs;
     const int* pidx;
+    int* ginv = nullptr;
   };
   void place(const rspl_ba_problem* pr, const Out& o);
 
@@ -38,5 +40,7 @@
   std::vector<int> pcut_, gcut_, rstart_;
 };
 
+size_t pair_offsets(const Active& G, const int* lm_off, const int* lm_pose, const uint8_t* lm_act, int* pp_off);
+
 }
 }
diff --git a/rspl-slam_amd/csrc/common.hpp b/rspl-slam_amd/csrc/common.hpp
--- a/rspl-slam_amd/csrc/common.hpp
+++ b/rspl-slam_amd/csrc/common.hpp
@@ -105,6 +105,10 @@
   }
 };
 
+constexpr unsigned kTimingEventFlags = hipEventDisableSystemFence;
+constexpr unsigned kOrderEventFlags = hipEventDisableTiming | hipEventReleaseToDevice;
+constexpr unsigned kHostEventFlags = hipEventDisableTiming;
+
 struct StageTimer {
   static constexpr int kRing = 64, kMax = 8;
   int n = 0;
@@ -118,7 +122,7 @@
     n = nstages;
     for (int r = 0; r < kRing; r++)
       for (int i = 0; i <= n; i++)
-        if (hipEventCreate(&ev[r][i]) != hipSuccess) return RSPL_E_DEVICE;
+        if (hipEventCreateWithFlags(&ev[r][i], kTimingEventFlags) != hipSuccess) return RSPL_E_DEVICE;
     return RSPL_OK;
   }
   void destroy() {
@@ -170,6 +174,7 @@
 int load_blob(const char* path, std::vector<Tensor>& out);
 
 hipError_t upload_mapped(void* dst, const void* src_mapped, size_t bytes, hipStream_t s);
+hipError_t copy_device(void* dst, const void* src, size_t bytes, hipStream_t s);
 const Tensor* find(const std::vector<Tensor>& ts, const std::string& name, int64_t numel);
 
 }
diff --git a/rspl-slam_amd/csrc/copy_kernels.hip b/rspl-slam_amd/csrc/copy_kernels.hip
--- a/rspl-slam_amd/csrc/copy_kernels.hip
+++ b/rspl-slam_amd/csrc/copy_kernels.hip
@@ -25,4 +25,36 @@
   return hipGetLastError();
 }
 
+template <typename V>
+__global__ __launch_bounds__(256) void copy_kernel(uint8_t* dst, const uint8_t* src, size_t head, size_t nv,
+                                                   size_t ntail) {
+  const size_t t = (size_t)blockIdx.x * 256 + threadIdx.x;
+  V* dv = reinterpret_cast<V*>(dst + head);
+  const V* sv = reinterpret_cast<const V*>(src + head);
+  for (size_t i = t; i < nv; i += (size_t)gridDim.x * 256) dv[i] = sv[i];
+  if (t < head) dst[t] = src[t];
+  if (t < ntail) dst[head + sizeof(V) * nv + t] = src[head + sizeof(V) * nv + t];
 }
+
+template <typename V>
+static hipError_t copy_launch(uint8_t* dst, const uint8_t* src, size_t bytes, hipStream_t s) {
+  constexpr size_t w = sizeof(V);
+  const size_t head = std::min<size_t>((w - reinterpret_cast<uintptr_t>(dst) % w) % w, bytes);
+  const size_t nv = (bytes - head) / w, ntail = bytes - head - w * nv;
+  const unsigned blocks = (unsigned)std::max<size_t>(1, std::min<size_t>((nv + 255) / 256, 1024));
+  hipLaunchKernelGGL(copy_kernel<V>, dim3(blocks), dim3(256), 0, s, dst, src, head, nv, ntail);
+  return hipGetLastError();
+}
+
+hipError_t copy_device(void* dst, const void* src, size_t bytes, hipStream_t s) {
+  if (!bytes) return hipSuccess;
+  uint8_t* d = static_cast<uint8_t*>(dst);
+  const uint8_t* c = static_cast<const uint8_t*>(src);
+  const uintptr_t skew = reinterpret_cast<uintptr_t>(dst) ^ reinterpret_cast<uintptr_t>(src);
+  if (skew % 16 == 0) return copy_launch<uint4>(d, c, bytes, s);
+  if (skew % 8 == 0) return copy_launch<uint2>(d, c, bytes, s);
+  if (skew % 4 == 0) return copy_launch<uint32_t>(d, c, bytes, s);
+  return copy_launch<uint8_t>(d, c, bytes, s);
+}
+
+}
diff --git a/rspl-slam_amd/csrc/lines.cpp b/rspl-slam_amd/csrc/lines.cpp
--- a/rspl-slam_amd/csrc/lines.cpp
+++ b/rspl-slam_amd/csrc/lines.cpp
@@ -908,7 +908,7 @@
     h->pin_cap = capacity;
   }
   const int k = h->pin_next;
-  if (!h->copy_ev[k]) RSPL_HIP(hipEventCreateWithFlags(&h->copy_ev[k], hipEventDisableTiming));
+  if (!h->copy_ev[k]) RSPL_HIP(hipEventCreateWithFlags(&h->copy_ev[k], kOrderEventFlags));
   if (h->copy_pending[k]) {
     RSPL_HIP(hipEventSynchronize(h->copy_ev[k]));
     h->copy_pending[k] = false;
@@ -981,7 +981,7 @@
       set_error("detector scratch carving failed");
       return RSPL_E_DEVICE;
     }
-    for (hipEvent_t& e : h->fld_ev) RSPL_HIP(hipEventCreate(&e));
+    for (hipEvent_t& e : h->fld_ev) RSPL_HIP(hipEventCreateWithFlags(&e, kTimingEventFlags));
   }
   if (hp > h->fld_hp) {
     if (h->fld_img) {
@@ -1253,8 +1253,8 @@
   constexpr size_t kPinBytes = sizeof(int32_t) * (fld::kMetaInts + 1) + sizeof(float) * 4 * rspl_lines::kDevSegCap;
   if (!h->dev_pin) {
     RSPL_HIP(hipHostMalloc((void**)&h->dev_pin, kPinBytes, hipHostMallocDefault));
-    RSPL_HIP(hipEventCreateWithFlags(&h->dev_in, hipEventDisableTiming));
-    RSPL_HIP(hipEventCreateWithFlags(&h->dev_done, hipEventDisableTiming));
+    RSPL_HIP(hipEventCreateWithFlags(&h->dev_in, kOrderEventFlags));
+    RSPL_HIP(hipEventCreateWithFlags(&h->dev_done, kHostEventFlags));
   }
   if (int rc = fld_reserve(h, (size_t)(H / 2) * (W / 2))) return rc;
   RSPL_HIP(hipEventRecord(h->dev_in, (hipStream_t)stream));
diff --git a/rspl-slam_amd/csrc/runtime.cpp b/rspl-slam_amd/csrc/runtime.cpp
--- a/rspl-slam_amd/csrc/runtime.cpp
+++ b/rspl-slam_amd/csrc/runtime.cpp
@@ -64,7 +64,18 @@
 }
 int rspl_memcpy_d2d(void* dst, const void* src, size_t bytes, void* stream) {
   if (!bytes) return RSPL_OK;
-  RSPL_HIP(hipMemcpyAsync(dst, src, bytes, hipMemcpyDeviceToDevice, (hipStream_t)stream));
+  int cur = -1;
+  hipPointerAttribute_t ad{}, as{};
+  const bool local = hipGetDevice(&cur) == hipSuccess &&
+                     hipPointerGetAttributes(&ad, dst) == hipSuccess && hipPointerGetAttributes(&as, src) == hipSuccess &&
+                     ad.type == hipMemoryTypeDevice && as.type == hipMemoryTypeDevice && ad.device == cur &&
+                     as.device == cur;
+  if (!local) {
+    (void)hipGetLastError();
+    RSPL_HIP(hipMemcpyAsync(dst, src, bytes, hipMemcpyDeviceToDevice, (hipStream_t)stream));
+    return RSPL_OK;
+  }
+  RSPL_HIP(copy_device(dst, src, bytes, (hipStream_t)stream));
   return RSPL_OK;
 }
 int rspl_stream_create(void** stream) {
@@ -102,7 +113,7 @@
 }
 int rspl_event_create(void** event) {
   RSPL_CHECK_ARG(event, "NULL event");
-  RSPL_HIP(hipEventCreateWithFlags((hipEvent_t*)event, hipEventDisableTiming));
+  RSPL_HIP(hipEventCreateWithFlags((hipEvent_t*)event, kOrderEventFlags));
   return RSPL_OK;
 }
 int rspl_event_record(void* event, void* stream) {
@@ -124,7 +135,8 @@
 int rspl_timer_create(rspl_timer** t) {
   RSPL_CHECK_ARG(t, "NULL timer");
   auto* x = new rspl_timer();
-  if (hipEventCreate(&x->ev[0]) != hipSuccess || hipEventCreate(&x->ev[1]) != hipSuccess) {
+  if (hipEventCreateWithFlags(&x->ev[0], kTimingEventFlags) != hipSuccess ||
+      hipEventCreateWithFlags(&x->ev[1], kTimingEventFlags) != hipSuccess) {
     set_error("hipEventCreate failed");
     delete x;
     return RSPL_E_DEVICE;
diff --git a/rspl-slam_amd/csrc/sg.cpp b/rspl-slam_amd/csrc/sg.cpp
--- a/rspl-slam_amd/csrc/sg.cpp
+++ b/rspl-slam_amd/csrc/sg.cpp
@@ -334,10 +334,10 @@
   }
   const size_t nm = s->nmax;
   if (s->timer.init(RSPL_SG_STAGES) != RSPL_OK || hipStreamCreateWithFlags(&s->stream, hipStreamNonBlocking) != hipSuccess ||
-      hipEventCreateWithFlags(&s->ev_ready, hipEventDisableTiming) != hipSuccess ||
-      hipEventCreateWithFlags(&s->ev_sink[0], hipEventDisableTiming) != hipSuccess ||
-      hipEventCreateWithFlags(&s->ev_sink[1], hipEventDisableTiming) != hipSuccess ||
-      hipEventCreateWithFlags(&s->ev_done, hipEventDisableTiming) != hipSuccess ||
+      hipEventCreateWithFlags(&s->ev_ready, kOrderEventFlags) != hipSuccess ||
+      hipEventCreateWithFlags(&s->ev_sink[0], kOrderEventFlags) != hipSuccess ||
+      hipEventCreateWithFlags(&s->ev_sink[1], kOrderEventFlags) != hipSuccess ||
+      hipEventCreateWithFlags(&s->ev_done, kOrderEventFlags) != hipSuccess ||
       hipHostMalloc(&s->h_f, sizeof(double) * nm * 259 * 2) != hipSuccess ||
       hipHostMalloc(&s->h_idx, sizeof(int32_t) * nm * 2 + 16) != hipSuccess ||
       hipHostMalloc(&s->h_ms, sizeof(double) * nm * 2) != hipSuccess ||
```

Result: faster. 1051 (median of 6 runs) (+1.9%).
